# honglianghe/CDNet

Measured on AMD Instinct MI355X. Metric: tiles/sec (train fwd+bwd+Adam), 256x256, higher is better.
Workload: dtype fp32

## Files before the change

cdnet_amd/_lib.py:

```python
import ctypes as C
import os

_HERE = os.path.dirname(os.path.abspath(__file__))
LIB_PATH = os.environ.get('CDNET_LIB_PATH') or os.path.join(_HERE, 'libcdnet_hip.so')

_vp, _i, _sz, _f, _u = C.c_void_p, C.c_int, C.c_size_t, C.c_float, C.c_uint


class ConvSrc(C.Structure):
    _fields_ = [('x', C.c_void_p), ('res', C.c_void_p), ('scale', C.c_void_p), ('shift', C.c_void_p),
                ('C', C.c_int), ('Hs', C.c_int), ('Ws', C.c_int), ('pool', C.c_int), ('relu', C.c_int),
                ('off_y', C.c_int), ('off_x', C.c_int), ('f16', C.c_int), ('row_stride', C.c_int)]


class ConvArgs(C.Structure):
    _fields_ = [('src', ConvSrc * 2), ('nsrc', C.c_int), ('w', C.c_void_p), ('bias', C.c_void_p),
                ('oscale', C.c_void_p), ('oshift', C.c_void_p), ('orelu', C.c_int), ('out', C.c_void_p),
                ('Cout', C.c_int), ('out_cstride', C.c_int), ('out_coff', C.c_int), ('stats', C.c_void_p),
                ('N', C.c_int), ('H', C.c_int), ('W', C.c_int), ('taps', C.c_int), ('npar', C.c_int),
                ('ostride', C.c_int), ('nchunk', C.c_int), ('tile', C.c_int), ('CK', C.c_int), ('BN', C.c_int),
                ('out_f16', C.c_int), ('debug', C.c_int), ('ws', C.c_int), ('f32', C.c_int),
                ('eres', C.c_void_p), ('eres_scale', C.c_void_p), ('eres_shift', C.c_void_p), ('eres_f16', C.c_int), ('eres_relu', C.c_int),
                ('taps1', C.c_int), ('pad_', C.c_int), ('pool_out', C.c_void_p),
                ('dot_w', C.c_void_p), ('dot_b', C.c_void_p), ('dot_out', C.c_void_p)]


class PackJob(C.Structure):
    _fields_ = [('w', C.c_void_p), ('packed', C.c_void_p), ('Cout', C.c_int), ('Cin', C.c_int), ('KH', C.c_int), ('KW', C.c_int),
                ('CK', C.c_int), ('BN', C.c_int), ('mode', C.c_int), ('pad_', C.c_int)]


class HeadFeat(C.Structure):
    _fields_ = [('raw', C.c_void_p), ('res', C.c_void_p), ('scale', C.c_void_p), ('shift', C.c_void_p),
                ('relu', C.c_int), ('f16', C.c_int)]


class FuseTerm(C.Structure):
    _fields_ = [('x', C.c_void_p), ('Hs', C.c_int), ('Ws', C.c_int), ('scale', C.c_void_p), ('shift', C.c_void_p),
                ('f16', C.c_int), ('pad_', C.c_int)]


class GradTerm(C.Structure):
    _fields_ = [('g', C.c_void_p), ('cstride', C.c_int), ('coff', C.c_int)]


class GradIn(C.Structure):
    _fields_ = [('g', C.c_void_p), ('Hg', C.c_int), ('Wg', C.c_int), ('oy', C.c_int), ('ox', C.c_int),
                ('pooled', C.c_int), ('coff', C.c_int), ('cstride', C.c_int), ('pad_', C.c_int)]


class BnBwdArgs(C.Structure):
    _fields_ = [('raw', C.c_void_p), ('res', C.c_void_p), ('scale', C.c_void_p), ('shift', C.c_void_p),
                ('mean', C.c_void_p), ('invstd', C.c_void_p), ('gin', GradIn * 3), ('ngin', C.c_int),
                ('f16', C.c_int), ('relu', C.c_int), ('N', C.c_int), ('H', C.c_int), ('W', C.c_int), ('C', C.c_int),
                ('hc_coef', C.c_void_p), ('hc_w', C.c_void_p), ('hc_slot', C.c_int), ('hc_k0', C.c_int), ('hc_nk', C.c_int),
                ('hc_pad_', C.c_int)]


class AugSample(C.Structure):
    _fields_ = [('minv', C.c_double * 6), ('img', C.c_void_p), ('weight', C.c_void_p), ('label', C.c_void_p)] + \
        [(n, C.c_int32) for n in ('H', 'W', 'img_stride', 'weight_stride', 'label_stride', 'label_i32')] + \
        [('color', C.c_float * 4)] + [(n, C.c_int32) for n in ('hflip', 'vflip', 'filter', 'y0', 'x0')] + \
        [('alpha', C.c_float), ('sigma', C.c_float), ('seed', C.c_uint32)]


class AugGeo(C.Structure):
    _fields_ = [('paff', C.c_double * 6), ('rinv', C.c_double * 6)] + [(n, C.c_int32) for n in ('Hr', 'Wr', 'fy0', 'fx0')] + \
        [('flags', C.c_uint32), ('reserved', C.c_int32)]


class WgradReduceDesc(C.Structure):
    _fields_ = [('slab', C.c_void_p), ('dw', C.c_void_p)] + [(n, C.c_int) for n in (
        'ksplit', 'npar', 'ci_blocks', 'co_blocks', 'taps', 'CI', 'CO', 'Csrc_real', 'Cin_real', 'src_coff', 'Cout', 'mode', 'block0', 'blocks')]

class DilatedConvArgs(C.Structure):
    _fields_ = [(n, C.c_void_p) for n in ('in_', 'w', 'scale', 'shift', 'out')] + [(n, C.c_int) for n in (
        'N', 'H', 'W', 'Cin', 'in_cstride', 'Cout', 'out_cstride', 'out_coff', 'taps', 'dilation', 'leaky')] + [
        ('slope', C.c_float), ('f32', C.c_int), ('out_nchw', C.c_int)]

class DilatedBwdDataArgs(C.Structure):
    _fields_ = [(n, C.c_void_p) for n in ('g', 'w', 'dx')] + [(n, C.c_int) for n in (
        'N', 'H', 'W', 'Cout', 'g_cstride', 'Cin', 'dx_cstride', 'dx_coff', 'taps', 'dilation', 'accumulate', 'f32')]

class DilatedWgradArgs(C.Structure):
    _fields_ = [(n, C.c_void_p) for n in ('x', 'g', 'dw', 'ws')] + [('ws_bytes', C.c_size_t)] + [(n, C.c_int) for n in (
        'N', 'H', 'W', 'Cin', 'x_cstride', 'Cout', 'g_cstride', 'taps', 'dilation')]

class SliceBnFwdArgs(C.Structure):
    _fields_ = [(n, C.c_void_p) for n in ('z', 'out', 'gamma', 'beta', 'running_mean', 'running_var', 'mean', 'invstd', 'ws')] + [
        ('ws_floats', C.c_size_t), ('P', C.c_longlong)] + [(n, C.c_int) for n in ('C', 'z_cstride', 'out_cstride', 'out_coff')] + [
        (n, C.c_float) for n in ('eps', 'momentum', 'p_drop')] + [('layer', C.c_int), ('key', C.c_ulonglong)]

class SliceBnBwdArgs(C.Structure):
    _fields_ = [(n, C.c_void_p) for n in ('dy', 'z', 'mean', 'invstd', 'gamma', 'dgamma', 'dbeta', 'g', 'ws')] + [
        ('ws_floats', C.c_size_t), ('P', C.c_longlong)] + [(n, C.c_int) for n in ('C', 'z_cstride', 'dy_cstride', 'dy_coff', 'g_cstride')] + [
        (n, C.c_float) for n in ('slope', 'p_drop')] + [('layer', C.c_int), ('key', C.c_ulonglong)]


MIRRORS = {
    'cdnet_conv_src': ConvSrc, 'cdnet_conv_args': ConvArgs, 'cdnet_pack_job': PackJob, 'cdnet_head_feat': HeadFeat,
    'cdnet_wgrad_reduce_desc': WgradReduceDesc, 'cdnet_grad_in': GradIn, 'cdnet_bn_bwd_args': BnBwdArgs, 'cdnet_fuse_term': FuseTerm,
    'cdnet_grad_term': GradTerm, 'cdnet_aug_sample': AugSample, 'cdnet_aug_geo': AugGeo, 'cdnet_dilated_conv_args': DilatedConvArgs,
    'cdnet_dilated_bwd_data_args': DilatedBwdDataArgs, 'cdnet_dilated_wgrad_args': DilatedWgradArgs,
    'cdnet_slice_bn_fwd_args': SliceBnFwdArgs, 'cdnet_slice_bn_bwd_args': SliceBnBwdArgs,
}

SIGNATURES = {
    'cdnet_abi_version': (_i, []),
    'cdnet_abi_sizeof': (_sz, [C.c_char_p]),
    'cdnet_last_error': (C.c_char_p, []),
    'cdnet_build_info': (C.c_char_p, []),
    'cdnet_spin': (_i, [_i, _vp]),
    'cdnet_box_copy': (_i, [_vp, _vp, _sz, _vp]),
    'cdnet_box_mfma': (_i, [_vp, _vp, _vp, _i, _i, _i, _vp]),
    'cdnet_ddm_codes': (_i, [_vp, _i, _i, _i, _i, _vp, _i, _i, _vp, _vp, _vp]),
    'cdnet_ddm_normalize': (_i, [_vp, _vp, _i, _i, _i, _vp, _vp]),
    'cdnet_probmaps': (_i, [_vp, _vp, _i, _i, _i, _i, _vp, _vp, _vp]),
    'cdnet_tta_boost_argmax': (_i, [_vp, _vp, _vp, _vp, _i, _i, _vp, _i, _i, _vp, _vp, _vp, _vp, _vp, _vp]),
    'cdnet_fuse_sum': (_i, [_vp, _i, _i, _i, _i, _i, _i, _vp, _i, _i, _vp]),
    'cdnet_upsample_bilinear_backward': (_i, [_vp, _i, _i, _i, _i, _i, _i, _i, _i, _vp, _vp]),
    'cdnet_s2d_to_nhwc': (_i, [_vp, _i, _i, _i, _i, _vp, _vp]),
    'cdnet_fuse_sum_f32': (_i, [_vp, _i, _i, _i, _i, _i, _i, _vp, _i, _i, _vp]),
    'cdnet_upsample_bilinear_backward_f32': (_i, [_vp, _i, _i, _i, _i, _i, _i, _i, _i, _vp, _vp]),
    'cdnet_s2d_to_nhwc_f32': (_i, [_vp, _i, _i, _i, _i, _vp, _vp]),
    'cdnet_bn_backward_stats': (_i, [_vp, _vp, _vp, _vp, _vp, _sz, _vp, _vp]),
    'cdnet_bn_backward_apply': (_i, [_vp, _vp, _vp, _vp]),
    'cdnet_bn_backward_finalize': (_i, [_vp, _vp, _vp, _vp, _vp, _i, _vp, _vp]),
    'cdnet_conv_ws_eligible': (_i, [_vp]),
    'cdnet_grad_sum': (_i, [_vp, _i, _vp, C.c_longlong, _i, _vp, _vp]),
    'cdnet_grad_sum_f32': (_i, [_vp, _i, _vp, C.c_longlong, _i, _vp, _vp]),
    'cdnet_label_pair_histogram': (_i, [_vp, _vp, _i, _i, _i, _i, _vp, _vp, _vp, _vp, _vp, _vp]),
    'cdnet_remap_label': (_i, [_vp, _i, _i, _i, _vp, _vp, _vp, _vp]),
    'cdnet_label_areas': (_i, [_vp, _i, _i, _i, _vp, _vp, _vp]),
    'cdnet_label_apply': (_i, [_vp, _i, _i, _i, _vp, _vp, _vp]),
    'cdnet_label_csr_workspace_bytes': (_sz, [_i]),
    'cdnet_label_csr': (_i, [_vp, _i, _i, _i, _vp, _sz, _vp, _vp, _vp, _vp, _vp]),
    'cdnet_hausdorff_tile_pixels': (_i, []),
    'cdnet_hausdorff_chunk_pixels': (_i, []),
    'cdnet_hausdorff_pairs': (_i, [_vp] * 8 + [_i, _i, _i, _vp, _i, _vp, _i, _vp, _vp, _vp]),
    'cdnet_watershed_workspace_bytes': (_sz, [_i, _i, _i]),
    'cdnet_watershed_process': (_i, [_vp, _i, _i, _i, _i, _vp, _sz, _vp, _vp, _vp, _vp]),
    'cdnet_fill_label_process': (_i, [_vp, _i, _i, _i, _i, _vp, _sz, _vp, _vp]),
    'cdnet_label_process': (_i, [_vp, _i, _i, _i, _i, _vp, _sz, _vp, _vp]),
    'cdnet_instance_redilate_workspace_bytes': (_sz, [_i, _i, _i, _i]),
    'cdnet_instance_redilate': (_i, [_vp, _i, _i, _i, _i, _i, _vp, _sz, _vp, _vp, _vp]),
    'cdnet_instance_redilate_lds_rows': (_i, []),
    'cdnet_instance_redilate_lds_cols': (_i, []),
    'cdnet_label_count': (_i, [_vp, _i, _i, _i, _vp, _vp, _vp, _vp]),
    'cdnet_tile_postproc_workspace_bytes': (_sz, [_i, _i, _i, _i]),
    'cdnet_tile_postproc': (_i, [_vp, _vp, _vp, _i, _i, _i, _i, _vp, _i, _i, _i, _i, _vp, _sz] + [_vp] * 10),
    'cdnet_cc_workspace_bytes': (_sz, [_i, _i, _i]),
    'cdnet_cc_chain': (_i, [_vp, _i, _i, _i, _i, _i, _i, _vp, _sz, _vp, _vp, _vp, _vp, _vp, _vp]),
    'cdnet_mask_views_argmax': (_i, [_vp, _i, _i, _i, _vp, _i, _i, _vp, _vp, _vp]),
    'cdnet_tile_mask_postproc_workspace_bytes': (_sz, [_i, _i, _i, _i]),
    'cdnet_tile_mask_postproc': (_i, [_vp, _i, _i, _i, _i, _i, _i, _vp, _sz] + [_vp] * 8),
    'cdnet_dilate_labels': (_i, [_vp, _i, _i, _i, _i, _vp, _vp]),
    'cdnet_conv_packed_weight_elems': (_sz, [_i] * 6),
    'cdnet_pack_conv_weights': (_i, [_vp, _vp] + [_i] * 7 + [_vp]),
    'cdnet_pack_conv_weights_scaled': (_i, [_vp, _vp, _vp] + [_i] * 7 + [_vp]),
    'cdnet_pack_batch_table_bytes': (_sz, [_i]),
    'cdnet_pack_conv_weights_batch': (_i, [_vp, _i, _vp, _sz, _i, _vp]),
    'cdnet_conv_forward': (_i, [_vp, _vp]),
    'cdnet_dilated_packed_weight_elems': (_sz, [_i, _i, _i, _i]),
    'cdnet_dilated_pack_weights': (_i, [_vp, _vp, _i, _i, _i, _i, _vp]),
    'cdnet_dilated_conv_forward': (_i, [_vp, _vp]),
    'cdnet_dilated_pack_weights_bwd': (_i, [_vp, _vp, _i, _i, _i, _i, _vp]),
    'cdnet_dilated_conv_backward_data': (_i, [_vp, _vp]),
    'cdnet_dilated_wgrad_workspace_bytes': (_sz, [_i] * 6),
    'cdnet_dilated_conv_backward_weight': (_i, [_vp, _vp]),
    'cdnet_slice_bn_workspace_floats': (_sz, [C.c_longlong, _i]),
    'cdnet_slice_bn_train_forward': (_i, [_vp, _vp]),
    'cdnet_slice_bn_train_backward': (_i, [_vp, _vp]),
    'cdnet_dropout_mask': (_i, [C.c_ulonglong, _i, _sz, _f, _vp, _vp]),
    'cdnet_maxpool2_forward': (_i, [_vp, _i, _vp, _i, _i, _vp, _i, _i, _i, _i, _i, _i, _vp]),
    'cdnet_maxpool2_backward': (_i, [_vp, _i, _i, _vp, _i, _vp, _i, _i, _i, _i, _i, _vp]),
    'cdnet_upsample4_bilinear_forward': (_i, [_vp, _i, _vp, _i, _i, _i, _i, _i, _i, _i, _vp]),
    'cdnet_upsample4_bilinear_backward': (_i, [_vp, _i, _i, _vp, _i, _i, _i, _i, _i, _vp]),
    'cdnet_src_materialize': (_i, [_vp, _i, _i, _i, _vp, _vp]),
    'cdnet_input_pack': (_i, [_vp, _i, _i, _i, _i, _vp, _vp]),
    'cdnet_input_pack_f32': (_i, [_vp, _i, _i, _i, _i, _vp, _vp]),
    'cdnet_bn_fold_eval': (_i, [_vp, _vp, _vp, _vp, _vp, _f, _i, _vp, _vp, _vp]),
    'cdnet_bn_finalize_train': (_i, [_vp, _i, _i, _f, _vp, _vp, _vp, _f, _f, _vp, _vp, _vp, _vp, _vp, _vp, _vp]),
    'cdnet_dam_head_forward': (_i, [_vp, _vp, _vp, _vp, _i, _i, _i, _vp, _vp, _vp, _vp]),
    'cdnet_final_conv1x1': (_i, [_vp, _vp, _vp, _i, _i, _i, _i, _vp, _vp]),
    'cdnet_bias_grad_workspace_floats': (_sz, [_i]),
    'cdnet_bias_grad': (_i, [_vp, _sz, _i, _vp, _sz, _vp, _vp]),
    'cdnet_bias_grad_f32': (_i, [_vp, _sz, _i, _vp, _sz, _vp, _vp]),
    'cdnet_final_conv1x1_backward_workspace_floats': (_sz, []),
    'cdnet_final_conv1x1_backward': (_i, [_vp, _vp, _vp, _i, _i, _i, _i, _vp, _vp, _sz, _vp, _vp, _vp]),
    'cdnet_final_conv1x1_c16': (_i, [_vp, _vp, _vp, _i, _i, _i, _i, _vp, _vp]),
    'cdnet_final_conv1x1_c16_backward_workspace_floats': (_sz, []),
    'cdnet_final_conv1x1_c16_backward': (_i, [_vp, _vp, _vp, _i, _i, _i, _i, _vp, _vp, _sz, _vp, _vp, _vp]),
    'cdnet_conv_wgrad_slab_floats': (_sz, [_i] * 6),
    'cdnet_conv_backward_weight': (_i, [_vp, _i, _i, _i, _vp] + [_i] * 9 + [_vp, _vp, _i, _vp]),
    'cdnet_conv_backward_weight_last_form': (_i, []),
    'cdnet_conv_forward_last_form': (_i, []),
    'cdnet_wgrad_reduce_desc_fill': (_i, [_i] * 9 + [_vp, _vp, _i, _i, _vp]),
    'cdnet_wgrad_reduce_batch': (_i, [_vp, _i, _i, _vp]),
    'cdnet_bn_backward_workspace_floats': (_sz, [_i]),
    'cdnet_bn_backward': (_i, [_vp, _vp, _vp, _vp, _vp, _sz, _vp, _vp, _vp]),
    'cdnet_bn_backward_last_plan': (_i, []),
    'cdnet_bn_backward_last_sums_plan': (_i, []),
    'cdnet_dam_head_backward_workspace_floats': (_sz, [_i, _i, _i]),
    'cdnet_dam_head_backward': (_i, [_vp] * 7 + [_i, _i, _i, _vp, _vp, _vp, _vp, _sz, _vp, _vp]),
    'cdnet_dam_head_backward_fused_blocks': (_i, []),
    'cdnet_dam_head_backward_fused_scratch_bytes': (_i, []),
    'cdnet_dam_head_backward_fused_workspace_floats': (_sz, []),
    'cdnet_dam_head_backward_fused': (_i, [_vp] * 7 + [_i, _i, _i, _vp, _vp, _vp, _vp, _sz, _vp, _vp]),
    'cdnet_dam_head_backward_coef_scratch_bytes': (_i, []),
    'cdnet_dam_head_backward_coef': (_i, [_vp] * 7 + [_i, _i, _i, _vp, _vp, _vp, _sz, _vp, _vp]),
    'cdnet_dam_loss_workspace_floats': (_sz, [_i, _i]),
    'cdnet_dam_loss': (_i, [_vp] * 7 + [_i, _i, _i, _i, _vp, _sz, _vp, _vp, _vp, _vp, _vp]),
    'cdnet_dam_loss_classes_workspace_floats': (_sz, [_i, _i, _i]),
    'cdnet_dam_loss_classes': (_i, [_vp] * 7 + [_i, _i, _i, _i, _i, _vp, _sz, _vp, _vp, _vp, _vp, _vp]),
    'cdnet_dam_loss_terms': (_i, [_vp] * 7 + [_i, _i, _i, _i, _i, _vp, _sz, _vp, _vp, _vp, _vp, _vp, _u]),
    'cdnet_mask_loss_workspace_floats': (_sz, [_i, _i]),
    'cdnet_mask_loss': (_i, [_vp, _vp, _vp, _i, _i, _i, _u, _vp, _sz, _vp, _vp, _vp]),
    'cdnet_variance_loss_workspace_bytes': (_sz, [_i, _i, _i, _i]),
    'cdnet_variance_loss': (_i, [_vp, _vp, _i, _i, _i, _i, _i, _f, _vp, _sz, _vp, _vp, _vp, _vp, _vp, _vp]),
    'cdnet_boundary_loss_workspace_bytes': (_sz, [_i, _i, _i, _i, _i]),
    'cdnet_boundary_loss': (_i, [_vp, _vp, _i, _i, _i, _i, _i, _f, _vp, _sz, _vp, _vp, _vp, _vp]),
    'cdnet_boundary_loss_scratch_bytes': (_i, []),
    'cdnet_dam_val_sums_workspace_floats': (_sz, [_i, _i]),
    'cdnet_dam_val_sums': (_i, [_vp] * 8 + [_i, _i, _i, _vp, _sz, _vp, _vp]),
    'cdnet_dam_val_sums_classes_workspace_floats': (_sz, [_i, _i, _i]),
    'cdnet_dam_val_sums_classes': (_i, [_vp] * 8 + [_i, _i, _i, _i, _vp, _sz, _vp, _vp]),
    'cdnet_adam_step': (_i, [_vp, _vp, _vp, _vp, _sz, _f, _f, _f, _f, _f, _i, _f, _vp]),
    'cdnet_moment_step': (_i, [_vp, _vp, _vp, _vp, _vp, _sz, C.c_double, C.c_double, _f, _i, _i, _f, _f, _f, _f, _i, _f, _vp]),
    'cdnet_sgd_step': (_i, [_vp, _vp, _vp, _sz, _f, _f, _f, _i, _f, _vp]),
    'cdnet_window_pack': (_i, [_vp] + [_i] * 9 + [_vp, _vp]),
    'cdnet_window_pack_f32': (_i, [_vp] + [_i] * 9 + [_vp, _vp]),
    'cdnet_window_stitch': (_i, [_vp] + [_i] * 9 + [_vp, _vp]),
    'cdnet_label_encoding_workspace_bytes': (_sz, [_i, _i, _i, _i]),
    'cdnet_label_encoding_instances_workspace_bytes': (_sz, [_i, _i, _i, _i]),
    'cdnet_label_encoding_instances': (_i, [_vp, _i, _i, _i, _i, _vp, _vp, _vp, _sz, _vp, _vp, _vp, _vp, _vp, _vp]),
    'cdnet_augment_workspace_bytes': (_sz, [_i, _i, _i]),
    'cdnet_augment_batch': (_i, [_vp, _vp, _i, _i, _vp, _vp, _sz, _vp, _vp, _vp, _i, _vp, _vp, _vp]),
    'cdnet_augment_geo_workspace_bytes': (_sz, [_i, _i, _i, _i]),
    'cdnet_augment_batch_geo': (_i, [_vp, _vp, _vp, _vp, _i, _i, _i, _vp, _vp, _sz, _vp, _vp, _vp, _i, _vp, _vp, _vp]),
    'cdnet_label_encoding': (_i, [_vp, _i, _i, _i, _i, _vp, _vp, _vp, _sz, _vp, _vp, _vp, _vp, _vp, _vp]),
    'cdnet_weight_map_radius': (_i, [C.c_double, C.c_double]),
    'cdnet_weight_map': (_i, [_vp, _i, _i, C.c_double, C.c_double, _vp, _vp]),
    'cdnet_resize_workspace_bytes': (_sz, [_i] * 7),
    'cdnet_resize_bilinear': (_i, [_vp] + [_i] * 6 + [_vp, _vp, _i, _vp, _vp, _i, _i, _i, _vp, _sz, _vp, _vp]),
    'cdnet_resize_last_form': (_i, []),
    'cdnet_fill_remove_small': (_i, [_vp, _i, _i, _i, _i, _i, _vp, _sz, _vp, _vp]),
    'cdnet_label8_dilate': (_i, [_vp, _i, _i, _i, _i, _vp, _sz, _vp, _vp, _vp, _vp]),
}

_lib = None


class CdnetHipError(RuntimeError):
    pass


def load():
    global _lib
    if _lib is not None:
        return _lib
    import torch
    if not os.path.exists(LIB_PATH):
        raise CdnetHipError('libcdnet_hip.so is not built: run `python -m cdnet_amd.csrc.build` '
                            '(or __graft_entry__.build()). There is no CPU fallback.')
    lib = C.CDLL(LIB_PATH)
    for name, (res, args) in SIGNATURES.items():
        fn = getattr(lib, name)
        fn.restype = res
        fn.argtypes = args
    if lib.cdnet_abi_version() != 5:
        raise CdnetHipError('ABI version mismatch (libcdnet_hip.so is version %d, this binding 5): rebuild with python -m cdnet_amd.csrc.build' % lib.cdnet_abi_version())
    _lib = lib
    return lib


def check(status, what=''):
    if status != 0:
        msg = load().cdnet_last_error().decode(errors='replace')
        raise CdnetHipError('%s failed (code %d): %s' % (what, status, msg))


def call(name, *args):
    check(getattr(load(), name)(*args), name)


def entry(name, f32):
    return name + '_f32' if f32 else name


_RAW_STREAM = None


def stream_ptr():
    global _RAW_STREAM
    if _RAW_STREAM is None:
        import torch
        get, dev = getattr(torch._C, '_cuda_getCurrentRawStream', None), getattr(torch._C, '_cuda_getDevice', None)
        if get is not None and dev is not None:
            _RAW_STREAM = lambda: get(dev())
        else:
            _RAW_STREAM = lambda: torch.cuda.current_stream().cuda_stream
    return C.c_void_p(_RAW_STREAM())


def ptr(t):
    if t is None:
        return None
    assert t.is_cuda and t.is_contiguous(), 'ABI needs contiguous device tensors'
    return C.c_void_p(t.data_ptr())
```

cdnet_amd/csrc/build.py:

```python
import os
import subprocess
import sys

HERE = os.path.dirname(os.path.abspath(__file__))
PKG = os.path.dirname(HERE)
LIB = os.path.join(PKG, 'libcdnet_hip.so')
OBJ_DIR = os.path.join(HERE, 'build')
SOURCES = ['abi.hip', 'box.hip', 'postproc.hip', 'postproc_tile.hip', 'conv.hip', 'conv_ws.hip', 'pack.hip', 'conv32.hip', 'conv32ws.hip', 'conv16ws.hip', 'dilated.hip', 'dilated_train.hip', 'resample.hip', 'wgrad.hip', 'model.hip', 'head_bwd.hip', 'classifier16.hip', 'dam_loss.hip', 'bn_bwd.hip', 'cdm.hip', 'metrics.hip', 'augment.hip', 'optim.hip', 'variance.hip', 'boundary.hip', 'mask_loss.hip', 'weight_map.hip', 'instance_fill.hip', 'resize.hip']
FLAGS = ['--offload-arch=gfx950', '-O3', '-std=c++20', '-fPIC', '-ffp-contract=off', '-Wall',
         '-Wno-unused-function', '-Wno-unused-result']


def _newer(a, bs):
    return os.path.exists(a) and all(os.path.getmtime(a) >= os.path.getmtime(b) for b in bs)


def build(force=False, verbose=False):
    hipcc = os.environ.get('HIPCC', 'hipcc')
    flags = FLAGS + os.environ.get('CDNET_HIPCC_FLAGS', '').split()
    os.makedirs(OBJ_DIR, exist_ok=True)
    headers = [os.path.join(HERE, f) for f in os.listdir(HERE) if f.endswith('.h')]
    headers.append(os.path.join(os.path.dirname(PKG), 'include', 'cdnet_hip.h'))
    objs, procs = [], []
    for s in SOURCES:
        src = os.path.join(HERE, s)
        if not os.path.exists(src):
            continue
        obj = os.path.join(OBJ_DIR, s.replace('.hip', '.o'))
        objs.append(obj)
        if force or not _newer(obj, [src] + headers):
            cmd = [hipcc] + flags + ['-c', src, '-o', obj]
            if verbose:
                print(' '.join(cmd))
            procs.append((s, subprocess.Popen(cmd)))
    for s, p in procs:
        if p.wait() != 0:
            raise RuntimeError('hipcc failed on ' + s)
    if force or procs or not _newer(LIB, objs):
        cmd = [hipcc, '--offload-arch=gfx950', '-shared', '-fPIC', '-o', LIB] + objs
        if verbose:
            print(' '.join(cmd))
        subprocess.check_call(cmd)
    return LIB


if __name__ == '__main__':
    print(build(force='--force' in sys.argv, verbose=True))
```

cdnet_amd/csrc/conv32.hip:

```cpp
#include <type_traits>
#include "common.h"
#include "conv_args.h"
#include "launch.h"
#include "split_bf16.h"
#include <stdlib.h>

using namespace cdnet;

namespace {

constexpr int CK = 16;
constexpr int PSTR = CK * 2 + 16;
constexpr int XF_MAX = 2048;

template <int TH, int TW, int BN, int TAPS>
struct Lds32 {
    static constexpr int NPIX = (TH + 2) * (TW + 2);
    static constexpr int A_PLANE = NPIX * PSTR;
    static constexpr int B_PLANE = TAPS * CK * BN * 2;
    static constexpr int STAGE = 2 * A_PLANE + 2 * B_PLANE;
    static constexpr int STATS_BYTES = 4 * 2 * BN * 4;
    static constexpr int MAIN = ((STAGE > STATS_BYTES ? STAGE : STATS_BYTES) + 15) / 16 * 16;
    static int bytes(int ctot) { return MAIN + 2 * ((ctot + 7) / 8 * 8) * 4; }
};


template <int MPW, int NPW, int TW>
__device__ __forceinline__ void store_tile_f32(const ConvArgs &A, const f32x16 (&acc)[MPW][NPW], int n, int y0, int x0, int mblock0, int nblock0,
                                               int half, int l31, int cout0, int pa_, int pb_) {
    const int Ho = A.H * A.ostride, Wo = A.W * A.ostride;
    float *out = reinterpret_cast<float *>(A.out);
    const float *eres = reinterpret_cast<const float *>(A.eres);
    const bool full = y0 + 16 <= A.H && x0 + TW <= A.W && cout0 + (nblock0 + NPW) * 32 <= A.Cout && A.ostride == 1 && TW == 16 &&
                      !(A.debug & 16);
    if (full) {
        const int cs = A.out_cstride, ce = A.Cout;
        float *tb = out + (((size_t)n * A.H + y0) * A.W + x0) * cs + A.out_coff;
        const float *te = eres ? eres + (((size_t)n * A.H + y0) * A.W + x0) * ce : nullptr;
#pragma unroll
        for (int ni = 0; ni < NPW; ++ni) {
            const int co = cout0 + (nblock0 + ni) * 32 + l31;
            const float osc = A.oscale ? A.oscale[co] : 1.f;
            const float osh = fmaf(A.bias ? A.bias[co] : 0.f, osc, A.oshift ? A.oshift[co] : 0.f);
            const float esc = (eres && A.eres_scale) ? A.eres_scale[co] : 1.f;
            const float esh = (eres && A.eres_shift) ? A.eres_shift[co] : 0.f;
            float *ob = tb + co;
#pragma unroll
            for (int mi = 0; mi < MPW; ++mi) {
                const int rowb = ((mblock0 + mi) * 2) * A.W + 4 * half;
                float ev[16];
                if (eres) {
#pragma unroll
                    for (int r = 0; r < 16; ++r) {
                        const int p = (r & 3) + 8 * (r >> 2);
                        ev[r] = te[(rowb + (p / 16) * A.W + (p % 16)) * ce + co];
                    }
                }
#pragma unroll
                for (int r = 0; r < 16; ++r) {
                    const int p = (r & 3) + 8 * (r >> 2);
                    const int off = (rowb + (p / 16) * A.W + (p % 16)) * cs;
                    float v = fmaf(acc[mi][ni][r], osc, osh);
                    if (A.orelu) v = fmaxf(v, 0.f);
                    if (eres) {
                        v = fmaf(ev[r], esc, esh) + v;
                        if (A.eres_relu) v = fmaxf(v, 0.f);
                    }
                    ob[off] = v;
                }
            }
        }
        return;
    }
#pragma unroll
    for (int ni = 0; ni < NPW; ++ni) {
        const int co = cout0 + (nblock0 + ni) * 32 + l31;
        const bool cok = co < A.Cout;
        const float osc = (A.oscale && cok) ? A.oscale[co] : 1.f;
        const float osh = fmaf((A.bias && cok) ? A.bias[co] : 0.f, osc, (A.oshift && cok) ? A.oshift[co] : 0.f);
        const float esc = (A.eres && A.eres_scale && cok) ? A.eres_scale[co] : 1.f;
        const float esh = (A.eres && A.eres_shift && cok) ? A.eres_shift[co] : 0.f;
#pragma unroll
        for (int mi = 0; mi < MPW; ++mi) {
            float ev[16];
            if (A.eres) {
#pragma unroll
                for (int r = 0; r < 16; ++r) {
                    const int m = (mblock0 + mi) * 32 + (r & 3) + 8 * (r >> 2) + 4 * half;
                    int y = y0 + m / TW, x = x0 + m % TW;
                    y = y < A.H ? y : A.H - 1; x = x < A.W ? x : A.W - 1;
                    ev[r] = eres[(((size_t)n * A.H + y) * A.W + x) * A.Cout + (cok ? co : 0)];
                }
            }
#pragma unroll
            for (int r = 0; r < 16; ++r) {
                const int m = (mblock0 + mi) * 32 + (r & 3) + 8 * (r >> 2) + 4 * half;
                const int y = y0 + m / TW, x = x0 + m % TW;
                float v = fmaf(acc[mi][ni][r], osc, osh);
                if (A.orelu) v = fmaxf(v, 0.f);
                if (A.eres) {
                    v = fmaf(ev[r], esc, esh) + v;
                    if (A.eres_relu) v = fmaxf(v, 0.f);
                }
                if (cok && y < A.H && x < A.W) {
                    const size_t opix = ((size_t)n * Ho + (y * A.ostride + pa_)) * Wo + (x * A.ostride + pb_);
                    out[opix * A.out_cstride + A.out_coff + co] = v;
                }
            }
        }
    }
}

template <int TH, int TW, int BN, int WM, int WN, int TAPS>
__global__ __launch_bounds__(256, 2) void conv_f32_kernel(ConvArgs A) {
    using L = Lds32<TH, TW, BN, TAPS>;
    constexpr int HW_ = TW + 2, NPIX = L::NPIX;
    constexpr int MT = TH * TW / 32, NT = BN / 32;
    constexpr int MPW = MT / WM, NPW = NT / WN;
    constexpr int VPP = CK / 8;
    constexpr int NA = (NPIX * VPP + 255) / 256;
    constexpr int NBV = 2 * L::B_PLANE / 16;
    constexpr int NB = (NBV + 255) / 256;
    static_assert(MT % WM == 0 && NT % WN == 0 && WM * WN == 4, "wave tiling");

    extern __shared__ __attribute__((aligned(16))) unsigned char smem[];
    unsigned char *lds_a = smem;
    unsigned char *lds_b = smem + 2 * L::A_PLANE;
    float (*s_stats)[2][BN] = reinterpret_cast<float (*)[2][BN]>(smem);
    float *s_xf = reinterpret_cast<float *>(smem + L::MAIN);

    const int tid = threadIdx.x, lane = tid & 63, wave = tid >> 6;
    const int wm = wave / WN, wn = wave % WN;
    const int half = lane >> 5, l31 = lane & 31;
    const int c0n = A.src[0].C, ctot = c0n + (A.nsrc > 1 ? A.src[1].C : 0);
    const int xfs = (ctot + 7) / 8 * 8;
    for (int c = tid; c < ctot; c += 256) {
        const ConvSrc &S = c < c0n ? A.src[0] : A.src[1];
        const int cc = c < c0n ? c : c - c0n;
        s_xf[c] = S.scale ? S.scale[cc] : 1.f;
        s_xf[xfs + c] = S.shift ? S.shift[cc] : 0.f;
    }

    const int tiles_x = (A.W + TW - 1) / TW, tiles_y = (A.H + TH - 1) / TH;
    const int tiles_img = tiles_x * tiles_y;
    int tile, cout_tile;
    {
        const int NC = (int)gridDim.y, lin = (int)blockIdx.y * (int)gridDim.x + (int)blockIdx.x;
        const int T = (int)gridDim.x * NC, q = T >> 3, rem = T & 7;
        const int xcd = lin & 7, idx = lin >> 3;
        const int seq = xcd < rem ? xcd * (q + 1) + idx : rem * (q + 1) + (xcd - rem) * q + idx;
        tile = seq / NC;
        cout_tile = seq - tile * NC;
    }
    const int z = tile / tiles_img, rt = tile - z * tiles_img;
    const int n = z / A.npar, par = z - n * A.npar;
    const int ty_ = rt / tiles_x;
    const int y0 = ty_ * TH, x0 = (rt - ty_ * tiles_x) * TW;

    int eoff[2][NA];
    const int slot = tid % VPP;
#pragma unroll
    for (int si = 0; si < 2; ++si) {
        if (si >= A.nsrc) break;
        const ConvSrc &s = A.src[si];
        const int rs = s.row_stride ? s.row_stride : s.Ws * s.C;
#pragma unroll
        for (int i = 0; i < NA; ++i) {
            const int v = tid + i * 256;
            const int pix = v / VPP;
            const int hy = pix / HW_, hx = pix - hy * HW_;
            const int y = y0 - 1 + hy, x = x0 - 1 + hx;
            const int ys = y - s.off_y, xs = x - s.off_x;
            const bool ok = v < NPIX * VPP && (unsigned)y < (unsigned)A.H && (unsigned)x < (unsigned)A.W && (unsigned)ys < (unsigned)s.Hs &&
                            (unsigned)xs < (unsigned)s.Ws;
            eoff[si][i] = ok ? ys * rs + xs * s.C + slot * 8 : -1;
        }
    }
    auto chunk_src = [&](int c, int &si, int &cc0) {
        const int n0 = A.src[0].C / CK;
        if (c < n0) { si = 0; cc0 = c * CK; } else { si = 1; cc0 = (c - n0) * CK; }
    };
    const unsigned short *wbase = A.w + ((size_t)(par * gridDim.y + cout_tile) * A.nchunk) * (size_t)(L::B_PLANE);

    f32x4 pa[NA][2];
    u32x4 pb[NB];
    auto issue = [&](int chunk) {
        int si, cc0;
        chunk_src(chunk, si, cc0);
        const ConvSrc &s = A.src[si];
        const size_t rs = s.row_stride ? (size_t)s.row_stride : (size_t)s.Ws * s.C;
        const float *base = reinterpret_cast<const float *>(s.x) + (size_t)n * s.Hs * rs + cc0;
#pragma unroll
        for (int i = 0; i < NA; ++i) {
            const int e = si ? eoff[1][i] : eoff[0][i];
            const f32x4 *p = reinterpret_cast<const f32x4 *>(base + (e >= 0 ? e : 0));
            pa[i][0] = p[0];
            pa[i][1] = p[1];
        }
        const u32x4 *wsrc = reinterpret_cast<const u32x4 *>(wbase + (size_t)chunk * L::B_PLANE);
#pragma unroll
        for (int i = 0; i < NB; ++i) {
            const int v = tid + i * 256;
            if (v < NBV) pb[i] = wsrc[v];
        }
    };
    auto commit = [&](int chunk) {
        int si, cc0;
        chunk_src(chunk, si, cc0);
        const ConvSrc &s = A.src[si];
        const bool on = s.scale != nullptr, relu = s.relu != 0;
        const float *xf = s_xf + (si ? c0n : 0) + cc0 + slot * 8;
        float sc[8], sh[8];
        if (on) {
#pragma unroll
            for (int j = 0; j < 8; ++j) { sc[j] = xf[j]; sh[j] = xf[xfs + j]; }
        }
        f32x4 rr[NA][2];
        if (s.res) {
            const size_t rs = s.row_stride ? (size_t)s.row_stride : (size_t)s.Ws * s.C;
            const float *rbase = reinterpret_cast<const float *>(s.res) + (size_t)n * s.Hs * rs + cc0;
#pragma unroll
            for (int i = 0; i < NA; ++i) {
                const int e = si ? eoff[1][i] : eoff[0][i];
                const f32x4 *p = reinterpret_cast<const f32x4 *>(rbase + (e >= 0 ? e : 0));
                rr[i][0] = p[0];
                rr[i][1] = p[1];
            }
        }
        unsigned char *dst0 = lds_a + (tid / VPP) * PSTR + slot * 16;
#pragma unroll
        for (int i = 0; i < NA; ++i) {
            if (tid + i * 256 >= NPIX * VPP) continue;
            const int e = si ? eoff[1][i] : eoff[0][i];
            u32x4 hi = {0u, 0u, 0u, 0u}, lo = {0u, 0u, 0u, 0u};
            if (e >= 0) {
                float v[8] = {pa[i][0][0], pa[i][0][1], pa[i][0][2], pa[i][0][3], pa[i][1][0], pa[i][1][1], pa[i][1][2], pa[i][1][3]};
                if (on) {
#pragma unroll
                    for (int j = 0; j < 8; ++j) v[j] = fmaf(v[j], sc[j], sh[j]);
                }
                if (s.res) {
                    const float r[8] = {rr[i][0][0], rr[i][0][1], rr[i][0][2], rr[i][0][3], rr[i][1][0], rr[i][1][1], rr[i][1][2], rr[i][1][3]};
#pragma unroll
                    for (int j = 0; j < 8; ++j) v[j] += r[j];
                }
                if (relu) {
#pragma unroll
                    for (int j = 0; j < 8; ++j) v[j] = fmaxf(v[j], 0.f);
                }
                split8(v, hi, lo);
            }
            unsigned char *d = dst0 + i * (256 / VPP) * PSTR;
            *reinterpret_cast<u32x4 *>(d) = hi;
            *reinterpret_cast<u32x4 *>(d + L::A_PLANE) = lo;
        }
        u32x4 *bdst = reinterpret_cast<u32x4 *>(lds_b);
#pragma unroll
        for (int i = 0; i < NB; ++i) {
            const int v = tid + i * 256;
            if (v < NBV) bdst[v] = pb[i];
        }
    };

    int abase[MPW];
#pragma unroll
    for (int mi = 0; mi < MPW; ++mi) {
        const int m = (wm * MPW + mi) * 32 + l31;
        abase[mi] = ((m / TW) * HW_ + m % TW) * PSTR + half * 16;
    }
    const int bbase = half * BN * 16 + (wn * NPW * 32 + l31) * 16;
    int toff[TAPS];
#pragma unroll
    for (int t = 0; t < TAPS; ++t) {
        int r, c;
        if (TAPS == 9) { r = t / 3; c = t % 3; }
        else if (TAPS == 4) {
            const int a = par >> 1, b = par & 1, ty = t >> 1, tx = t & 1;
            r = a == 0 ? (ty == 0 ? 1 : 0) : (ty == 0 ? 2 : 1);
            c = b == 0 ? (tx == 0 ? 1 : 0) : (tx == 0 ? 2 : 1);
        } else { r = 1; c = 1; }
        toff[t] = (r * HW_ + c) * PSTR;
    }
    f32x16 acc[MPW][NPW];
#pragma unroll
    for (int mi = 0; mi < MPW; ++mi)
#pragma unroll
        for (int ni = 0; ni < NPW; ++ni)
#pragma unroll
            for (int r = 0; r < 16; ++r) acc[mi][ni][r] = 0.f;

    issue(0);
    for (int chunk = 0; chunk < A.nchunk; ++chunk) {
        __syncthreads();
        commit(chunk);
        __syncthreads();
        if (chunk + 1 < A.nchunk) issue(chunk + 1);
#pragma unroll
        for (int t = 0; t < TAPS; ++t) {
            bf16x8 ah[MPW], al[MPW], bh[NPW], bl[NPW];
#pragma unroll
            for (int mi = 0; mi < MPW; ++mi) {
                ah[mi] = *reinterpret_cast<const bf16x8 *>(lds_a + abase[mi] + toff[t]);
                al[mi] = *reinterpret_cast<const bf16x8 *>(lds_a + L::A_PLANE + abase[mi] + toff[t]);
            }
#pragma unroll
            for (int ni = 0; ni < NPW; ++ni) {
                bh[ni] = *reinterpret_cast<const bf16x8 *>(lds_b + bbase + t * 2 * BN * 16 + ni * 512);
                bl[ni] = *reinterpret_cast<const bf16x8 *>(lds_b + L::B_PLANE + bbase + t * 2 * BN * 16 + ni * 512);
            }
#pragma unroll
            for (int mi = 0; mi < MPW; ++mi)
#pragma unroll
                for (int ni = 0; ni < NPW; ++ni) {
                    acc[mi][ni] = mfma3(acc[mi][ni], ah[mi], al[mi], bh[ni], bl[ni]);
                }
        }
    }
    __syncthreads();

    const int cout0 = cout_tile * BN;
    if (A.stats) {
        float ssum[NPW], ssq[NPW];
        const bool full_tile = y0 + TH <= A.H && x0 + TW <= A.W && !(A.debug & 16);
#pragma unroll
        for (int ni = 0; ni < NPW; ++ni) {
            ssum[ni] = 0.f; ssq[ni] = 0.f;
            if (full_tile) {
#pragma unroll
                for (int mi = 0; mi < MPW; ++mi)
#pragma unroll
                    for (int r = 0; r < 16; ++r) {
                        const float v = acc[mi][ni][r];
                        ssum[ni] += v;
                        ssq[ni] = fmaf(v, v, ssq[ni]);
                    }
            } else {
#pragma unroll
            for (int mi = 0; mi < MPW; ++mi)
#pragma unroll
                for (int r = 0; r < 16; ++r) {
                    const int m = (wm * MPW + mi) * 32 + (r & 3) + 8 * (r >> 2) + 4 * half;
                    const float v = ((y0 + m / TW) < A.H && (x0 + m % TW) < A.W) ? acc[mi][ni][r] : 0.f;
                    ssum[ni] += v;
                    ssq[ni] = fmaf(v, v, ssq[ni]);
                }
            }
            ssum[ni] += __shfl_xor(ssum[ni], 32);
            ssq[ni] += __shfl_xor(ssq[ni], 32);
            if (half == 0) {
                s_stats[wave][0][(wn * NPW + ni) * 32 + l31] = ssum[ni];
                s_stats[wave][1][(wn * NPW + ni) * 32 + l31] = ssq[ni];
            }
        }
        __syncthreads();
        if (tid < 2 * BN) {
            const int which = tid / BN, col = tid % BN;
            const int wn_of = col / (NPW * 32);
            float v = 0.f;
#pragma unroll
            for (int k = 0; k < WM; ++k) v += s_stats[k * WN + wn_of][which][col];
            const int co = cout0 + col;
            if (co < A.Cout) A.stats[((size_t)tile * 2 + which) * A.Cout + co] = v;
        }
    }
    store_tile_f32<MPW, NPW, TW>(A, acc, n, y0, x0, wm * MPW, wn * NPW, half, l31, cout0, par >> 1, par & 1);
}

template <int TH, int TW, int BN, int WM, int WN, int TAPS>
int launch_conv32(const ConvArgs &A, hipStream_t st) {
    using L = Lds32<TH, TW, BN, TAPS>;
    int ctot = 0;
    for (int i = 0; i < A.nsrc; ++i) ctot += A.src[i].C;
    const int smem = L::bytes(ctot);
    dim3 grid(cdiv(A.W, TW) * cdiv(A.H, TH) * A.N * A.npar, cdiv(A.Cout, BN), 1);
    g_conv_last_form = conv_form(CDNET_CONV_FAMILY_F32, BN, TAPS, 0, false, false, false, 0, 0, TH);
    return launch_lds<conv_f32_kernel<TH, TW, BN, WM, WN, TAPS>>(grid, 256, L::bytes(XF_MAX), smem, st, "hipFuncSetAttribute(conv32)", "conv_f32_kernel", A);
}

template <int TAPS>
int dispatch_conv32(const ConvArgs &A, hipStream_t st) {
    if (A.tile == 16 && A.BN == 64) return launch_conv32<16, 16, 64, 4, 1, TAPS>(A, st);
    if (A.tile == 16 && A.BN == 32) return launch_conv32<16, 16, 32, 4, 1, TAPS>(A, st);
    if (A.tile == 8 && A.BN == 64) return launch_conv32<8, 8, 64, 2, 2, TAPS>(A, st);
    set_error("cdnet_conv_forward(f32): unsupported configuration tile=%d CK=%d BN=%d", A.tile, A.CK, A.BN);
    return CDNET_E_ARG;
}

template <int BN, int NCH, bool XF, bool ERES>
__global__ __launch_bounds__(256, 4) void conv1x1_f32_stream_kernel(ConvArgs A) {
    constexpr int NPW = BN / 32;
    constexpr int B_PLANE = CK * BN * 2;
    constexpr int CIN = NCH * CK;
    __shared__ __attribute__((aligned(16))) unsigned char smem[NCH * 2 * B_PLANE + 2 * CIN * 4];
    unsigned char *lds_b = smem;
    float *s_xf = reinterpret_cast<float *>(smem + NCH * 2 * B_PLANE);

    const int tid = threadIdx.x, lane = tid & 63, wave = __builtin_amdgcn_readfirstlane(tid >> 6);
    const int half = lane >> 5, l31 = lane & 31;
    const int cout_tile = blockIdx.y, cout0 = cout_tile * BN;
    const ConvSrc &S = A.src[0];
    {
        const u32x4 *wsrc = reinterpret_cast<const u32x4 *>(A.w + (size_t)cout_tile * NCH * B_PLANE);
        u32x4 *bdst = reinterpret_cast<u32x4 *>(lds_b);
        for (int v = tid; v < NCH * 2 * B_PLANE / 16; v += 256) bdst[v] = wsrc[v];
        for (int c = tid; c < CIN; c += 256) {
            s_xf[c] = S.scale ? S.scale[c] : 1.f;
            s_xf[CIN + c] = S.shift ? S.shift[c] : 0.f;
        }
    }
    __syncthreads();

    const size_t P = (size_t)A.N * A.H * A.W;
    const int nblk = (int)((P + 31) / 32), bstride = (int)gridDim.x * 4;
    int blk = (int)blockIdx.x * 4 + wave;
    if (blk >= nblk) return;
    const bool relu = S.relu != 0, orelu = A.orelu != 0, eres_relu = A.eres_relu != 0;
    const int cout = A.Cout;
    const int bbase = half * BN * 16 + l31 * 16;

    float osc[NPW], osh[NPW], esc[NPW], esh[NPW];
#pragma unroll
    for (int ni = 0; ni < NPW; ++ni) {
        const int co = cout0 + ni * 32 + l31, c = co < A.Cout ? co : 0;
        osc[ni] = A.oscale ? A.oscale[c] : 1.f;
        osh[ni] = fmaf(A.bias ? A.bias[c] : 0.f, osc[ni], A.oshift ? A.oshift[c] : 0.f);
        esc[ni] = (ERES && A.eres_scale) ? A.eres_scale[c] : 1.f;
        esh[ni] = (ERES && A.eres_shift) ? A.eres_shift[c] : 0.f;
    }

    const char *xbase = reinterpret_cast<const char *>(S.x);
    char *obase = reinterpret_cast<char *>(A.out) + (size_t)A.out_coff * 4;
    const char *ebase = ERES ? reinterpret_cast<const char *>(A.eres) : xbase;
    const unsigned cs4 = (unsigned)A.out_cstride * 4, ce4 = (unsigned)cout * 4;
    const unsigned vo_in = l31 * (CIN * 4) + half * 32;
    unsigned vo_out[NPW], vo_eres[NPW];
#pragma unroll
    for (int ni = 0; ni < NPW; ++ni) {
        const unsigned co = cout0 + ni * 32 + l31;
        vo_out[ni] = co < (unsigned)cout ? 4 * half * cs4 + co * 4 : 0x7fff0000u;
        vo_eres[ni] = co < (unsigned)cout ? 4 * half * ce4 + co * 4 : 0x7fff0000u;
    }
    auto rsrc = [&](const char *base, size_t bytes) {
        return __builtin_amdgcn_make_buffer_rsrc(const_cast<char *>(base), 0, (int)bytes, 0x00020000);
    };

    auto request = [&](f32x4 (&v)[NCH][2], int b) {
        const size_t left = P - (size_t)b * 32;
        const __amdgpu_buffer_rsrc_t rx = rsrc(xbase + (size_t)b * (32 * CIN * 4), (left < 32 ? left : 32) * (CIN * 4));
#pragma unroll
        for (int c = 0; c < NCH; ++c) {
            v[c][0] = __builtin_bit_cast(f32x4, __builtin_amdgcn_raw_buffer_load_b128(rx, (int)(vo_in + c * 64), 0, 0));
            v[c][1] = __builtin_bit_cast(f32x4, __builtin_amdgcn_raw_buffer_load_b128(rx, (int)(vo_in + c * 64 + 16), 0, 0));
        }
    };
    auto block = [&](auto tail_c, const f32x4 (&cur)[NCH][2], f32x4 (&nxt)[NCH][2]) {
        constexpr bool TAIL = decltype(tail_c)::value;
        asm volatile("" ::: "memory");
        if (!TAIL) {
            request(nxt, blk + bstride < nblk ? blk + bstride : blk);
            __builtin_amdgcn_sched_barrier(0);
        }
        f32x16 acc[NPW];
#pragma unroll
        for (int ni = 0; ni < NPW; ++ni)
#pragma unroll
            for (int r = 0; r < 16; ++r) acc[ni][r] = 0.f;
#pragma unroll
        for (int c = 0; c < NCH; ++c) {
            float v[8] = {cur[c][0][0], cur[c][0][1], cur[c][0][2], cur[c][0][3], cur[c][1][0], cur[c][1][1], cur[c][1][2], cur[c][1][3]};
            if (XF) {
                const float *xf = s_xf + c * CK + half * 8;
#pragma unroll
                for (int j = 0; j < 8; ++j) {
                    v[j] = fmaf(v[j], xf[j], xf[CIN + j]);
                    v[j] = relu ? fmaxf(v[j], 0.f) : v[j];
                }
            }
            u32x4 hi, lo;
            split8(v, hi, lo);
            const bf16x8 ah = __builtin_bit_cast(bf16x8, hi), al = __builtin_bit_cast(bf16x8, lo);
#pragma unroll
            for (int ni = 0; ni < NPW; ++ni) {
                const bf16x8 bh = *reinterpret_cast<const bf16x8 *>(lds_b + c * 2 * B_PLANE + bbase + ni * 512);
                const bf16x8 bl = *reinterpret_cast<const bf16x8 *>(lds_b + c * 2 * B_PLANE + B_PLANE + bbase + ni * 512);
                acc[ni] = mfma3(acc[ni], ah, al, bh, bl);
            }
        }
        const size_t left = P - (size_t)blk * 32, rows = left < 32 ? left : 32;
        const __amdgpu_buffer_rsrc_t ro = rsrc(obase + (size_t)blk * 32 * cs4, rows * cs4);
        float ev[NPW][16];
        if (ERES) {
            const __amdgpu_buffer_rsrc_t re = rsrc(ebase + (size_t)blk * 32 * ce4, rows * ce4);
#pragma unroll
            for (int ni = 0; ni < NPW; ++ni)
#pragma unroll
                for (int r = 0; r < 16; ++r) {
                    const unsigned pr = (r & 3) + 8 * (r >> 2);
                    ev[ni][r] = __builtin_bit_cast(float, TAIL ? __builtin_amdgcn_raw_buffer_load_b32(re, (int)(vo_eres[ni] + pr * ce4), 0, 0)
                                                               : __builtin_amdgcn_raw_buffer_load_b32(re, (int)vo_eres[ni], (int)(pr * ce4), 0));
                }
        }
#pragma unroll
        for (int ni = 0; ni < NPW; ++ni)
#pragma unroll
            for (int r = 0; r < 16; ++r) {
                const unsigned pr = (r & 3) + 8 * (r >> 2);
                float v = fmaf(acc[ni][r], osc[ni], osh[ni]);
                v = orelu ? fmaxf(v, 0.f) : v;
                if (ERES) {
                    v = fmaf(ev[ni][r], esc[ni], esh[ni]) + v;
                    v = eres_relu ? fmaxf(v, 0.f) : v;
                }
                if (TAIL) __builtin_amdgcn_raw_buffer_store_b32(__builtin_bit_cast(unsigned, v), ro, (int)(vo_out[ni] + pr * cs4), 0, 0);
                else __builtin_amdgcn_raw_buffer_store_b32(__builtin_bit_cast(unsigned, v), ro, (int)vo_out[ni], (int)(pr * cs4), 0);
            }
    };
    f32x4 xa[NCH][2], xb[NCH][2];
    const int nfull = (int)(P / 32);
    if (blk < nfull) {
        request(xa, blk);
#pragma unroll
        for (int c = 0; c < NCH; ++c) asm volatile("" ::"v"(xa[c][0]), "v"(xa[c][1]));
        for (;;) {
            block(std::false_type{}, xa, xb);
            blk += bstride;
            if (blk >= nfull) break;
            block(std::false_type{}, xb, xa);
            blk += bstride;
            if (blk >= nfull) break;
        }
    }
    if (blk < nblk) {
        request(xa, blk);
        block(std::true_type{}, xa, xb);
    }
}

template <int BN, int NCH>
int launch_conv1x1_stream(const ConvArgs &A, hipStream_t st) {
    int n_cu = 0;
    if (const int rc = cu_count(&n_cu)) return rc;
    const long long nblk = ((long long)A.N * A.H * A.W + 31) / 32;
    const int ctiles = cdiv(A.Cout, BN);
    const long long waves = (long long)n_cu * 16 / ctiles > 4 ? (long long)n_cu * 16 / ctiles : 4;
    const long long rounds = (nblk + waves - 1) / waves;
    const long long G = ((nblk + rounds - 1) / rounds + 3) / 4;
    dim3 grid((unsigned)G, ctiles, 1);
    return with_bool(A.src[0].scale != nullptr, [&](auto xf_c) {
        return with_bool(A.eres != nullptr, [&](auto er_c) {
            g_conv_last_form = conv_form(CDNET_CONV_FAMILY_STREAM, BN, 1, decltype(xf_c)::value ? 1 : 0, false, false, false, 0, 0, 16, 16, NCH, decltype(er_c)::value);
            conv1x1_f32_stream_kernel<BN, NCH, decltype(xf_c)::value, decltype(er_c)::value><<<grid, 256, 0, st>>>(A);
            return check_launch("conv1x1_f32_stream_kernel");
        });
    });
}

int try_conv1x1_stream(const ConvArgs &A, hipStream_t st) {
    if (A.debug & CONV_DBG_NO_STREAM_1X1) return -1;
    if (A.taps != 1 || A.taps1 != 0 || A.npar != 1 || A.ostride != 1 || A.ws || A.stats || A.pool_out || A.nsrc != 1) return -1;
    const ConvSrc &s = A.src[0];
    if (s.off_y || s.off_x || s.Hs != A.H || s.Ws != A.W || (s.row_stride && s.row_stride != s.Ws * s.C) || s.pool || s.res) return -1;
    if (s.relu && !s.scale) return -1;
    if (s.C != A.nchunk * CK || (long long)A.N * A.H * A.W > (1LL << 31) - 64 || (long long)A.out_cstride * 4 * 36 >= (1LL << 31)) return -1;
    auto go = [&](auto bn_c) -> int {
        constexpr int BN = decltype(bn_c)::value;
        if (A.nchunk == 1) return launch_conv1x1_stream<BN, 1>(A, st);
        if (A.nchunk == 2) return launch_conv1x1_stream<BN, 2>(A, st);
        if (A.nchunk == 4) return launch_conv1x1_stream<BN, 4>(A, st);
        return -1;
    };
    if (A.BN == 64) return go(std::integral_constant<int, 64>{});
    if (A.BN == 32) return go(std::integral_constant<int, 32>{});
    return -1;
}

__global__ __launch_bounds__(256) void materialize_f32_kernel(const ConvSrc s, int N, int H, int W, float *__restrict__ out) {
    const int VPP = s.C / 4;
    const size_t total = (size_t)N * H * W * VPP;
    const bool relu = s.relu != 0, on = s.scale != nullptr;
    const int Hl = s.pool ? (s.Hs + (s.pool == 2)) / 2 : s.Hs, Wl = s.pool ? (s.Ws + (s.pool == 2)) / 2 : s.Ws;
    const size_t rs = s.row_stride ? (size_t)s.row_stride : (size_t)s.Ws * s.C;
    const float *sx = reinterpret_cast<const float *>(s.x), *sr = reinterpret_cast<const float *>(s.res);
    for (size_t i = (size_t)blockIdx.x * 256 + threadIdx.x; i < total; i += (size_t)gridDim.x * 256) {
        const int c = (int)(i % VPP) * 4;
        const size_t pix = i / VPP;
        const int x = (int)(pix % W), y = (int)((pix / W) % H), n = (int)(pix / ((size_t)W * H));
        float4 sc = make_float4(1.f, 1.f, 1.f, 1.f), sh = make_float4(0.f, 0.f, 0.f, 0.f);
        if (on) { sc = *reinterpret_cast<const float4 *>(s.scale + c); sh = *reinterpret_cast<const float4 *>(s.shift + c); }
        const size_t img = (size_t)n * s.Hs * rs;
        float4 val = make_float4(0.f, 0.f, 0.f, 0.f);
        const int ys = y - s.off_y, xs = x - s.off_x;
        auto xf = [&](float4 v, const float4 *r) {
            v.x = fmaf(v.x, sc.x, sh.x); v.y = fmaf(v.y, sc.y, sh.y); v.z = fmaf(v.z, sc.z, sh.z); v.w = fmaf(v.w, sc.w, sh.w);
            if (r) { v.x += r->x; v.y += r->y; v.z += r->z; v.w += r->w; }
            if (relu) { v.x = fmaxf(v.x, 0.f); v.y = fmaxf(v.y, 0.f); v.z = fmaxf(v.z, 0.f); v.w = fmaxf(v.w, 0.f); }
            return v;
        };
        if (ys >= 0 && ys < Hl && xs >= 0 && xs < Wl) {
            if (!s.pool) {
                const size_t e = img + (size_t)ys * rs + (size_t)xs * s.C + c;
                const float4 raw = *reinterpret_cast<const float4 *>(sx + e);
                if (sr) { const float4 r = *reinterpret_cast<const float4 *>(sr + e); val = xf(raw, &r); }
                else val = xf(raw, nullptr);
            } else {
                float4 raw[4];
                bool ok[4];
#pragma unroll
                for (int q = 0; q < 4; ++q) {
                    int yy = 2 * ys + (q >> 1), xx = 2 * xs + (q & 1);
                    ok[q] = q == 0 || (yy < s.Hs && xx < s.Ws);
                    yy = yy < s.Hs ? yy : s.Hs - 1;
                    xx = xx < s.Ws ? xx : s.Ws - 1;
                    raw[q] = *reinterpret_cast<const float4 *>(sx + img + (size_t)yy * rs + (size_t)xx * s.C + c);
                }
#pragma unroll
                for (int q = 0; q < 4; ++q) {
                    const float4 t = xf(raw[q], nullptr);
                    if (q == 0) val = t;
                    else if (ok[q]) { val.x = fmaxf(val.x, t.x); val.y = fmaxf(val.y, t.y); val.z = fmaxf(val.z, t.z); val.w = fmaxf(val.w, t.w); }
                }
            }
        }
        *reinterpret_cast<float4 *>(out + pix * s.C + c) = val;
    }
}

}

namespace cdnet {

int conv_forward_f32(const ConvArgs &A, hipStream_t st) {
    CDNET_REQUIRE(A.CK == 16, "cdnet_conv_forward(f32): CK must be 16 (got %d)", A.CK);
    for (int i = 0; i < A.nsrc; ++i)
        CDNET_REQUIRE(!A.src[i].pool, "cdnet_conv_forward(f32): pooled sources must be materialised (cdnet_src_materialize)");
    CDNET_REQUIRE(!A.out_f16, "cdnet_conv_forward(f32): out_f16 must be 0");
    {
        const int rc = conv_forward_f32_ws(A, st);
        if (rc >= 0) return rc;
    }
    CDNET_REQUIRE(A.ws != 2, "cdnet_conv_forward(f32): the BatchNorm-backward statistics epilogue (ws = 2) needs the producer / consumer kernel "
                             "(ask cdnet_conv_ws_eligible first)");
    CDNET_REQUIRE(A.taps1 == 0 || A.taps1 == A.taps, "cdnet_conv_forward(f32): a one-tap second source runs on conv_ws32_kernel only (ask cdnet_conv_ws_eligible)");
    CDNET_REQUIRE(!A.pool_out, "cdnet_conv_forward(f32): the fused max-pool output rides in conv_ws32_kernel's epilogue only (ask cdnet_conv_ws_eligible)");
    if (A.taps == 9) return dispatch_conv32<9>(A, st);
    if (A.taps == 4) return dispatch_conv32<4>(A, st);
    {
        const int rc = try_conv1x1_stream(A, st);
        if (rc >= 0) return rc;
    }
    return dispatch_conv32<1>(A, st);
}

int materialize_f32(const ConvSrc &s, int N, int H, int W, void *out, hipStream_t st) {
    const size_t total = (size_t)N * H * W * (s.C / 4);
    size_t g = (total + 255) / 256;
    g = g > 8192 ? 8192 : g;
    materialize_f32_kernel<<<(int)g, 256, 0, st>>>(s, N, H, W, reinterpret_cast<float *>(out));
    return check_launch("cdnet_src_materialize(f32)");
}

}
```

cdnet_amd/csrc/conv_args.h:

```cpp
#pragma once
#include "../../include/cdnet_hip.h"

struct ConvSrc {
    const unsigned short *x;
    const unsigned short *res;
    const float *scale;
    const float *shift;
    int C, Hs, Ws, pool, relu, off_y, off_x;
    int f16, row_stride;
};

struct ConvArgs {
    ConvSrc src[2];
    int nsrc;
    const unsigned short *w;
    const float *bias;
    const float *oscale;
    const float *oshift;
    int orelu;
    unsigned short *out;
    int Cout, out_cstride, out_coff;
    float *stats;
    int N, H, W;
    int taps, npar, ostride, nchunk;
    int tile, CK, BN;
    int out_f16;
    int debug;
    int ws;
    int f32;
    const unsigned short *eres;
    const float *eres_scale, *eres_shift;
    int eres_f16, eres_relu;
    int taps1, pad_;
    unsigned short *pool_out;
    const float *dot_w, *dot_b;
    float *dot_out;
};

enum : int {
    CONV_DBG_WS16_QUAD = 16,
    CONV_DBG_ONE_TILE = 32,
    CONV_DBG_PERSIST_SMALL = 64,
    CONV_DBG_OLD_WS16 = 128,
    CONV_DBG_NO_STREAM_1X1 = 256,
    CONV_DBG_GRID_SHIFT = 8,
};
enum : int {
    WGRAD_DBG_NO_WS = 8,
    WGRAD_DBG_ALL_QUADS = 16,
};

static_assert(sizeof(ConvSrc) == sizeof(cdnet_conv_src), "ConvSrc layout");
static_assert(sizeof(ConvArgs) == sizeof(cdnet_conv_args), "ConvArgs layout");

namespace cdnet {
extern thread_local int g_conv_last_form;
constexpr int conv_form(int family, int bn, int taps, int xf = 0, bool stats = false, bool stream = false, bool mix = false, int ncs = 0,
                        int site = 0, int tile = 16, int ck = 16, int nch = 0, bool eres = false) {
    return family | ((bn == 128 ? 2 : (bn == 64 ? 1 : 0)) << 4) | (taps << 6) | (xf << 10) | ((stats ? 1 : 0) << 12) | ((stream ? 1 : 0) << 13) |
           ((mix ? 1 : 0) << 14) | (ncs << 15) | (site << 17) | ((tile == 8 ? 1 : 0) << 20) | ((ck == 64 ? 2 : (ck == 32 ? 1 : 0)) << 21) |
           (nch << 23) | ((eres ? 1 : 0) << 26);
}
int conv_forward_f32(const ConvArgs &A, hipStream_t st);
int conv_forward_f32_ws(const ConvArgs &A, hipStream_t st, bool dry_run = false);
int conv_forward_ws16(const ConvArgs &A, hipStream_t st, bool dry_run = false);
int conv_forward_ws(const ConvArgs &A, hipStream_t st, bool dry_run = false);
int materialize_f32(const ConvSrc &s, int N, int H, int W, void *out, hipStream_t st);
}
```

cdnet_amd/engine.py:

```python
import ctypes as C
import os
import torch

from . import _lib
from ._lib import ConvArgs, ConvSrc, PackJob


def _dp(t):
    return None if t is None else t.data_ptr()


class Src:
    __slots__ = ('x', 'scale', 'shift', 'relu', 'pool', 'res', 'off', 'N', 'Hs', 'Ws', 'Cc', 'ptr_off', 'row_stride', 'grad_to', 'is_input')

    def __init__(self, x, scale=None, shift=None, relu=False, pool=False, res=None, off=(0, 0), view=None, grad_to=None, is_input=False):
        assert x.dtype in (torch.bfloat16, torch.float16, torch.float32) and x.is_contiguous()
        assert res is None or res.dtype == x.dtype
        self.x, self.scale, self.shift, self.relu, self.pool, self.res, self.off = x, scale, shift, relu, pool, res, off
        self.grad_to, self.is_input = grad_to, is_input
        if view is None:
            assert x.dim() == 4
            self.N, self.Hs, self.Ws, self.Cc = x.shape
            self.ptr_off, self.row_stride = 0, 0
        else:
            self.ptr_off, self.Hs, self.Ws, self.Cc, self.row_stride = view
            self.N = x.shape[0]

    @property
    def f16(self):
        return {torch.bfloat16: 0, torch.float16: 1, torch.float32: 2}[self.x.dtype]

    @property
    def f32(self):
        return self.x.dtype == torch.float32

    @property
    def C(self):
        return self.Cc

    def ptr(self):
        return self.x.data_ptr() + self.x.element_size() * self.ptr_off

    def logical_hw(self):
        h, w = self.Hs, self.Ws
        if self.pool:
            c = 1 if int(self.pool) == 2 else 0
            return ((h + c) // 2, (w + c) // 2)
        return (h, w)

    def fill(self, cs):
        cs.x = self.ptr()
        cs.res = _dp(self.res)
        cs.scale, cs.shift = _dp(self.scale), _dp(self.shift)
        cs.C, cs.Hs, cs.Ws = self.C, self.Hs, self.Ws
        cs.pool, cs.relu = int(self.pool), int(self.relu)
        cs.off_y, cs.off_x = self.off
        cs.f16 = int(self.f16)
        cs.row_stride = int(self.row_stride)


_SUPPORTED = {(16, 16, 32), (16, 16, 64), (16, 32, 32), (16, 32, 64), (16, 32, 128), (16, 64, 64),
              (8, 32, 64), (8, 32, 128), (8, 64, 64)}


def choose_cfg(src_channels, Cout, H, W, override=None, taps=9, transposed=False, N=16, f32=False):
    if f32:
        assert all(c % 16 == 0 for c in src_channels), src_channels
        assert override is None or (tuple(override)[1] == 16 and tuple(override) in ((16, 16, 64), (16, 16, 32), (8, 16, 64))), \
            'fp32 precision: configuration override %s is not one of the fp32 kernels' % (override,)
        if override is not None:
            return tuple(override)
        small = min(H, W) <= 8 or (min(H, W) <= 16 and N <= 32)
        if small and Cout > 32:
            if os.environ.get('CDNET_F32_WS16', '1') == '1' and taps == 9 and not transposed and H == 16 and W == 16 and \
                    sum(src_channels) >= 256 and Cout >= 256 and 8 <= N <= 32:
                return (16, 16, 32)
            return (8, 16, 64)
        return (16, 16, 64 if Cout > 32 else 32)
    if override is not None:
        assert tuple(override) in _SUPPORTED, override
        return tuple(override)
    ctot = sum(src_channels)
    small = min(H, W) <= 8 or (min(H, W) <= 16 and N <= 32)
    ck = 64
    while any(c % ck for c in src_channels):
        ck //= 2
    assert ck >= 16, 'source channels must be multiples of 16: %s' % (src_channels,)
    if small:
        ws16 = taps == 9 and not transposed and H % 16 == 0 and W % 16 == 0 and min(H, W) == 16 and ctot % 64 == 0 and 256 <= ctot <= 768
        if ck >= 32 and not ws16:
            return (8, 32, 64)
    if ck == 64:
        ck = 32
    bn = 64 if Cout > 32 else 32
    if ck >= 16:
        ck = 16
    if ck == 16 and bn > 64:
        bn = 64
    return (16, ck, bn)


def dominant_kernel_name(precision, tiles=16):
    if precision == 'fp32':
        return 'conv_ws32_kernel<64,0,false>'
    quad = tiles * 256 * 256 * (64 + 64) * 2 >= (512 << 20)
    return 'conv_ws16_kernel<64,0,false,false,0,4,4,true,false,true,%s>' % ('true' if quad else 'false')


def packed_elems(Cout, nchunk, taps, CK, BN, npar):
    return _lib.load().cdnet_conv_packed_weight_elems(Cout, nchunk, taps, CK, BN, npar)


def _pack_dims(w, cfg, mode):
    _, CK, BN = cfg[:3]
    if mode == 0:
        Cout, Cin, KH, KW = w.shape
    elif mode == 1:
        Cin, Cout, KH, KW = w.shape
    elif mode in (4, 5, 6):
        Cout, ct, KH, KW = w.shape
        Cin = 4 * ct
    elif mode == 7:
        Cin, ct, KH, KW = w.shape
        Cout = 4 * ct
    else:
        Cin, Cout, KH, KW = w.shape
    taps = {2: 4, 3: 1, 4: 9, 5: 1, 6: 9, 7: 9}.get(mode, KH * KW)
    npar = 4 if mode in (2, 3) else 1
    return Cout, Cin, KH, KW, CK, BN, taps, npar


def pack_job(w, cfg, mode, out, split=False):
    Cout, Cin, KH, KW, CK, BN, taps, npar = _pack_dims(w, cfg, mode)
    assert out.numel() == packed_elems(Cout, Cin // CK, taps, CK, BN, npar) * (2 if split else 1)
    j = PackJob()
    j.w, j.packed, j.Cout, j.Cin, j.KH, j.KW, j.CK, j.BN = w.data_ptr(), out.data_ptr(), Cout, Cin, KH, KW, CK, BN
    j.mode = mode | (PACK_SPLIT if split else 0)
    return j


PACK_SPLIT = 16


def pack_weights(w, cfg, mode, Cin_pad=None, out=None, split=False, cout_scale=None):
    assert w.dtype == torch.float32 and w.is_cuda and w.is_contiguous()
    Cout, Cin, KH, KW, CK, BN, taps, npar = _pack_dims(w, cfg, mode)
    Cin_p = Cin if Cin_pad is None else Cin_pad
    if Cin_p != Cin:
        if mode == 0:
            wp = torch.zeros((Cout, Cin_p, KH, KW), dtype=torch.float32, device=w.device)
            wp[:, :Cin] = w
        else:
            raise NotImplementedError
        w, Cin = wp.contiguous(), Cin_p
    n = packed_elems(Cout, Cin // CK, taps, CK, BN, npar) * (2 if split else 1)
    if out is None or out.numel() != n:
        out = torch.empty((n,), dtype=torch.int16, device=w.device)
    if cout_scale is not None:
        assert mode == 0 and cout_scale.dtype == torch.float32 and cout_scale.numel() == Cout
        _lib.call('cdnet_pack_conv_weights_scaled', _lib.ptr(w), _lib.ptr(cout_scale), _lib.ptr(out), Cout, Cin, KH, KW, CK, BN,
                  mode | (PACK_SPLIT if split else 0), _lib.stream_ptr())
        return out
    _lib.call('cdnet_pack_conv_weights', _lib.ptr(w), _lib.ptr(out), Cout, Cin, KH, KW, CK, BN, mode | (PACK_SPLIT if split else 0),
              _lib.stream_ptr())
    return out


CONV_DEBUG = 0


def conv_forward(srcs, wpacked, Cout, cfg, taps=9, transposed=False, bias=None, oscale=None, oshift=None,
                 orelu=False, out=None, stats=None, H=None, W=None, out_dtype=torch.bfloat16, eres=None, query_ws=False, bns=None, taps1=0, pool_out=None, dot=None,
                 pad_chunks=0, debug_or=0, out_coff=0):
    tile, CK, BN = cfg[:3]
    s0 = srcs[0]
    f32 = s0.f32
    assert all(s.f32 == f32 for s in srcs)
    if f32:
        out_dtype = torch.float32
    N = s0.N
    if H is None:
        H, W = s0.logical_hw()
        H, W = H + 0, W + 0
    ostride = 2 if transposed else 1
    npar = 4 if transposed else 1
    a = ConvArgs()
    nchunk = 0
    for i, s in enumerate(srcs):
        assert s.C % CK == 0, (s.C, CK)
        s.fill(a.src[i])
        nchunk += s.C // CK
    a.nsrc = len(srcs)
    if dot is not None:
        assert out is None and stats is None and eres is None and bns is None and pool_out is None and not f32 and not transposed
        a.dot_w, a.dot_b, a.dot_out = dot[0].data_ptr(), dot[1].data_ptr(), dot[2].data_ptr()
        assert dot[0].numel() == Cout and dot[0].dtype == torch.float32 and dot[2].dtype == torch.float32 and dot[2].numel() == N * H * W
    elif out is None:
        out = torch.empty((N, H * ostride, W * ostride, Cout), dtype=out_dtype, device=s0.x.device)
    ntiles = ((H + tile - 1) // tile) * ((W + tile - 1) // tile)
    if stats is True:
        stats = torch.empty((N * npar * ntiles, 2, Cout), dtype=torch.float32, device=s0.x.device)
    a.w, a.bias, a.oscale, a.oshift = _dp(wpacked), _dp(bias), _dp(oscale), _dp(oshift)
    a.orelu = int(orelu)
    a.out, a.Cout, a.out_cstride, a.out_coff = (None if out is None else out.data_ptr()), Cout, (Cout if out is None else out.shape[3]), out_coff
    a.stats = _dp(stats)
    a.N, a.H, a.W = N, H, W
    assert pad_chunks == 0 or (len(srcs) == 2 and taps == 9 and not f32 and all(s.scale is None and not s.relu and s.res is None and not s.f16 for s in srcs))
    a.taps, a.npar, a.ostride, a.nchunk = taps, npar, ostride, nchunk + pad_chunks
    a.tile, a.CK, a.BN = tile, CK, BN
    a.out_f16 = int(out is not None and out.dtype == torch.float16)
    a.ws = 0
    a.taps1 = taps1
    a.pool_out = _dp(pool_out)
    a.debug = CONV_DEBUG | debug_or
    a.f32 = int(f32)
    assert out is None or (out.dtype == torch.float32) == f32
    if eres is not None:
        assert not transposed and stats is None and not orelu and out.dtype == (torch.float32 if f32 else torch.bfloat16) and tuple(eres.x.shape) == tuple(out.shape)
        assert eres.f32 == f32
        a.eres, a.eres_scale, a.eres_shift = eres.x.data_ptr(), _dp(eres.scale), _dp(eres.shift)
        a.eres_f16, a.eres_relu = int(eres.f16), int(eres.relu)
    if bns is not None:
        raw, sc, sh, mu, inv, partial = bns
        assert eres is None and stats is None and bias is None and oscale is None and oshift is None and tuple(raw.shape) == tuple(out.shape)
        a.ws = 2
        a.eres, a.oscale, a.oshift, a.eres_scale, a.eres_shift, a.stats = raw.data_ptr(), sc.data_ptr(), sh.data_ptr(), mu.data_ptr(), inv.data_ptr(), partial.data_ptr()
    if query_ws:
        return int(_lib.load().cdnet_conv_ws_eligible(C.byref(a)))
    _lib.call('cdnet_conv_forward', C.byref(a), _lib.stream_ptr())
    return out, stats
```

cdnet_amd/trainer.py:

```python
import ctypes as C
import os

import torch

from . import _lib, engine, optim, runtime, streams
from ._lib import BnBwdArgs, GradIn, GradTerm
from .allreduce import BucketReducer, bucketed_allreduce
from .engine import Src
from .optim import HEAD_PARAMS, FlatState
from .synth import synthetic_batch


_WGRAD_WGS_DEEP, _WGRAD_WGS_SHALLOW = 128, 160
_WGRAD_WGS_KQ = 128
_WGRAD_WGS_F32 = 160
_RU_1X1_SIDE = True
WGRAD_STREAM = True
HEAD_BWD_FUSE = True
HEAD_COEF_SRC = os.environ.get('CDNET_HEAD_COEF_SRC', '1') != '0'
_WGRAD_DEFER = 0x100
_WGRAD_DEEP_HW = 16384


class _on_stream:
    __slots__ = ('s', 'prev')

    def __init__(self, s):
        self.s = s

    def __enter__(self):
        self.prev = torch.cuda.current_stream()
        torch.cuda.set_stream(self.s)

    def __exit__(self, *exc):
        torch.cuda.set_stream(self.prev)
        return False


class _G:
    __slots__ = ('t', 'Hg', 'Wg', 'oy', 'ox', 'pooled', 'coff', 'cstride', 'event', 'masked', 'hc')

    def __init__(self, t, Hg, Wg, oy=0, ox=0, pooled=0, coff=0, cstride=0):
        self.t, self.Hg, self.Wg, self.oy, self.ox, self.pooled, self.coff, self.cstride = t, Hg, Wg, oy, ox, pooled, coff, cstride
        self.event = None
        self.masked = False
        self.hc = None


def _choose_ci_tiles(C_src, Cout):
    if Cout <= 32 and runtime.PRECISION != 'fp32':
        return 1
    best, best_cost = 2, None
    for ci_t in (2, 1, 4):
        CI, CO = ci_t * 32, (4 // ci_t) * 32
        cost = -(-C_src // CI) * CI * -(-Cout // CO) * CO
        if best_cost is None or cost < best_cost:
            best, best_cost = ci_t, cost
    return best


def _wgrad_wgs(beside, HW, Cout):
    if not beside:
        return 256
    if runtime.PRECISION == 'fp32':
        return _WGRAD_WGS_F32
    if Cout <= 32 and HW > 65536:
        return _WGRAD_WGS_KQ
    return _WGRAD_WGS_DEEP if HW <= _WGRAD_DEEP_HW or HW > 65536 else _WGRAD_WGS_SHALLOW


class Trainer:
    def __init__(self, model, lr=1e-3, weight_decay=1e-4, betas=(0.9, 0.99), eps=None, quirk_sample0=True,
                 world_size=1, bucket_mb=25, optimizer='adam', momentum=0.95):
        self.model = model
        self._pack_jobs = None
        self._pack_prec = None
        self._ar = None
        self.optimizer = str(optimizer).lower()
        if self.optimizer not in optim.OPTIMIZERS:
            raise ValueError('Optimizer {} not available (one of {})'.format(optimizer, ', '.join(optim.OPTIMIZERS)))
        if eps is None:
            eps = optim.RANGER_EPS if self.optimizer == 'ranger' else 1e-8
        self.lr, self.wd, self.betas, self.eps, self.momentum = lr, weight_decay, betas, eps, momentum
        self.quirk = int(quirk_sample0)
        self.world = world_size
        self.bucket = int(float(bucket_mb) * (1 << 20) // 4)
        self.flat = FlatState(model, self.optimizer)
        frozen = set(self.flat.frozen)
        self._frozen_ids = frozenset(id(p) for n, p in model.named_parameters() if n in frozen)
        self._nograd = set()
        self.narrowed = {}
        model._trainer_bound = True
        model._head_flat = self.flat.P[:self.flat.n_head] if self.flat.n_head == 855 else None
        self.dev = self.flat.P.device
        self._bufs = {}
        self._wss = {}
        self.losses = torch.zeros((11,), dtype=torch.float32, device=self.dev)
        self.alpha = 0.0
        self.dice, self.weight_map = 1, 1
        self.loss_var = torch.full((1,), -1.0, dtype=torch.float32, device=self.dev)
        self.boundary = 0
        self.loss_boundary = torch.zeros((1,), dtype=torch.float32, device=self.dev)
        self.tape = []
        self._cat_cache = {}
        self._wstream, self._events = None, {}
        self.ar_stats = None
        self._packb_pending = False
        self._packb_stream = True
        self._side_active = False
        self.head_fused = False
        self.head_coef = False
        self._rd_mb = float(os.environ.get('CDNET_WGRAD_REDUCE_MB', '300'))
        self._rd_pending, self._rd_params, self._rd_bytes, self._rd_tables = [], [], 0, {}
        self._forwards, self._bn_base = 0, 0
        if world_size > 1:
            self.sync_from_rank0()

    def sync_from_rank0(self, src=0):
        import torch.distributed as dist
        if not (dist.is_available() and dist.is_initialized()) or dist.get_world_size() == 1:
            return
        f = self.flat
        works = [dist.broadcast(t, src=src, async_op=True) for t in (f.P, f.M, f.V, f.S) if t is not None]
        meta = torch.tensor([float(f.step_count), float(self._bn_base + self._forwards)], dtype=torch.float64, device=self.dev)
        works.append(dist.broadcast(meta, src=src, async_op=True))
        bufs = [b for b in self.model.buffers() if b.is_floating_point()]
        if bufs:
            flatb = torch.cat([b.detach().reshape(-1).float() for b in bufs])
            dist.broadcast(flatb, src=src)
            off = 0
            with torch.no_grad():
                for b in bufs:
                    b.copy_(flatb[off:off + b.numel()].view(b.shape))
                    off += b.numel()
        for w in works:
            w.wait()
        f.step_count = int(meta[0].item())
        self._bn_base, self._forwards = int(meta[1].item()), 0
        self.refresh_parameters()

    def reduce_scalars(self, values):
        import torch.distributed as dist
        if self.world <= 1 or not (dist.is_available() and dist.is_initialized()):
            return values
        t = torch.as_tensor(values, dtype=torch.float64).to(self.dev)
        dist.all_reduce(t, op=dist.ReduceOp.SUM)
        return (t / dist.get_world_size()).cpu().numpy()

    def buf(self, key, shape, dtype):
        b = self._bufs.get(key)
        if b is None or tuple(b.shape) != tuple(shape) or b.dtype != dtype:
            b = torch.empty(shape, dtype=dtype, device=self.dev)
            self._bufs[key] = b
        return b

    def _ws(self, name, need, side=False):
        ws = self._wss.get(name)
        if ws is None or ws.numel() < need:
            if side and self._wstream is not None:
                self._wstream.synchronize()
            ws = self._wss[name] = torch.empty((need,), dtype=torch.float32, device=self.dev)
        return ws

    def grad_sum(self, gl, mask, npix, Cc, out):
        assert 1 <= len(gl) <= 6
        arr = (GradTerm * len(gl))()
        for k, g in enumerate(gl):
            assert not g.pooled and g.oy == 0 and g.ox == 0
            arr[k].g, arr[k].cstride, arr[k].coff = g.t.data_ptr(), g.cstride or Cc, g.coff
        _lib.call(_lib.entry('cdnet_grad_sum', out.dtype == torch.float32), C.byref(arr), len(gl), None if mask is None else _lib.ptr(mask),
                  npix, Cc, _lib.ptr(out), _lib.stream_ptr())

    def take(self, grads, key):
        gl = grads.pop(key, None)
        if gl is not None:
            for g_ in gl:
                if g_.event is not None:
                    torch.cuda.current_stream().wait_event(g_.event)
                    g_.event = None
        return gl

    def cat_grad(self, o, grads):
        key = id(o)
        if key not in self._cat_cache:
            gl = self.take(grads, key)
            if gl is None:
                d = None
            elif len(gl) == 1 and not gl[0].coff and gl[0].cstride in (0, o.shape[3]):
                d = gl[0].t
            else:
                d = self.buf(('dcat', key), o.shape, runtime.act_dtype())
                self.grad_sum(gl, None, o.shape[0] * o.shape[1] * o.shape[2], o.shape[3], d)
            self._cat_cache[key] = d
        return self._cat_cache[key]

    def forward(self, x):
        m = self.model
        m.train()
        self._forwards += 1
        runtime.TAPE = self.tape
        del self.tape[:]
        try:
            out = m(x)
        finally:
            runtime.TAPE = None
        return out

    def loss_and_grads(self, mask, point, direction, label, dirlab, point_t, weight):
        B, _, H, W = mask.shape
        lib = _lib.load()
        ND = direction.shape[1]
        ws = self._ws('loss', lib.cdnet_dam_loss_classes_workspace_floats(B, H * W, ND))
        dmask = self.buf('dmask', mask.shape, torch.float32)
        dpoint = self.buf('dpoint', point.shape, torch.float32)
        ddir = self.buf('ddir', direction.shape, torch.float32)
        assert label.dtype == torch.uint8 and dirlab.dtype == torch.uint8 and weight.dtype == torch.uint8
        assert point_t.dtype == torch.float16
        if self.dice != 1:
            raise ValueError('dice = %r with a DAM model: the reference dies on an unbound loss_direction_dice (train_util_dam.py:297); only 1 works'
                             % (self.dice,))
        from .utils import loss_terms
        terms = loss_terms(self.dice, self.weight_map, self.alpha)
        args = (_lib.ptr(mask), _lib.ptr(point), _lib.ptr(direction), _lib.ptr(label.contiguous()),
                _lib.ptr(dirlab.contiguous()), _lib.ptr(point_t.contiguous()), _lib.ptr(weight.contiguous()), B, H, W, ND,
                self.quirk, _lib.ptr(ws), ws.numel(), _lib.ptr(self.losses), _lib.ptr(dmask),
                _lib.ptr(dpoint), _lib.ptr(ddir), _lib.stream_ptr())
        if terms == 7:
            _lib.call('cdnet_dam_loss_classes', *args)
        else:
            _lib.call('cdnet_dam_loss_terms', *args, terms)
        if self.alpha:
            self._variance_term(mask, label, dmask)
        if self.boundary:
            self._boundary_term(mask, label, dmask)
        return dmask, dpoint, ddir

    def _variance_term(self, mask, label, dmask, total=None):
        if self.alpha not in (1, 2):
            raise ValueError('alpha = %r: the variance term is built for alpha = 1 and 2 (0 switches it off)' % (self.alpha,))
        B, K, H, W = mask.shape
        need = _lib.load().cdnet_variance_loss_workspace_bytes(B, K, H, W)
        ws = self._ws('variance', (need + 3) // 4)
        total = self.losses[0:1] if total is None else total
        _lib.call('cdnet_variance_loss', _lib.ptr(mask), _lib.ptr(label.contiguous()), 1, B, K, H, W, float(self.alpha), _lib.ptr(ws),
                  ws.numel() * 4, _lib.ptr(self.loss_var), None if dmask is None else _lib.ptr(total), None if dmask is None else _lib.ptr(dmask),
                  None, None, _lib.stream_ptr())

    def _boundary_term(self, mask, label, dmask, total=None):
        if self.boundary not in (1, 2, 3):
            raise ValueError('boundary = %r: 1 (BoundaryLoss), 2 (FocalLoss2d) or 3 (RobustFocalLoss2d); 0 switches the term off' % (self.boundary,))
        B, K, H, W = mask.shape
        need = _lib.load().cdnet_boundary_loss_workspace_bytes(self.boundary, B, K, H, W)
        if need == 0:
            raise ValueError('the boundary term serves three-class mask logits, got %s' % (tuple(mask.shape),))
        ws = self._ws('boundary', (need + 3) // 4)
        total = self.losses[0:1] if total is None else total
        _lib.call('cdnet_boundary_loss', _lib.ptr(mask), _lib.ptr(label.contiguous()), self.boundary, B, K, H, W, 1.0, _lib.ptr(ws),
                  ws.numel() * 4, _lib.ptr(self.loss_boundary), _lib.ptr(total), _lib.ptr(dmask), _lib.stream_ptr())

    def backward(self, dmask, dpoint, ddir):
        m = self.model
        f1, f2, f3 = m._last_feats
        N, H, W, _ = f1.x.shape
        hf = [runtime.head_feat(f) for f in (f1, f2, f3)]
        dhead = self.flat.G[:self.flat.n_head]
        owner = self._head_fusable(f1, f2, f3)
        self.head_fused = owner is not None
        self.head_coef = owner is not None and HEAD_COEF_SRC and os.environ.get('CDNET_BN_DZ_REUSE', '1').strip() not in ('0', '') \
            and self._head_coef_ok(f1) and self._head_coef_ok(f2)
        if self.head_coef:
            coef = self.buf('head_coef', (N, H, W, 16), torch.float32)
            dz3 = self.buf('dF2', (N, H, W, 64), torch.float32)
            hw = m.head_weight_block()
            ws = self._ws('head', _lib.load().cdnet_dam_head_backward_fused_workspace_floats())
            _lib.call('cdnet_dam_head_backward_coef', C.byref(hf[0]), C.byref(hf[1]), C.byref(hf[2]), _lib.ptr(hw), _lib.ptr(dmask),
                      _lib.ptr(dpoint), _lib.ptr(ddir), N, H, W, _lib.ptr(coef), _lib.ptr(dz3), _lib.ptr(ws), ws.numel(), _lib.ptr(dhead),
                      _lib.stream_ptr())
            heads = [(f1.x, _G(None, H, W)), (f2.x, _G(None, H, W)), (f3.x, _G(dz3, H, W))]
            heads[0][1].hc = (coef, hw, 640, 10, 3)
            heads[1][1].hc = (coef, hw, 64, 1, 9)
            heads[2][1].masked = True
            self._run_tape(heads, None)
            return
        df = [self.buf('dF%d' % k, (N, H, W, 64), runtime.act_dtype()) for k in range(3)]
        if owner is not None:
            ws = self._ws('head', _lib.load().cdnet_dam_head_backward_fused_workspace_floats())
            _lib.call('cdnet_dam_head_backward_fused', C.byref(hf[0]), C.byref(hf[1]), C.byref(hf[2]), _lib.ptr(m.head_weight_block()),
                      _lib.ptr(dmask), _lib.ptr(dpoint), _lib.ptr(ddir), N, H, W, _lib.ptr(df[0]), _lib.ptr(df[1]), _lib.ptr(df[2]),
                      _lib.ptr(ws), ws.numel(), _lib.ptr(dhead), _lib.stream_ptr())
            heads = [(f.x, _G(d, H, W)) for f, d in zip((f1, f2, f3), df)]
            heads[2][1].masked = True
            self._run_tape(heads, None)
            return
        ws = self._ws('head', _lib.load().cdnet_dam_head_backward_workspace_floats(N, H, W))
        _lib.call('cdnet_dam_head_backward', C.byref(hf[0]), C.byref(hf[1]), C.byref(hf[2]), _lib.ptr(m.head_weight_block()),
                  _lib.ptr(dmask), _lib.ptr(dpoint), _lib.ptr(ddir), N, H, W, _lib.ptr(df[0]), _lib.ptr(df[1]),
                  _lib.ptr(df[2]), _lib.ptr(ws), ws.numel(), _lib.ptr(dhead), _lib.stream_ptr())
        self._run_tape([((f.grad_to or (f.x,))[0], _G(d, H, W)) for f, d in zip((f1, f2, f3), df)], None)

    def _head_coef_ok(self, f):
        readers = 0
        for Rt in self.tape:
            if isinstance(Rt, runtime.FuseRecord):
                if any(t.x is f.x for t in Rt.terms):
                    return False
                continue
            for sx in Rt.srcs:
                if sx.res is f.x or (sx.x is f.x and (sx.pool or tuple(sx.off) != (0, 0))):
                    return False
                readers += sx.x is f.x
        P = next((Rt for Rt in self.tape if not isinstance(Rt, runtime.FuseRecord) and Rt.out is f.x), None)
        owner = None if P is None or P.layer.kind != 'conv1' else P.fused_res_of
        return readers <= 2 and owner is not None and owner.layer.bn is not None and owner.relu == 2 and owner.res is f.x \
            and owner.out.dtype == torch.float32 and tuple(owner.out.shape) == tuple(f.x.shape)

    def _head_fusable(self, f1, f2, f3):
        if not HEAD_BWD_FUSE or runtime.PRECISION != 'fp32' or getattr(self.model, 'VARIANT', None) != 'rev1':
            return None
        for f in (f1, f2, f3):
            if f.x.dtype != torch.float32 or f.scale is not None or f.shift is not None or f.res is not None or f.relu or f.pool \
                    or f.grad_to is not None or tuple(f.off) != (0, 0) or f.C != 64:
                return None
        owner = None
        for Rt in self.tape:
            if isinstance(Rt, runtime.FuseRecord):
                if any(t.x is f3.x for t in Rt.terms):
                    return None
                continue
            if any(sx.x is f3.x or sx.res is f3.x for sx in Rt.srcs):
                return None
            if Rt.out is f3.x:
                owner = Rt.fused_res_of if Rt.layer.kind == 'conv1' else None
        if owner is None or owner.layer.bn is None or owner.relu != 2 or owner.res is not f3.x \
                or owner.out.dtype != torch.float32 or tuple(owner.out.shape) != tuple(f3.x.shape):
            return None
        return owner

    def _classifier_backward(self, key, f, conv, dl):
        N, H, W, _ = f.x.shape
        K = conv.out_channels
        df = self.buf(key, (N, H, W, 64), runtime.act_dtype())
        ws = self._ws('slab', _lib.load().cdnet_final_conv1x1_backward_workspace_floats(), side=True)
        hf = runtime.head_feat(f)
        w = conv.weight.detach().reshape(K, 64)
        _lib.call('cdnet_final_conv1x1_backward', C.byref(hf), _lib.ptr(w), _lib.ptr(dl), K, N, H, W, _lib.ptr(df), _lib.ptr(ws),
                  ws.numel(), _lib.ptr(conv.weight.grad), _lib.ptr(conv.bias.grad), _lib.stream_ptr())
        return _G(df, H, W)

    def _run_tape(self, heads, params):
        grads = {}

        def add(t, g):
            grads.setdefault(id(t), []).append(g)
        for t, g in heads:
            add(t, g)
        self._overlap_begin()
        self._overlap_done(params)
        self._backward_tape(grads, add)

    def _backward_tape(self, grads, add):
        self._cat_cache = {}
        self._rd_pending, self._rd_params, self._rd_bytes = [], [], 0
        if len(self._rd_tables) > 16:
            self._rd_tables.clear()
        self._readers, self._producer, self._bn_partials = {}, {}, {}
        self._tape_pos = {Rt: k for k, Rt in enumerate(self.tape)}
        for Rt in self.tape:
            if isinstance(Rt, runtime.FuseRecord):
                for t in Rt.terms:
                    self._readers[id(t.x)] = self._readers.get(id(t.x), 0) + 1
                continue
            for sx in Rt.srcs:
                self._readers[id(sx.x)] = self._readers.get(id(sx.x), 0) + 1
                if sx.res is not None:
                    self._readers[id(sx.res)] = self._readers.get(id(sx.res), 0) + 1
            self._producer[id(Rt.out)] = Rt
        self._nograd = self._no_grad_outputs()
        side = self._side_stream()
        self._side_active = side is not None
        if self._packb_pending:
            torch.cuda.current_stream().wait_event(self._event('packb'))
            self._packb_pending = False
        for k, R in enumerate(reversed(self.tape)):
            if isinstance(R, runtime.FuseRecord):
                self._fuse_backward(R, grads, add)
                continue
            gl = self.take(grads, id(R.out))
            if gl is None:
                continue
            owner = R.fused_res_of
            if owner is not None:
                grads.setdefault(id(owner.out), []).extend(gl)
                owner.deferred = R
                continue
            self._layer_backward(k, R, gl, grads, add, side)
            d = R.deferred
            if d is not None:
                R.deferred = None
                self._layer_backward(('deferred', k), d, self.take(grads, id(d.out)), grads, add, side)
        if side is not None:
            with _on_stream(side):
                self._flush_reduces()
            ev = self._event(-1)
            ev.record(side)
            torch.cuda.current_stream().wait_event(ev)
        else:
            self._flush_reduces()

    def _no_grad_outputs(self):
        dead = set()
        if not self._frozen_ids:
            return dead
        fr = self._frozen_ids
        for Rt in self.tape:
            if isinstance(Rt, runtime.FuseRecord):
                continue
            L = Rt.layer
            ps = (L.weight, L.bias, None if L.bn is None else L.bn.weight, None if L.bn is None else L.bn.bias)
            if all(p is None or id(p) in fr for p in ps) and \
                    all(sx.res is None and (sx.is_input or id((sx.grad_to or (sx.x,))[0]) in dead) for sx in Rt.srcs):
                dead.add(id(Rt.out))
        return dead

    def _fuse_backward(self, R, grads, add):
        terms, o, relu, H, W, Cc, coff, name = R.terms, R.out, R.relu, R.H, R.W, R.C, R.coff, R.node.name
        sliced = o.shape[3] != Cc
        if sliced:
            d, dcs, dco = self.cat_grad(o, grads), o.shape[3], coff
            if d is None:
                return
        else:
            gl = self.take(grads, id(o))
            if gl is None:
                return
            if relu and self._residual_tail(grads, gl, terms, o, H, W, Cc):
                return
            if relu or len(gl) > 1 or gl[0].coff or gl[0].cstride not in (0, Cc):
                d = self.buf(('dfuse', name), o.shape, o.dtype)
                self.grad_sum(gl, o if relu else None, o.shape[0] * H * W, Cc, d)
            else:
                d = gl[0].t
            dcs, dco = 0, 0
        N = o.shape[0]
        for k, t in enumerate(terms):
            if t.Hs == H and t.Ws == W:
                add(t.x, _G(d, H, W, coff=dco, cstride=dcs))
            else:
                din = self.buf(('dup', name, k), (N, t.Hs, t.Ws, Cc), d.dtype)
                _lib.call(_lib.entry('cdnet_upsample_bilinear_backward', d.dtype == torch.float32), _lib.ptr(d),
                          N, H, W, Cc, dcs, dco, t.Hs, t.Ws, _lib.ptr(din), _lib.stream_ptr())
                add(t.x, _G(din, t.Hs, t.Ws))

    def _residual_tail(self, grads, gl, terms, o, H, W, Cc):
        if runtime.DEBUG_NORELU:
            return False
        if len(terms) == 1:
            y = terms[0]
            P = self._producer.get(id(y.x)) if y.scale is not None else None
            if P is None or P.layer.bn is None or P.res is not None or self._readers.get(id(y.x), 0) != 1 or id(y.x) in grads \
                    or tuple(y.x.shape) != tuple(o.shape) or P.fused_res_of is not None or (y.Hs, y.Ws) != (H, W):
                return False
            P.relu, P.res = True, None
            grads[id(y.x)] = gl
            return True
        if len(terms) != 2 or len(gl) > 3:
            return False
        bn_t = [t for t in terms if t.scale is not None]
        if not bn_t or any((t.Hs, t.Ws) != (H, W) for t in terms):
            return False
        y = max(bn_t, key=lambda t: self._tape_pos.get(self._producer.get(id(t.x)), -1))
        x = terms[1] if terms[0] is y else terms[0]
        P = self._producer.get(id(y.x))
        if P is None or P.layer.bn is None or P.res is not None or self._readers.get(id(y.x), 0) != 1 or id(y.x) in grads \
                or tuple(y.x.shape) != tuple(o.shape) or P.fused_res_of is not None:
            return False
        if any(g.pooled or g.oy or g.ox or (g.Hg, g.Wg) != (H, W) for g in gl):
            return False
        P.relu, P.res, P.res_grad_to = 2, o, x.x
        grads[id(y.x)] = gl
        return True

    def _weights_done(self, params):
        if not self._rd_pending:
            self._overlap_done(params)
            return
        self._rd_params.append(params)
        if self._rd_bytes >= self._rd_mb * (1 << 20):
            self._flush_reduces()

    def _flush_reduces(self):
        if self._rd_pending:
            key = tuple(self._rd_pending)
            tab = self._rd_tables.get(key)
            if tab is None:
                lib = _lib.load()
                descs = (_lib.WgradReduceDesc * len(key))()
                b0 = 0
                for i, a in enumerate(key):
                    _lib.call('cdnet_wgrad_reduce_desc_fill', *a, b0, C.byref(descs[i]))
                    b0 += descs[i].blocks
                dev_tab = torch.frombuffer(bytearray(bytes(descs)), dtype=torch.uint8).to(self.dev)
                tab = self._rd_tables[key] = (dev_tab, len(key), b0)
            _lib.call('cdnet_wgrad_reduce_batch', _lib.ptr(tab[0]), tab[1], tab[2], _lib.stream_ptr())
        for params in self._rd_params:
            self._overlap_done(params)
        self._rd_pending, self._rd_params, self._rd_bytes = [], [], 0

    def _layer_backward(self, k, R, gl, grads, add, side):
        L, srcs, out, Hl, Wl = R.layer, R.srcs, R.out, R.H, R.W
        No, Ho, Wo, Co = out.shape
        params = (L.weight, L.bias, None if L.bn is None else L.bn.weight, None if L.bn is None else L.bn.bias)
        part = self._bn_partials.pop(id(out), None)
        if len(gl) == 1 and gl[0].masked:
            g = self._bn_backward_masked(R, out, gl[0], add)
        elif part is not None:
            assert len(gl) == 1, (L.name, len(gl))
            a, ktab = self._bn_backward_stats(L, out, gl[0], partial=part)
            g = self.buf(('draw', L.name), (No, Ho, Wo, Co), runtime.act_dtype())
            _lib.call('cdnet_bn_backward_apply', C.byref(a), _lib.ptr(ktab), _lib.ptr(g), _lib.stream_ptr())
        elif L.bn is not None or len(gl) > 1 or gl[0].pooled or gl[0].coff or (gl[0].cstride not in (0, Co)):
            g = self._bn_backward(R, out, gl, add)
        else:
            g = gl[0].t
        if side is None:
            self._weight_backward(L, srcs, g, Hl, Wl)
            self._weights_done(params)
            self._input_backward(L, srcs, g, Hl, Wl, add)
        else:
            ev = self._event(k)
            ev.record()
            beside = _RU_1X1_SIDE and L.kind == 'conv1' and isinstance(k, tuple) and L.needs_input_grad
            if not beside:
                self._input_backward(L, srcs, g, Hl, Wl, add)
            side.wait_event(ev)
            with _on_stream(side):
                if beside:
                    ev2 = self._event(('beside', k))

                    def add_beside(tgt, g_):
                        g_.event = ev2
                        add(tgt, g_)
                    self._input_backward(L, srcs, g, Hl, Wl, add_beside)
                    ev2.record()
                self._weight_backward(L, srcs, g, Hl, Wl)
                self._weights_done(params)

    def _bn_backward_stats(self, L, out, g, partial):
        a = self._bn_args(L, out, [_G(g.t, g.Hg, g.Wg)], res=None, relu=1)
        ktab = self.buf(('ktab', L.name), (7, out.shape[3]), torch.float32)
        bn = L.bn
        _lib.call('cdnet_bn_backward_finalize', C.byref(a), _lib.ptr(bn.weight.detach()), _lib.ptr(bn.weight.grad), _lib.ptr(bn.bias.grad),
                  _lib.ptr(partial), partial.shape[0], _lib.ptr(ktab), _lib.stream_ptr())
        return a, ktab

    def _bn_backward_masked(self, R, out, g, add):
        L = R.layer
        No, Ho, Wo, Co = out.shape
        a = self._bn_args(L, out, [_G(g.t, g.Hg, g.Wg)], res=None, relu=0)
        draw = self.buf(('draw', L.name), (No, Ho, Wo, Co), runtime.act_dtype())
        ws = self._ws('bn', _lib.load().cdnet_bn_backward_workspace_floats(Co))
        bn = L.bn
        _lib.call('cdnet_bn_backward', C.byref(a), _lib.ptr(bn.weight.detach()), _lib.ptr(bn.weight.grad), _lib.ptr(bn.bias.grad),
                  _lib.ptr(ws), ws.numel(), _lib.ptr(draw), None, _lib.stream_ptr())
        add(R.res, _G(g.t, Ho, Wo))
        return draw

    def _stats_fusable(self, L, srcs, H, W, N, wpb, cfgb, cin_total):
        f32 = runtime.PRECISION == 'fp32'
        if not f32 or os.environ.get('CDNET_BN_STATS_FUSE', '1') != '1' or runtime.DEBUG_NORELU:
            return None
        if L.kind != 'conv3' or L.transposed or len(srcs) != 1:
            return None
        sx = srcs[0]
        if sx.is_input or sx.scale is None or sx.shift is None or sx.relu is not True or sx.res is not None or sx.pool \
                or tuple(sx.off) != (0, 0) or sx.x.dtype != runtime.raw_dtype() or sx.grad_to is not None or sx.row_stride:
            return None
        if f32 and cin_total % 64:
            return None
        PR = self._producer.get(id(sx.x))
        if PR is None or PR.layer.bn is None or PR.res is not None or PR.relu is not True \
                or self._readers.get(id(sx.x), 0) != 1 or tuple(sx.x.shape) != (N, H, W, cin_total):
            return None
        P = PR.layer
        key = ('statsfusable', L.name, N, H, W, runtime.PRECISION)
        hit = self._bufs.get(key)
        if hit is None:
            part = torch.zeros((1024, 2, cin_total), dtype=torch.float32, device=self.dev)
            gin = self.buf(('din', L.name), (N, H, W, cin_total), runtime.act_dtype())
            gdummy = self.buf(('draw', L.name), (N, H, W, L.Cout), runtime.act_dtype())
            ok = engine.conv_forward([Src(gdummy)], wpb, cin_total, cfgb, taps=L.taps, out=gin, H=H, W=W, query_ws=True,
                                     bns=(sx.x, P.scale, P.shift, P.save_mean, P.save_invstd, part))
            hit = self._bufs[key] = (part if ok else False)
        if hit is False:
            return None
        return P, hit

    def _bn_args(self, L, out, gl, res, relu):
        a = BnBwdArgs()
        a.raw = out.data_ptr()
        a.res = None if res is None else res.data_ptr()
        if L.bn is not None:
            a.scale, a.shift = L.scale.data_ptr(), L.shift.data_ptr()
            a.mean, a.invstd = L.save_mean.data_ptr(), L.save_invstd.data_ptr()
        a.ngin = len(gl)
        assert 1 <= len(gl) <= 3, (L.name, len(gl))
        for k, g in enumerate(gl):
            if g.hc is not None:
                coef, hw, w0, k0, nk = g.hc
                a.hc_coef, a.hc_w, a.hc_slot, a.hc_k0, a.hc_nk = coef.data_ptr(), hw.data_ptr() + 4 * w0, k, k0, nk
            a.gin[k].g = None if g.t is None else g.t.data_ptr()
            a.gin[k].Hg, a.gin[k].Wg, a.gin[k].oy, a.gin[k].ox = g.Hg, g.Wg, g.oy, g.ox
            a.gin[k].pooled, a.gin[k].coff, a.gin[k].cstride = int(g.pooled), g.coff, g.cstride or out.shape[3]
        a.f16 = {torch.bfloat16: 0, torch.float16: 1, torch.float32: 2}[out.dtype]
        a.relu = relu
        a.N, a.H, a.W, a.C = out.shape
        return a

    def _bn_backward(self, R, out, gl, add):
        L = R.layer
        No, Ho, Wo, Co = out.shape
        res = R.res
        has_bn = L.bn is not None
        if len(gl) > 3:
            plain = [g for g in gl if not g.pooled and g.oy == 0 and g.ox == 0 and (g.Hg, g.Wg) == (Ho, Wo)]
            rest = [g for g in gl if g not in plain]
            assert len(rest) <= 2 and len(plain) >= 2, (L.name, len(gl))
            d = self.buf(('gsum', L.name), (No, Ho, Wo, Co), runtime.act_dtype())
            self.grad_sum(plain, None, No * Ho * Wo, Co, d)
            gl = rest + [_G(d, Ho, Wo)]
        a = self._bn_args(L, out, gl, res, int(R.relu))
        draw = self.buf(('draw', L.name), (No, Ho, Wo, Co), runtime.act_dtype())
        dz = None
        if res is not None:
            dz = self.buf(('dz', L.name), (No, Ho, Wo, Co), runtime.act_dtype())
        ws = self._ws('bn', _lib.load().cdnet_bn_backward_workspace_floats(Co))
        bn = L.bn
        _lib.call('cdnet_bn_backward', C.byref(a), _lib.ptr(bn.weight.detach()) if has_bn else None,
                  _lib.ptr(bn.weight.grad) if has_bn else None, _lib.ptr(bn.bias.grad) if has_bn else None,
                  _lib.ptr(ws), ws.numel(), _lib.ptr(draw), _lib.ptr(dz), _lib.stream_ptr())
        if res is not None:
            add(R.res_grad_to if R.res_grad_to is not None else res, _G(dz, Ho, Wo))
            R.res_grad_to = None
        return draw

    def _side_stream(self):
        if not WGRAD_STREAM or self.dev.type != 'cuda':
            return None
        if self._wstream is None:
            self._wstream = streams.side_stream(self.dev)
            self._events = {}
        return self._wstream

    def _event(self, k):
        e = self._events.get(k)
        if e is None:
            e = self._events[k] = torch.cuda.Event()
        return e

    def _weight_backward(self, L, srcs, g, H, W):
        lib = _lib.load()
        N = g.shape[0]
        Cout = L.Cout
        cin_total = sum(s.C for s in srcs)
        cin_real = L.Cin
        mode = {'conv3': 0, 'conv1': 0, 'convT4': 2, 'convT2': 3, 'conv3s2': 6}[L.kind]
        taps, npar, ostride = L.taps, (4 if L.transposed else 1), (2 if L.transposed else 1)
        cap = _wgrad_wgs(self._side_active and L.needs_input_grad, H * W, Cout)
        coff = 0
        for s in srcs:
            ci_t = _choose_ci_tiles(s.C, Cout)
            CI, CO = ci_t * 32, (4 // ci_t) * 32
            other = -(-s.C // CI) * -(-Cout // CO) * npar
            ntiles = N * (-(-H // 8)) * (-(-W // 16))
            ksplit = max(1, min(ntiles, cap // other if other < cap else 1))
            nslab = lib.cdnet_conv_wgrad_slab_floats(s.C, Cout, taps, npar, ci_t, ksplit)
            defer = self._rd_mb > 0
            slab = self.buf(('wslab', L.name, coff), (nslab,), torch.float32) if defer else self._ws('slab', nslab, side=True)
            cs = engine.ConvSrc()
            s.fill(cs)
            csrc_real = min(s.C, cin_real - coff) if cin_total != cin_real else s.C
            _lib.call('cdnet_conv_backward_weight', C.byref(cs), coff, csrc_real, cin_real, _lib.ptr(g), Cout, N, H, W, taps,
                      npar, ostride, ci_t, ksplit, _lib.ptr(slab), _lib.ptr(L.weight.grad), mode | (_WGRAD_DEFER if defer else 0),
                      _lib.stream_ptr())
            if defer:
                self._rd_pending.append((s.C, coff, csrc_real, cin_real, Cout, taps, npar, ci_t, ksplit, slab.data_ptr(),
                                         L.weight.grad.data_ptr(), mode))
                self._rd_bytes += nslab * 4
            coff += s.C
        if L.bias is not None and L.bn is None:
            owner = L.bias_grad_from
            if owner is not None:
                L.bias.grad.copy_(owner.bn.bias.grad)
            else:
                ws = self._ws('slab', lib.cdnet_bias_grad_workspace_floats(Cout), side=True)
                _lib.call(_lib.entry('cdnet_bias_grad', g.dtype == torch.float32), _lib.ptr(g), g.numel() // Cout, Cout,
                          _lib.ptr(ws), ws.numel(), _lib.ptr(L.bias.grad), _lib.stream_ptr())

    def _narrow_ok(self, L, g, wpb, cfgb, gin, H, W, c_live):
        key = ('narrow', L.name, tuple(g.shape), c_live, runtime.PRECISION, engine.CONV_DEBUG)
        ok = self._bufs.get(key)
        if ok is None:
            q = [engine.conv_forward([Src(g)], wpb, c, cfgb, taps=L.taps, out=gin, H=H, W=W, query_ws=True) for c in (gin.shape[3], c_live)]
            ok = self._bufs[key] = c_live % 8 == 0 and q[0] == q[1]
            self.narrowed[L.name] = c_live if ok else None
        return ok

    def _input_backward(self, L, srcs, g, H, W, add):
        if not L.needs_input_grad:
            return
        N = g.N if isinstance(g, Src) else g.shape[0]
        Cout = L.Cout
        cin_total = sum(s.C for s in srcs)
        dead = [id((s.grad_to or (s.x,))[0]) in self._nograd for s in srcs] if self._nograd else [False] * len(srcs)
        if all(dead):
            return
        wpb, cfgb = L.backward_pack(cin_total, H, W)
        if L.kind == 'conv3s2':
            Cp = cin_total // 4
            gs2d = self.buf(('ds2d', L.name), (N, H, W, cin_total), runtime.act_dtype())
            engine.conv_forward([Src(g)], wpb, cin_total, cfgb, taps=9, out=gs2d, H=H, W=W)
            gin = self.buf(('din', L.name), (N, 2 * H, 2 * W, Cp), runtime.act_dtype())
            _lib.call(_lib.entry('cdnet_s2d_to_nhwc', gin.dtype == torch.float32), _lib.ptr(gs2d), N, H, W, Cp, _lib.ptr(gin),
                      _lib.stream_ptr())
            add(srcs[0].x, _G(gin, 2 * H, 2 * W))
            return
        if not L.transposed:
            gin = self.buf(('din', L.name), (N, H, W, cin_total), runtime.act_dtype())
            fuse = None if isinstance(g, Src) else self._stats_fusable(L, srcs, H, W, N, wpb, cfgb, cin_total)
            if fuse is not None:
                P, part = fuse
                engine.conv_forward([Src(g)], wpb, cin_total, cfgb, taps=L.taps, out=gin, H=H, W=W,
                                    bns=(srcs[0].x, P.scale, P.shift, P.save_mean, P.save_invstd, part))
                self._bn_partials[id(srcs[0].x)] = part
            else:
                c_live = srcs[0].C if dead == [False, True] and not isinstance(g, Src) and self._narrow_ok(L, g, wpb, cfgb, gin, H, W, srcs[0].C) \
                    else cin_total
                engine.conv_forward([g if isinstance(g, Src) else Src(g)], wpb, c_live, cfgb, taps=L.taps, out=gin, H=H, W=W)
        else:
            gin = self.buf(('din', L.name), (N, H, W, cin_total), runtime.act_dtype())
            views = [Src(g, view=(a * 2 * W * Cout, H, W, 2 * Cout, 4 * W * Cout)) for a in (0, 1)]
            engine.conv_forward(views, wpb, cin_total, cfgb, taps=(9 if L.kind == 'convT4' else 1), out=gin, H=H, W=W)
        coff = 0
        for s, dead_s in zip(srcs, dead):
            if s.is_input or dead_s:
                coff += s.C
                continue
            tgt, pool = s.grad_to or (s.x, int(s.pool))
            add(tgt, _G(gin, H, W, oy=s.off[0], ox=s.off[1], pooled=pool, coff=coff, cstride=cin_total))
            coff += s.C

    def _overlap_begin(self):
        self._ar = None
        if not self._reduce_active() or os.environ.get('CDNET_ALLREDUCE_OVERLAP', '1') == '0':
            return
        f = self.flat
        base = f.G.data_ptr()
        pend = {}
        owners = [p for L in (R.layer for R in self.tape if not isinstance(R, runtime.FuseRecord)) for p in (L.weight, L.bias, None if L.bn is None else L.bn.weight,
                                                 None if L.bn is None else L.bn.bias) if p is not None]
        for p in owners:
            off = (p.grad.data_ptr() - base) // 4
            if 0 <= off < f.n_used:
                pend[off] = off + p.numel()
        if f.n_head:
            pend[0] = f.n_head
        self._ar = BucketReducer(f.G, f.n_used, self.bucket, pend)

    def _overlap_done(self, params):
        if self._ar is None:
            return
        if params is None:
            self._ar.done([0])
        else:
            base = self.flat.G.data_ptr()
            self._ar.done([(p.grad.data_ptr() - base) // 4 for p in params if p is not None])

    def _reduce_active(self):
        return self.world > 1 or os.environ.get('CDNET_FORCE_ALLREDUCE', '0') == '1'

    def allreduce_and_step(self):
        f = self.flat
        gscale = 1.0
        works = None
        if self._reduce_active():
            if self._ar is not None:
                ranges = self._ar.finish(wait=False)
                works = self._ar.works
                self.ar_stats = dict(buckets=len(works), released_during_backward=self._ar.early)
                self._ar = None
            else:
                bucketed_allreduce(f.G, f.n_used, self.bucket)
            gscale = 1.0 / self.world
        f.step_count += 1
        step = self._rule_stepper(gscale)
        if works is None:
            step(0, f.n_used)
        else:
            for w, (a, b) in zip(works, ranges):
                w.wait()
                step(a, b)
        runtime.WEIGHTS_EPOCH[0] += 1
        self._repack_all()

    def _rule_stepper(self, gscale):
        return optim.stepper(self, gscale)

    def _repack_all(self):
        f = self.flat
        lo, hi = f.P.data_ptr(), f.P.data_ptr() + f.P.numel() * 4
        if self._pack_jobs is not None and self._pack_prec != runtime.PRECISION:
            self._pack_jobs = None
        if self._pack_jobs is None:
            groups = ([], []), ([], [])
            for L in runtime.LAYERS:
                if not (lo <= L.weight.data_ptr() < hi):
                    continue
                w = L.weight.detach()
                if L.wp is not None and not L.wp_padded:
                    groups[0][0].append(engine.pack_job(w, L.cfg, L.pack_mode, L.wp, split=L.cfg_f32)); groups[0][1].append((L, 'wp_version'))
                if L.wpb is not None:
                    mode = (4 if L.kind == 'convT4' else 5) if L.transposed else (7 if L.kind == 'conv3s2' else 1)
                    groups[1][0].append(engine.pack_job(w, L.cfg_bwd, mode, L.wpb, split=L.cfg_f32)); groups[1][1].append((L, 'wpb_version'))
            if not groups[0][0] or not groups[1][0] or self.flat.step_count < 1:
                return
            self._pack_jobs = []
            self._pack_prec = runtime.PRECISION
            for jobs, owners in groups:
                arr = (engine.PackJob * len(jobs))(*jobs)
                nbytes = _lib.load().cdnet_pack_batch_table_bytes(len(jobs))
                table = torch.empty((nbytes,), dtype=torch.uint8, device=f.P.device)
                self._pack_jobs.append((arr, len(jobs), table, owners, [True]))
        side = self._side_stream()
        for k, (arr, n, table, owners, first) in enumerate(self._pack_jobs):
            if k == 1 and side is not None and self._packb_stream:
                ev = self._event('adam')
                ev.record()
                side.wait_event(ev)
                with _on_stream(side):
                    _lib.call('cdnet_pack_conv_weights_batch', C.byref(arr), n, _lib.ptr(table), table.numel(), int(first[0]), _lib.stream_ptr())
                    self._event('packb').record()
                self._packb_pending = True
            else:
                _lib.call('cdnet_pack_conv_weights_batch', C.byref(arr), n, _lib.ptr(table), table.numel(), int(first[0]), _lib.stream_ptr())
            first[0] = False
            for L, attr in owners:
                setattr(L, attr, (L.weight._version, runtime.WEIGHTS_EPOCH[0]))

    def write_bn_counters(self):
        with torch.no_grad():
            unused = tuple(getattr(self.model, 'UNUSED_PREFIXES', ()))
            for name, mod in self.model.named_modules():
                if isinstance(mod, torch.nn.BatchNorm2d) and mod.num_batches_tracked is not None and not (name + '.').startswith(unused or ('\0',)):
                    mod.num_batches_tracked.fill_(self._bn_base + self._forwards)

    def refresh_parameters(self):
        if hasattr(self.model, 'sync_real_parameters') and getattr(self.model, '_rt', None) is not None:
            self.model._ensure_runtime()
        runtime.WEIGHTS_EPOCH[0] += 1

    def state_dict(self):
        return optim.state_dict(self)

    def load_state_dict(self, sd):
        optim.load_state_dict(self, sd)

    def train_step(self, x, label, dirlab, point_t, weight):
        mask, point, direction = self.forward(x)
        dmask, dpoint, ddir = self.loss_and_grads(mask, point, direction, label, dirlab, point_t, weight)
        self.backward(dmask, dpoint, ddir)
        self.allreduce_and_step()
        return self.losses


class UNetTrainer(Trainer):

    def __init__(self, model, **kw):
        super().__init__(model, **kw)
        self.mask_losses = torch.zeros((8,), dtype=torch.float32, device=self.dev)
        self.unet_losses = self.mask_losses[0:3]
        self.unet_metrics = self.mask_losses[3:8]

    def mask_loss(self, logits, label, weight, terms, dmask):
        B, K, H, W = logits.shape
        if K != 3:
            raise ValueError('the mask loss serves the 3-class configuration (options.py: out_c = 3), got %d classes' % K)
        assert label.dtype == torch.uint8 and (weight is None or weight.dtype == torch.uint8)
        ws = self._ws('mask_loss', _lib.load().cdnet_mask_loss_workspace_floats(B, H * W))
        _lib.call('cdnet_mask_loss', _lib.ptr(logits), _lib.ptr(label.contiguous()), None if weight is None else _lib.ptr(weight.contiguous()),
                  B, H, W, terms, _lib.ptr(ws), ws.numel(), _lib.ptr(self.mask_losses), None if dmask is None else _lib.ptr(dmask),
                  _lib.stream_ptr())

    def loss_and_grads(self, logits, label, weight):
        from .utils import loss_terms
        terms = loss_terms(self.dice, self.weight_map, self.alpha)
        dmask = self.buf('dmask', logits.shape, torch.float32)
        self.mask_loss(logits, label, weight, terms, dmask)
        total = self.mask_losses[0:1]
        if self.dice == 2:
            if self.alpha:
                self._variance_term(logits, label, None)
            return dmask
        if self.alpha:
            self._variance_term(logits, label, dmask, total)
        if self.boundary:
            self._boundary_term(logits, label, dmask, total)
        return dmask

    def backward(self, dlogits):
        conv, feat = self.model.final_conv, self.model._last_feat
        self._run_tape([(feat.x, self._classifier_backward('dF', feat, conv, dlogits))], [conv.weight, conv.bias])

    def train_step(self, x, label, weight):
        logits = self.forward(x)
        dlogits = self.loss_and_grads(logits, label, weight)
        self.backward(dlogits)
        self.allreduce_and_step()
        return self.unet_losses


class BackboneUNetTrainer(UNetTrainer):

    def _classifier_backward(self, key, f, conv, dl):
        N, H, W, _ = f.x.shape
        K = conv.out_channels
        df = self.buf(key, (N, H, W, 16), runtime.act_dtype())
        ws = self._ws('classifier16', _lib.load().cdnet_final_conv1x1_c16_backward_workspace_floats())
        hf = runtime.head_feat16(f)
        w = conv.weight.detach().reshape(K, 16)
        _lib.call('cdnet_final_conv1x1_c16_backward', C.byref(hf), _lib.ptr(w), _lib.ptr(dl), K, N, H, W, _lib.ptr(df), _lib.ptr(ws),
                  ws.numel(), _lib.ptr(conv.weight.grad), _lib.ptr(conv.bias.grad), _lib.stream_ptr())
        return _G(df, H, W)


class FullNetTrainer(UNetTrainer):

    def __init__(self, model, seed=0, **kw):
        if runtime.PRECISION != 'fp32':
            raise NotImplementedError('FullNet trains in the fp32 precision mode only (CDNET_PRECISION=fp32 / runtime.set_precision("fp32")); '
                                      'bf16-mode training is not built')
        super().__init__(model, **kw)
        self.seed = int(seed)

    def dropout_key(self):
        return ((self.seed & 0xffffffff) << 32) | (self.flat.step_count & 0xffffffff)

    def forward(self, x):
        self.model._train_key = self.dropout_key()
        return super().forward(x)

    def backward(self, dlogits):
        self._ar = None
        self.model.train_backward(self.tape[-1], dlogits)


class AblationTrainer(Trainer):

    def __init__(self, model, **kw):
        assert getattr(model, 'VARIANT', 'rev1') in ('MandD', 'MandDandP') and model.DIRECTION_OUT in (5, 9, 17), \
            'AblationTrainer serves model_unet_MandD / MandD4 / MandD16 / MandDandP'
        super().__init__(model, **kw)

    def loss_and_grads(self, outputs, label, dirlab, point_t, weight):
        if len(outputs) == 3:
            return super().loss_and_grads(outputs[0], outputs[1], outputs[2], label, dirlab, point_t, weight)
        mask, direction = outputs
        B, _, H, W = mask.shape
        point = self.buf('zero_point', (B, 1, H, W), torch.float32)
        pt = self.buf('zero_point_t', (B, H, W), torch.float16)
        point.zero_()
        pt.zero_()
        dmask, _, ddir = super().loss_and_grads(mask, point, direction, label, dirlab, pt, weight)
        return dmask, None, ddir

    def backward(self, dmask, dpoint, ddir):
        m = self.model
        f1m, f2, f3 = m._last_feats
        heads, params = [], []
        for name, f, conv, dl in (('m', f1m, m.mask_conv, dmask), ('d', f2, m.direction_conv, ddir), ('p', f3, m.point_conv, dpoint)):
            if f is None or dl is None:
                continue
            heads.append(((f.grad_to or (f.x,))[0], self._classifier_backward('dF' + name, f, conv, dl)))
            params += [conv.weight, conv.bias]
        self._run_tape(heads, params)

    def train_step(self, x, label, dirlab, point_t, weight):
        out = self.forward(x)
        g = self.loss_and_grads(out, label, dirlab, point_t, weight)
        self.backward(*g)
        self.allreduce_and_step()
        return self.losses


def make_bench_step(model, B, dev, rank, world):
    tr = Trainer(model, world_size=world)
    batch = synthetic_batch(B, dev, seed=2022 + rank)

    def step():
        return tr.train_step(*batch)
    metric = 'tiles/sec (train fwd+bwd+Adam), 256x256'
    workload = ('CDNet UNet2RevA1_vgg16 (UNet+DAM) training step: forward, 5-term loss, backward%s, %s fused Adam; '
                '256x256x3 synthetic tiles, batch %d per GPU' % ('', 'RCCL gradient all-reduce,' if world > 1 else '', B))
    return step, metric, workload
```

include/cdnet_hip.h:

```cpp
#ifndef CDNET_HIP_H
#define CDNET_HIP_H

#include <stddef.h>
#include <stdint.h>

#ifdef __cplusplus
extern "C" {
#endif

#define CDNET_OK            0
#define CDNET_E_ARG         1
#define CDNET_E_WORKSPACE   2
#define CDNET_E_LAUNCH      3

#define CDNET_ABI_VERSION   5

int         cdnet_abi_version(void);
size_t      cdnet_abi_sizeof(const char *struct_name);
const char *cdnet_last_error(void);
const char *cdnet_build_info(void);
int         cdnet_spin(int microseconds, void *stream);
int         cdnet_box_copy(const void *src, void *dst, size_t bytes, void *stream);
int         cdnet_box_mfma(const uint32_t *seed, float *sink, unsigned long long *stamps, int workgroups, int waves_per_wg, int iters, void *stream);

size_t cdnet_tile_postproc_workspace_bytes(int B, int C, int H, int W);
int cdnet_tile_postproc(const float *mask_logits, const float *dir_logits, const float *point, int B, int C, int H, int W,
                        const int8_t *lut_host, int nbr, int extra_zero, int min_area, int radius, void *workspace, size_t workspace_bytes,
                        float *prob, uint8_t *dcm, int32_t *minmax, uint8_t *pred, uint8_t *fill, uint8_t *small, int32_t *label,
                        int32_t *final_, int32_t *counts, void *stream);

int cdnet_ddm_codes(const uint8_t *dcm, int N, int H, int W, int classes, const int8_t *lut_host, int nbr,
                    int extra_zero, uint8_t *code, int32_t *minmax, void *stream);
int cdnet_ddm_normalize(const uint8_t *code, const int32_t *minmax, int N, int H, int W, float *out,
                        void *stream);

int cdnet_probmaps(const float *mask_logits, const float *dir_logits, int N, int C, int H, int W,
                   float *prob, uint8_t *dcm, void *stream);

int cdnet_tta_boost_argmax(const float *probs, const float *points, const uint8_t *codes, const int32_t *minmax,
                           int I, int V, const int *view_xform_host, int H, int W,
                           float *prob_mean, float *point_mean, uint8_t *ddm16, uint8_t *pred,
                           float *pmax_ws, void *stream);

size_t cdnet_watershed_workspace_bytes(int N, int H, int W);
int cdnet_watershed_process(const uint8_t *pred, int N, int H, int W, int min_size, void *workspace, size_t workspace_bytes,
                            uint8_t *dist, int32_t *marker, int32_t *labels, void *stream);
int cdnet_fill_label_process(const uint8_t *pred, int N, int H, int W, int min_size, void *workspace, size_t workspace_bytes,
                             int32_t *labels, void *stream);
int cdnet_label_process(const uint8_t *pred, int N, int H, int W, int min_size, void *workspace, size_t workspace_bytes,
                        int32_t *labels, void *stream);

size_t cdnet_instance_redilate_workspace_bytes(int N, int H, int W, int cap);
int cdnet_instance_redilate(const int32_t *label, int N, int H, int W, int r, int cap, void *workspace, size_t workspace_bytes,
                            int32_t *out, int32_t *err_flag, void *stream);
int cdnet_instance_redilate_lds_rows(void);
int cdnet_instance_redilate_lds_cols(void);
int cdnet_label_count(const int32_t *lab, int N, int plane, int cap, int32_t *seen, int32_t *counts, int32_t *err_flag, void *stream);

size_t cdnet_cc_workspace_bytes(int N, int H, int W);
int cdnet_cc_chain(const uint8_t *pred, int fg_value, int N, int H, int W, int min_area, int radius,
                   void *workspace, size_t workspace_bytes,
                   uint8_t *fill, uint8_t *small, int32_t *label, int32_t *final_, int32_t *counts,
                   void *stream);

int cdnet_mask_views_argmax(const float *logits, int I, int V, int K, const int *view_xform_host, int H, int W, float *prob_mean,
                            uint8_t *pred, void *stream);
size_t cdnet_tile_mask_postproc_workspace_bytes(int B, int K, int H, int W);
int cdnet_tile_mask_postproc(const float *logits, int B, int K, int H, int W, int min_area, int radius, void *workspace, size_t workspace_bytes,
                             float *prob, uint8_t *pred, uint8_t *fill, uint8_t *small, int32_t *label, int32_t *final_, int32_t *counts,
                             void *stream);
int cdnet_dilate_labels(const int32_t *label, int N, int H, int W, int radius, int32_t *out, void *stream);


typedef struct cdnet_conv_src {
    const uint16_t *x;
    const uint16_t *res;
    const float *scale;
    const float *shift;
    int C;
    int Hs, Ws;
    int pool;
    int relu;
    int off_y, off_x;
    int f16;
    int row_stride;
} cdnet_conv_src;

typedef struct cdnet_conv_args {
    cdnet_conv_src src[2];
    int nsrc;
    const uint16_t *w;
    const float *bias;
    const float *oscale;
    const float *oshift;
    int orelu;
    uint16_t *out;
    int Cout, out_cstride, out_coff;
    float *stats;
    int N, H, W;
    int taps;
    int npar;
    int ostride;
    int nchunk;
    int tile, CK, BN;
    int out_f16;
    int debug;
    int ws;
    int f32;
    const uint16_t *eres;
    const float *eres_scale, *eres_shift;
    int eres_f16, eres_relu;
    int taps1;
    int pad_;
    uint16_t *pool_out;
    const float *dot_w;
    const float *dot_b;
    float *dot_out;
} cdnet_conv_args;

size_t cdnet_conv_packed_weight_elems(int Cout, int nchunk, int taps, int CK, int BN, int npar);
#define CDNET_PACK_SPLIT 16
int cdnet_pack_conv_weights(const float *w, void *packed, int Cout, int Cin, int KH, int KW, int CK, int BN, int mode,
                            void *stream);
int cdnet_pack_conv_weights_scaled(const float *w, const float *cout_scale, void *packed, int Cout, int Cin, int KH, int KW, int CK,
                                   int BN, int mode, void *stream);
typedef struct cdnet_pack_job {
    const float *w;
    void *packed;
    int Cout, Cin, KH, KW, CK, BN, mode, pad_;
} cdnet_pack_job;
size_t cdnet_pack_batch_table_bytes(int n_jobs);
int cdnet_pack_conv_weights_batch(const cdnet_pack_job *jobs, int n_jobs, void *table, size_t table_bytes, int upload,
                                  void *stream);
int cdnet_conv_forward(const cdnet_conv_args *args, void *stream);

#define CDNET_CONV_FAMILY_FWD    1
#define CDNET_CONV_FAMILY_WS     2
#define CDNET_CONV_FAMILY_WS16   3
#define CDNET_CONV_FAMILY_F32    4
#define CDNET_CONV_FAMILY_STREAM 5
#define CDNET_CONV_FAMILY_WS32   6
int cdnet_conv_forward_last_form(void);

typedef struct cdnet_dilated_conv_args {
    const void *in;
    const void *w;
    const float *scale;
    const float *shift;
    void *out;
    int N, H, W;
    int Cin, in_cstride;
    int Cout, out_cstride, out_coff;
    int taps, dilation;
    int leaky;
    float slope;
    int f32, out_nchw;
} cdnet_dilated_conv_args;
size_t cdnet_dilated_packed_weight_elems(int Cin, int Cout, int taps, int f32);
int cdnet_dilated_pack_weights(const float *w, void *packed, int Cin, int Cout, int taps, int f32, void *stream);
int cdnet_dilated_conv_forward(const cdnet_dilated_conv_args *args, void *stream);


typedef struct cdnet_dilated_bwd_data_args {
    const void *g;
    const void *w;
    void *dx;
    int N, H, W;
    int Cout, g_cstride;
    int Cin, dx_cstride, dx_coff;
    int taps, dilation;
    int accumulate;
    int f32;
} cdnet_dilated_bwd_data_args;
int cdnet_dilated_pack_weights_bwd(const float *w, void *packed, int Cin, int Cout, int taps, int f32, void *stream);
int cdnet_dilated_conv_backward_data(const cdnet_dilated_bwd_data_args *args, void *stream);

typedef struct cdnet_dilated_wgrad_args {
    const float *x;
    const float *g;
    float *dw;
    void *ws;
    size_t ws_bytes;
    int N, H, W;
    int Cin, x_cstride;
    int Cout, g_cstride;
    int taps, dilation;
} cdnet_dilated_wgrad_args;
size_t cdnet_dilated_wgrad_workspace_bytes(int N, int H, int W, int Cin, int Cout, int taps);
int cdnet_dilated_conv_backward_weight(const cdnet_dilated_wgrad_args *args, void *stream);

typedef struct cdnet_slice_bn_fwd_args {
    const float *z;
    float *out;
    const float *gamma, *beta;
    float *running_mean, *running_var;
    float *mean, *invstd;
    float *ws;
    size_t ws_floats;
    long long P;
    int C, z_cstride, out_cstride, out_coff;
    float eps, momentum, p_drop;
    int layer;
    unsigned long long key;
} cdnet_slice_bn_fwd_args;
typedef struct cdnet_slice_bn_bwd_args {
    const float *dy;
    const float *z;
    const float *mean, *invstd, *gamma;
    float *dgamma, *dbeta;
    float *g;
    float *ws;
    size_t ws_floats;
    long long P;
    int C, z_cstride, dy_cstride, dy_coff, g_cstride;
    float slope, p_drop;
    int layer;
    unsigned long long key;
} cdnet_slice_bn_bwd_args;
size_t cdnet_slice_bn_workspace_floats(long long P, int C);
int cdnet_slice_bn_train_forward(const cdnet_slice_bn_fwd_args *args, void *stream);
int cdnet_slice_bn_train_backward(const cdnet_slice_bn_bwd_args *args, void *stream);
int cdnet_dropout_mask(unsigned long long key, int layer, size_t count, float p_drop, uint8_t *mask, void *stream);


int cdnet_maxpool2_forward(const void *x, int x_cstride, void *y, int y_cstride, int y_coff, uint8_t *idx, int idx_cstride, int N, int H, int W,
                           int C, int f32, void *stream);
int cdnet_maxpool2_backward(const float *dy, int dy_cstride, int dy_coff, const uint8_t *idx, int idx_cstride, float *dx, int dx_cstride, int N,
                            int H, int W, int C, void *stream);
int cdnet_upsample4_bilinear_forward(const void *x, int x_cstride, void *y, int y_cstride, int y_coff, int N, int Hs, int Ws, int C, int f32,
                                     void *stream);
int cdnet_upsample4_bilinear_backward(const float *dy, int dy_cstride, int dy_coff, float *dx, int dx_cstride, int N, int Hs, int Ws, int C,
                                      void *stream);

int cdnet_input_pack(const float *x, int N, int C, int H, int W, void *out_bf16_nhwc16, void *stream);
int cdnet_input_pack_f32(const float *x, int N, int C, int H, int W, float *out_f32_nhwc16, void *stream);
int cdnet_bn_fold_eval(const float *gamma, const float *beta, const float *running_mean, const float *running_var,
                       const float *conv_bias, float eps, int C, float *scale, float *shift, void *stream);
int cdnet_bn_finalize_train(const float *stats, int T, int C, float count, const float *gamma, const float *beta,
                            const float *conv_bias, float eps, float momentum, float *running_mean,
                            float *running_var, float *scale, float *shift, float *save_mean, float *save_invstd,
                            void *stream);

typedef struct cdnet_head_feat {
    const uint16_t *raw;
    const uint16_t *res;
    const float *scale;
    const float *shift;
    int relu;
    int f16;
} cdnet_head_feat;

#define CDNET_HEAD_WEIGHT_FLOATS 855
int cdnet_dam_head_forward(const cdnet_head_feat *f1, const cdnet_head_feat *f2, const cdnet_head_feat *f3,
                           const float *head_weights, int N, int H, int W, float *mask, float *point,
                           float *direction, void *stream);
int cdnet_final_conv1x1(const cdnet_head_feat *f, const float *w, const float *b, int K, int N, int H, int W,
                        float *out, void *stream);
size_t cdnet_bias_grad_workspace_floats(int C);
int cdnet_bias_grad(const uint16_t *grad_out, size_t npix, int C, float *workspace, size_t workspace_floats, float *db, void *stream);
int cdnet_bias_grad_f32(const float *grad_out, size_t npix, int C, float *workspace, size_t workspace_floats, float *db, void *stream);
size_t cdnet_final_conv1x1_backward_workspace_floats(void);
int cdnet_final_conv1x1_backward(const cdnet_head_feat *f, const float *w, const float *dlogits, int K, int N, int H, int W,
                                 uint16_t *df, float *workspace, size_t workspace_floats, float *dw, float *db, void *stream);
int cdnet_final_conv1x1_c16(const cdnet_head_feat *f, const float *w, const float *b, int K, int N, int H, int W,
                            float *out, void *stream);
size_t cdnet_final_conv1x1_c16_backward_workspace_floats(void);
int cdnet_final_conv1x1_c16_backward(const cdnet_head_feat *f, const float *w, const float *dlogits, int K, int N, int H, int W,
                                     void *df, float *workspace, size_t workspace_floats, float *dw, float *db, void *stream);

int cdnet_conv_ws_eligible(const cdnet_conv_args *args);

int cdnet_src_materialize(const cdnet_conv_src *src, int N, int H, int W, uint16_t *out, void *stream);

size_t cdnet_conv_wgrad_slab_floats(int C_src, int Cout, int taps, int npar, int ci_tiles, int ksplit);
int cdnet_conv_backward_weight(const cdnet_conv_src *src, int src_coff, int Csrc_real, int Cin_real,
                               const uint16_t *grad_out, int Cout, int N, int H, int W, int taps, int npar,
                               int ostride, int ci_tiles, int ksplit, float *slab, float *dw, int mode, void *stream);

#define CDNET_WGRAD_FAMILY_GEN  1
#define CDNET_WGRAD_FAMILY_WS   2
#define CDNET_WGRAD_FAMILY_F32  3
#define CDNET_WGRAD_FAMILY_WS32 4
int cdnet_conv_backward_weight_last_form(void);

#define CDNET_WGRAD_DEFER_REDUCE 0x100
typedef struct cdnet_wgrad_reduce_desc {
    const float *slab;
    float *dw;
    int ksplit, npar, ci_blocks, co_blocks, taps, CI, CO, Csrc_real, Cin_real, src_coff, Cout, mode;
    int block0, blocks;
} cdnet_wgrad_reduce_desc;
int cdnet_wgrad_reduce_desc_fill(int C_src, int src_coff, int Csrc_real, int Cin_real, int Cout, int taps, int npar, int ci_tiles,
                                 int ksplit, const float *slab, float *dw, int mode, int block0, cdnet_wgrad_reduce_desc *out);
int cdnet_wgrad_reduce_batch(const cdnet_wgrad_reduce_desc *table_dev, int n, int total_blocks, void *stream);

typedef struct cdnet_grad_in {
    const uint16_t *g;
    int Hg, Wg;
    int oy, ox;
    int pooled;
    int coff, cstride;
    int pad_;
} cdnet_grad_in;

typedef struct cdnet_bn_bwd_args {
    const uint16_t *raw;
    const uint16_t *res;
    const float *scale, *shift;
    const float *mean, *invstd;
    cdnet_grad_in gin[3];
    int ngin;
    int f16, relu;
    int N, H, W, C;
    const float *hc_coef, *hc_w;
    int hc_slot, hc_k0, hc_nk, hc_pad_;
} cdnet_bn_bwd_args;

size_t cdnet_bn_backward_workspace_floats(int C);
int cdnet_bn_backward_stats(const cdnet_bn_bwd_args *args, const float *gamma, float *dgamma, float *dbeta, float *workspace,
                            size_t workspace_floats, float *ktab, void *stream);
int cdnet_bn_backward_apply(const cdnet_bn_bwd_args *args, const float *ktab, uint16_t *draw, void *stream);
int cdnet_bn_backward_finalize(const cdnet_bn_bwd_args *args, const float *gamma, float *dgamma, float *dbeta, const float *partial,
                               int nb, float *ktab, void *stream);
int cdnet_bn_backward(const cdnet_bn_bwd_args *args, const float *gamma, float *dgamma, float *dbeta, float *workspace,
                      size_t workspace_floats, uint16_t *draw, uint16_t *dz_out, void *stream);

#define CDNET_BN_PATH_WINDOW  1
#define CDNET_BN_PATH_FLAT    2
#define CDNET_BN_PATH_GENERIC 3
int cdnet_bn_backward_last_plan(void);
int cdnet_bn_backward_last_sums_plan(void);

size_t cdnet_dam_head_backward_workspace_floats(int N, int H, int W);
int cdnet_dam_head_backward(const cdnet_head_feat *f1, const cdnet_head_feat *f2, const cdnet_head_feat *f3,
                            const float *head_weights, const float *dmask, const float *dpoint, const float *ddir,
                            int N, int H, int W, uint16_t *df1, uint16_t *df2, uint16_t *df3, float *workspace,
                            size_t workspace_floats, float *dhead_weights, void *stream);
int cdnet_dam_head_backward_fused_blocks(void);
int cdnet_dam_head_backward_fused_scratch_bytes(void);
size_t cdnet_dam_head_backward_fused_workspace_floats(void);
int cdnet_dam_head_backward_fused(const cdnet_head_feat *f1, const cdnet_head_feat *f2, const cdnet_head_feat *f3,
                                  const float *head_weights, const float *dmask, const float *dpoint, const float *ddir, int N, int H,
                                  int W, float *df1, float *df2, float *dz3, float *workspace, size_t workspace_floats,
                                  float *dhead_weights, void *stream);
int cdnet_dam_head_backward_coef_scratch_bytes(void);
int cdnet_dam_head_backward_coef(const cdnet_head_feat *f1, const cdnet_head_feat *f2, const cdnet_head_feat *f3,
                                 const float *head_weights, const float *dmask, const float *dpoint, const float *ddir, int N, int H,
                                 int W, float *coef, float *dz3, float *workspace, size_t workspace_floats, float *dhead_weights,
                                 void *stream);

size_t cdnet_dam_loss_workspace_floats(int B, int P);
int cdnet_dam_loss(const float *mask, const float *point, const float *direction, const uint8_t *label,
                   const uint8_t *dirlab, const uint16_t *point_target_f16, const uint8_t *weight_u8, int B, int H, int W,
                   int quirk_sample0, float *workspace, size_t workspace_floats, float *losses, float *dmask,
                   float *dpoint, float *ddir, void *stream);
size_t cdnet_dam_loss_classes_workspace_floats(int B, int P, int direction_classes);
int cdnet_dam_loss_classes(const float *mask, const float *point, const float *direction, const uint8_t *label,
                           const uint8_t *dirlab, const uint16_t *point_target_f16, const uint8_t *weight_u8, int B, int H, int W,
                           int direction_classes, int quirk_sample0, float *workspace, size_t workspace_floats, float *losses,
                           float *dmask, float *dpoint, float *ddir, void *stream);

#define CDNET_LOSS_WMAP 1u
#define CDNET_LOSS_CE   2u
#define CDNET_LOSS_DICE 4u

int cdnet_dam_loss_terms(const float *mask, const float *point, const float *direction, const uint8_t *label,
                         const uint8_t *dirlab, const uint16_t *point_target_f16, const uint8_t *weight_u8, int B, int H, int W,
                         int direction_classes, int quirk_sample0, float *workspace, size_t workspace_floats, float *losses,
                         float *dmask, float *dpoint, float *ddir, void *stream, unsigned terms);

size_t cdnet_mask_loss_workspace_floats(int B, int P);
int cdnet_mask_loss(const float *mask_logits, const uint8_t *label, const uint8_t *weight_u8, int B, int H, int W, unsigned terms,
                    float *workspace, size_t workspace_floats, float *losses, float *dmask, void *stream);

size_t cdnet_variance_loss_workspace_bytes(int B, int K, int H, int W);
int cdnet_variance_loss(const float *mask_logits, const uint8_t *label, int fg_value, int B, int K, int H, int W, float alpha,
                        void *workspace, size_t workspace_bytes, float *loss_var, float *total, float *dmask, int32_t *root_out,
                        int32_t *counts, void *stream);

size_t cdnet_boundary_loss_workspace_bytes(int kind, int B, int K, int H, int W);
int cdnet_boundary_loss(const float *mask_logits, const uint8_t *label, int kind, int B, int K, int H, int W, float beta,
                        void *workspace, size_t workspace_bytes, float *loss_out, float *total, float *dmask, void *stream);
int cdnet_boundary_loss_scratch_bytes(void);

#define CDNET_VAL_SUMS 42
size_t cdnet_dam_val_sums_workspace_floats(int B, int P);
int cdnet_dam_val_sums(const float *mask, const float *point, const float *dirn, const uint8_t *label, const uint8_t *dirlab,
                       const uint16_t *point_target_f16, const uint8_t *weight_u8, const int *dir_rank_host, int B, int H, int W,
                       float *workspace, size_t workspace_floats, float *sums, void *stream);
size_t cdnet_dam_val_sums_classes_workspace_floats(int B, int P, int direction_classes);
int cdnet_dam_val_sums_classes(const float *mask, const float *point, const float *dirn, const uint8_t *label, const uint8_t *dirlab,
                               const uint16_t *point_target_f16, const uint8_t *weight_u8, const int *dir_rank_host,
                               int direction_classes, int B, int H, int W, float *workspace, size_t workspace_floats, float *sums,
                               void *stream);

int cdnet_adam_step(float *param, const float *grad, float *exp_avg, float *exp_avg_sq, size_t n, float lr, float beta1,
                    float beta2, float eps, float weight_decay, int step, float grad_scale, void *stream);

int cdnet_moment_step(float *param, const float *grad, float *exp_avg, float *exp_avg_sq, float *slow, size_t n, double beta1,
                      double beta2, float grad_scale, int move, int rect, float decay, float step_size, float v_div, float eps,
                      int sync, float alpha, void *stream);
int cdnet_sgd_step(float *param, const float *grad, float *momentum_buffer, size_t n, float lr, float momentum, float weight_decay,
                   int step, float grad_scale, void *stream);

int cdnet_window_pack(const float *img, int C, int H, int W, int view_xform, int tile_h, int tile_w, int stride, int ny,
                      int nx, void *out_bf16_nhwc16, void *stream);
int cdnet_window_pack_f32(const float *img, int C, int H, int W, int view_xform, int tile_h, int tile_w, int stride, int ny,
                          int nx, float *out_f32_nhwc16, void *stream);
int cdnet_window_stitch(const float *tiles, int K, int tile_h, int tile_w, int stride, int overlap, int ny, int nx, int Hv,
                        int Wv, float *out, void *stream);

typedef struct cdnet_aug_sample {
    double minv[6];
    const uint8_t *img;
    const uint8_t *weight;
    const void *label;
    int32_t H, W, img_stride, weight_stride, label_stride, label_i32;
    float color[4];
    int32_t hflip, vflip, filter, y0, x0;
    float alpha, sigma;
    uint32_t seed;
} cdnet_aug_sample;
size_t cdnet_augment_workspace_bytes(int B, int size, int max_radius);
int cdnet_augment_batch(const cdnet_aug_sample *samples, const cdnet_aug_sample *samples_host, int B, int size, const float *norm_host,
                        void *workspace, size_t workspace_bytes, float *image, uint8_t *weight, void *label, int label_i32, int32_t *varied,
                        float *field, void *stream);

typedef struct cdnet_aug_geo {
    double paff[6];
    double rinv[6];
    int32_t Hr, Wr, fy0, fx0;
    uint32_t flags;
    int32_t reserved;
} cdnet_aug_geo;
size_t cdnet_augment_geo_workspace_bytes(int B, int size, int max_radius, int field_edge);
int cdnet_augment_batch_geo(const cdnet_aug_sample *samples, const cdnet_aug_sample *samples_host, const cdnet_aug_geo *geo,
                            const cdnet_aug_geo *geo_host, int field_edge, int B, int size, const float *norm_host, void *workspace,
                            size_t workspace_bytes, float *image, uint8_t *weight, void *label, int label_i32, int32_t *varied, float *field,
                            void *stream);

size_t cdnet_label_encoding_workspace_bytes(int N, int H, int W, int max_instances);
int cdnet_label_encoding(const uint8_t *label_ch0, int N, int H, int W, int max_instances, const double *rays_host,
                         const double *gauss_host, void *workspace, size_t workspace_bytes, uint8_t *label3,
                         uint16_t *point_f16, uint8_t *direction, int32_t *inst_out, int32_t *counts_out, void *stream);
size_t cdnet_label_encoding_instances_workspace_bytes(int N, int H, int W, int max_instances);
int cdnet_label_encoding_instances(const int32_t *label_inst, int N, int H, int W, int max_instances, const double *rays_host,
                                   const double *gauss_host, void *workspace, size_t workspace_bytes, uint8_t *label3,
                                   uint16_t *point_f16, uint8_t *direction, int32_t *inst, int32_t *counts, void *stream);

typedef struct cdnet_fuse_term {
    const uint16_t *x;
    int Hs, Ws;
    const float *scale;
    const float *shift;
    int f16, pad_;
} cdnet_fuse_term;
int cdnet_fuse_sum(const cdnet_fuse_term *terms, int nterm, int N, int H, int W, int C, int relu, uint16_t *out, int out_cstride,
                   int out_coff, void *stream);

int cdnet_upsample_bilinear_backward(const uint16_t *dout, int N, int H, int W, int C, int dout_cstride, int dout_coff, int Hs, int Ws,
                                     uint16_t *din, void *stream);
int cdnet_s2d_to_nhwc(const uint16_t *in, int N, int H2, int W2, int C, uint16_t *out, void *stream);
int cdnet_fuse_sum_f32(const cdnet_fuse_term *terms, int nterm, int N, int H, int W, int C, int relu, float *out, int out_cstride,
                       int out_coff, void *stream);
int cdnet_upsample_bilinear_backward_f32(const float *dout, int N, int H, int W, int C, int dout_cstride, int dout_coff, int Hs, int Ws,
                                         float *din, void *stream);
int cdnet_s2d_to_nhwc_f32(const float *in, int N, int H2, int W2, int C, float *out, void *stream);

typedef struct cdnet_grad_term {
    const uint16_t *g;
    int cstride, coff;
} cdnet_grad_term;
int cdnet_grad_sum(const cdnet_grad_term *terms, int nterm, const uint16_t *mask, long long npix, int C, uint16_t *out, void *stream);
int cdnet_grad_sum_f32(const cdnet_grad_term *terms, int nterm, const float *mask, long long npix, int C, float *out, void *stream);

int cdnet_label_pair_histogram(const int32_t *true_lab, const int32_t *pred_lab, int N, int plane, int cap, int hash_slots,
                               int32_t *area_true, int32_t *area_pred, uint32_t *hash_keys, int32_t *hash_counts, int32_t *err_flag,
                               void *stream);
int cdnet_remap_label(const int32_t *lab, int N, int plane, int cap, int32_t *scratch, int32_t *out, int32_t *err_flag, void *stream);
int cdnet_label_areas(const int32_t *lab, int N, int plane, int cap, int32_t *area, int32_t *err_flag, void *stream);
int cdnet_label_apply(const int32_t *lab, int N, int plane, int cap, const int32_t *lut, int32_t *out, void *stream);

size_t cdnet_label_csr_workspace_bytes(int cap);
int cdnet_label_csr(const int32_t *lab, int H, int W, int cap, void *workspace, size_t workspace_bytes, int32_t *tab, int32_t *pix,
                    int32_t *bpix, int32_t *err_flag, void *stream);
int cdnet_hausdorff_tile_pixels(void);
int cdnet_hausdorff_chunk_pixels(void);
int cdnet_hausdorff_pairs(const int32_t *true_lab, const int32_t *true_tab, const int32_t *true_pix, const int32_t *true_bpix,
                          const int32_t *pred_lab, const int32_t *pred_tab, const int32_t *pred_pix, const int32_t *pred_bpix, int H, int W,
                          int cap, const int32_t *pairs, int M, const int32_t *items, int n_items, int32_t *d2, int32_t *err_flag,
                          void *stream);

int cdnet_weight_map_radius(double w0, double sigma);
int cdnet_weight_map(const int32_t *instances, int H, int W, double w0, double sigma, uint8_t *weight, void *stream);

size_t cdnet_resize_workspace_bytes(int N, int H, int W, int C, int oh, int ow, int form);
int cdnet_resize_bilinear(const uint8_t *src, int N, int H, int W, int C, int oh, int ow, const int32_t *hbounds, const int32_t *hkk,
                          int hksize, const int32_t *vbounds, const int32_t *vkk, int vksize, int mask_mode, int form, void *workspace,
                          size_t workspace_bytes, uint8_t *out, void *stream);
int cdnet_resize_last_form(void);
int cdnet_fill_remove_small(const uint8_t *pred, int fg_value, int N, int H, int W, int min_area, void *workspace, size_t workspace_bytes,
                            uint8_t *small, void *stream);
int cdnet_label8_dilate(const uint8_t *mask, int N, int H, int W, int radius, void *workspace, size_t workspace_bytes, int32_t *label,
                        int32_t *final_, int32_t *counts, void *stream);

#ifdef __cplusplus
}
#endif
#endif
```

Measured before the change: 1097.

## Add fp32 transposed-conv kernels that run only live taps per parity

Moves the shared fp32 conv staging, stats and store code into a reusable header and adds a new convt32 source with two kernels. One computes stride-2 transposed conv forward as a quad of 4-tap parity sub-convolutions. The other computes the convT4 backward data gradient by running only the 4 of 9 taps that are non-zero for each source chunk. The backward path is on by default through an environment flag. This cuts MFMA work and LDS reads for these layers, at the cost of added kernel variants and routing heuristics based on CU count.

```diff
diff --git a/cdnet_amd/_lib.py b/cdnet_amd/_lib.py
--- a/cdnet_amd/_lib.py
+++ b/cdnet_amd/_lib.py
@@ -21,7 +21,7 @@
                 ('ostride', C.c_int), ('nchunk', C.c_int), ('tile', C.c_int), ('CK', C.c_int), ('BN', C.c_int),
                 ('out_f16', C.c_int), ('debug', C.c_int), ('ws', C.c_int), ('f32', C.c_int),
                 ('eres', C.c_void_p), ('eres_scale', C.c_void_p), ('eres_shift', C.c_void_p), ('eres_f16', C.c_int), ('eres_relu', C.c_int),
-                ('taps1', C.c_int), ('pad_', C.c_int), ('pool_out', C.c_void_p),
+                ('taps1', C.c_int), ('live_taps', C.c_int), ('pool_out', C.c_void_p),
                 ('dot_w', C.c_void_p), ('dot_b', C.c_void_p), ('dot_out', C.c_void_p)]
 
 
diff --git a/cdnet_amd/csrc/build.py b/cdnet_amd/csrc/build.py
--- a/cdnet_amd/csrc/build.py
+++ b/cdnet_amd/csrc/build.py
@@ -6,7 +6,7 @@
 PKG = os.path.dirname(HERE)
 LIB = os.path.join(PKG, 'libcdnet_hip.so')
 OBJ_DIR = os.path.join(HERE, 'build')
-SOURCES = ['abi.hip', 'box.hip', 'postproc.hip', 'postproc_tile.hip', 'conv.hip', 'conv_ws.hip', 'pack.hip', 'conv32.hip', 'conv32ws.hip', 'conv16ws.hip', 'dilated.hip', 'dilated_train.hip', 'resample.hip', 'wgrad.hip', 'model.hip', 'head_bwd.hip', 'classifier16.hip', 'dam_loss.hip', 'bn_bwd.hip', 'cdm.hip', 'metrics.hip', 'augment.hip', 'optim.hip', 'variance.hip', 'boundary.hip', 'mask_loss.hip', 'weight_map.hip', 'instance_fill.hip', 'resize.hip']
+SOURCES = ['abi.hip', 'box.hip', 'postproc.hip', 'postproc_tile.hip', 'conv.hip', 'conv_ws.hip', 'pack.hip', 'conv32.hip', 'convt32.hip', 'conv32ws.hip', 'conv16ws.hip', 'dilated.hip', 'dilated_train.hip', 'resample.hip', 'wgrad.hip', 'model.hip', 'head_bwd.hip', 'classifier16.hip', 'dam_loss.hip', 'bn_bwd.hip', 'cdm.hip', 'metrics.hip', 'augment.hip', 'optim.hip', 'variance.hip', 'boundary.hip', 'mask_loss.hip', 'weight_map.hip', 'instance_fill.hip', 'resize.hip']
 FLAGS = ['--offload-arch=gfx950', '-O3', '-std=c++20', '-fPIC', '-ffp-contract=off', '-Wall',
          '-Wno-unused-function', '-Wno-unused-result']
 
diff --git a/cdnet_amd/csrc/conv32.hip b/cdnet_amd/csrc/conv32.hip
--- a/cdnet_amd/csrc/conv32.hip
+++ b/cdnet_amd/csrc/conv32.hip
@@ -2,265 +2,45 @@
 #include "common.h"
 #include "conv_args.h"
 #include "launch.h"
-#include "split_bf16.h"
+#include "conv32_tile.h"
 #include <stdlib.h>
 
 using namespace cdnet;
+using namespace cdnet::conv32;
 
 namespace {
-
-constexpr int CK = 16;
-constexpr int PSTR = CK * 2 + 16;
-constexpr int XF_MAX = 2048;
-
-template <int TH, int TW, int BN, int TAPS>
-struct Lds32 {
-    static constexpr int NPIX = (TH + 2) * (TW + 2);
-    static constexpr int A_PLANE = NPIX * PSTR;
-    static constexpr int B_PLANE = TAPS * CK * BN * 2;
-    static constexpr int STAGE = 2 * A_PLANE + 2 * B_PLANE;
-    static constexpr int STATS_BYTES = 4 * 2 * BN * 4;
-    static constexpr int MAIN = ((STAGE > STATS_BYTES ? STAGE : STATS_BYTES) + 15) / 16 * 16;
-    static int bytes(int ctot) { return MAIN + 2 * ((ctot + 7) / 8 * 8) * 4; }
-};
-
-
-template <int MPW, int NPW, int TW>
-__device__ __forceinline__ void store_tile_f32(const ConvArgs &A, const f32x16 (&acc)[MPW][NPW], int n, int y0, int x0, int mblock0, int nblock0,
-                                               int half, int l31, int cout0, int pa_, int pb_) {
-    const int Ho = A.H * A.ostride, Wo = A.W * A.ostride;
-    float *out = reinterpret_cast<float *>(A.out);
-    const float *eres = reinterpret_cast<const float *>(A.eres);
-    const bool full = y0 + 16 <= A.H && x0 + TW <= A.W && cout0 + (nblock0 + NPW) * 32 <= A.Cout && A.ostride == 1 && TW == 16 &&
-                      !(A.debug & 16);
-    if (full) {
-        const int cs = A.out_cstride, ce = A.Cout;
-        float *tb = out + (((size_t)n * A.H + y0) * A.W + x0) * cs + A.out_coff;
-        const float *te = eres ? eres + (((size_t)n * A.H + y0) * A.W + x0) * ce : nullptr;
-#pragma unroll
-        for (int ni = 0; ni < NPW; ++ni) {
-            const int co = cout0 + (nblock0 + ni) * 32 + l31;
-            const float osc = A.oscale ? A.oscale[co] : 1.f;
-            const float osh = fmaf(A.bias ? A.bias[co] : 0.f, osc, A.oshift ? A.oshift[co] : 0.f);
-            const float esc = (eres && A.eres_scale) ? A.eres_scale[co] : 1.f;
-            const float esh = (eres && A.eres_shift) ? A.eres_shift[co] : 0.f;
-            float *ob = tb + co;
-#pragma unroll
-            for (int mi = 0; mi < MPW; ++mi) {
-                const int rowb = ((mblock0 + mi) * 2) * A.W + 4 * half;
-                float ev[16];
-                if (eres) {
-#pragma unroll
-                    for (int r = 0; r < 16; ++r) {
-                        const int p = (r & 3) + 8 * (r >> 2);
-                        ev[r] = te[(rowb + (p / 16) * A.W + (p % 16)) * ce + co];
-                    }
-                }
-#pragma unroll
-                for (int r = 0; r < 16; ++r) {
-                    const int p = (r & 3) + 8 * (r >> 2);
-                    const int off = (rowb + (p / 16) * A.W + (p % 16)) * cs;
-                    float v = fmaf(acc[mi][ni][r], osc, osh);
-                    if (A.orelu) v = fmaxf(v, 0.f);
-                    if (eres) {
-                        v = fmaf(ev[r], esc, esh) + v;
-                        if (A.eres_relu) v = fmaxf(v, 0.f);
-                    }
-                    ob[off] = v;
-                }
-            }
-        }
-        return;
-    }
-#pragma unroll
-    for (int ni = 0; ni < NPW; ++ni) {
-        const int co = cout0 + (nblock0 + ni) * 32 + l31;
-        const bool cok = co < A.Cout;
-        const float osc = (A.oscale && cok) ? A.oscale[co] : 1.f;
-        const float osh = fmaf((A.bias && cok) ? A.bias[co] : 0.f, osc, (A.oshift && cok) ? A.oshift[co] : 0.f);
-        const float esc = (A.eres && A.eres_scale && cok) ? A.eres_scale[co] : 1.f;
-        const float esh = (A.eres && A.eres_shift && cok) ? A.eres_shift[co] : 0.f;
-#pragma unroll
-        for (int mi = 0; mi < MPW; ++mi) {
-            float ev[16];
-            if (A.eres) {
-#pragma unroll
-                for (int r = 0; r < 16; ++r) {
-                    const int m = (mblock0 + mi) * 32 + (r & 3) + 8 * (r >> 2) + 4 * half;
-                    int y = y0 + m / TW, x = x0 + m % TW;
-                    y = y < A.H ? y : A.H - 1; x = x < A.W ? x : A.W - 1;
-                    ev[r] = eres[(((size_t)n * A.H + y) * A.W + x) * A.Cout + (cok ? co : 0)];
-                }
-            }
-#pragma unroll
-            for (int r = 0; r < 16; ++r) {
-                const int m = (mblock0 + mi) * 32 + (r & 3) + 8 * (r >> 2) + 4 * half;
-                const int y = y0 + m / TW, x = x0 + m % TW;
-                float v = fmaf(acc[mi][ni][r], osc, osh);
-                if (A.orelu) v = fmaxf(v, 0.f);
-                if (A.eres) {
-                    v = fmaf(ev[r], esc, esh) + v;
-                    if (A.eres_relu) v = fmaxf(v, 0.f);
-                }
-                if (cok && y < A.H && x < A.W) {
-                    const size_t opix = ((size_t)n * Ho + (y * A.ostride + pa_)) * Wo + (x * A.ostride + pb_);
-                    out[opix * A.out_cstride + A.out_coff + co] = v;
-                }
-            }
-        }
-    }
-}
 
 template <int TH, int TW, int BN, int WM, int WN, int TAPS>
 __global__ __launch_bounds__(256, 2) void conv_f32_kernel(ConvArgs A) {
     using L = Lds32<TH, TW, BN, TAPS>;
-    constexpr int HW_ = TW + 2, NPIX = L::NPIX;
+    using Stage = Stage32<TH, TW, 2 * L::B_PLANE / 16>;
+    constexpr int HW_ = TW + 2;
     constexpr int MT = TH * TW / 32, NT = BN / 32;
     constexpr int MPW = MT / WM, NPW = NT / WN;
-    constexpr int VPP = CK / 8;
-    constexpr int NA = (NPIX * VPP + 255) / 256;
-    constexpr int NBV = 2 * L::B_PLANE / 16;
-    constexpr int NB = (NBV + 255) / 256;
     static_assert(MT % WM == 0 && NT % WN == 0 && WM * WN == 4, "wave tiling");
 
     extern __shared__ __attribute__((aligned(16))) unsigned char smem[];
     unsigned char *lds_a = smem;
     unsigned char *lds_b = smem + 2 * L::A_PLANE;
     float (*s_stats)[2][BN] = reinterpret_cast<float (*)[2][BN]>(smem);
-    float *s_xf = reinterpret_cast<float *>(smem + L::MAIN);
 
     const int tid = threadIdx.x, lane = tid & 63, wave = tid >> 6;
     const int wm = wave / WN, wn = wave % WN;
     const int half = lane >> 5, l31 = lane & 31;
-    const int c0n = A.src[0].C, ctot = c0n + (A.nsrc > 1 ? A.src[1].C : 0);
-    const int xfs = (ctot + 7) / 8 * 8;
-    for (int c = tid; c < ctot; c += 256) {
-        const ConvSrc &S = c < c0n ? A.src[0] : A.src[1];
-        const int cc = c < c0n ? c : c - c0n;
-        s_xf[c] = S.scale ? S.scale[cc] : 1.f;
-        s_xf[xfs + c] = S.shift ? S.shift[cc] : 0.f;
-    }
+    Stage S;
+    S.init(A, reinterpret_cast<float *>(smem + L::MAIN), tid);
 
     const int tiles_x = (A.W + TW - 1) / TW, tiles_y = (A.H + TH - 1) / TH;
     const int tiles_img = tiles_x * tiles_y;
     int tile, cout_tile;
-    {
-        const int NC = (int)gridDim.y, lin = (int)blockIdx.y * (int)gridDim.x + (int)blockIdx.x;
-        const int T = (int)gridDim.x * NC, q = T >> 3, rem = T & 7;
-        const int xcd = lin & 7, idx = lin >> 3;
-        const int seq = xcd < rem ? xcd * (q + 1) + idx : rem * (q + 1) + (xcd - rem) * q + idx;
-        tile = seq / NC;
-        cout_tile = seq - tile * NC;
-    }
+    xcd_tile_order(tile, cout_tile);
     const int z = tile / tiles_img, rt = tile - z * tiles_img;
     const int n = z / A.npar, par = z - n * A.npar;
     const int ty_ = rt / tiles_x;
     const int y0 = ty_ * TH, x0 = (rt - ty_ * tiles_x) * TW;
-
-    int eoff[2][NA];
-    const int slot = tid % VPP;
-#pragma unroll
-    for (int si = 0; si < 2; ++si) {
-        if (si >= A.nsrc) break;
-        const ConvSrc &s = A.src[si];
-        const int rs = s.row_stride ? s.row_stride : s.Ws * s.C;
-#pragma unroll
-        for (int i = 0; i < NA; ++i) {
-            const int v = tid + i * 256;
-            const int pix = v / VPP;
-            const int hy = pix / HW_, hx = pix - hy * HW_;
-            const int y = y0 - 1 + hy, x = x0 - 1 + hx;
-            const int ys = y - s.off_y, xs = x - s.off_x;
-            const bool ok = v < NPIX * VPP && (unsigned)y < (unsigned)A.H && (unsigned)x < (unsigned)A.W && (unsigned)ys < (unsigned)s.Hs &&
-                            (unsigned)xs < (unsigned)s.Ws;
-            eoff[si][i] = ok ? ys * rs + xs * s.C + slot * 8 : -1;
-        }
-    }
-    auto chunk_src = [&](int c, int &si, int &cc0) {
-        const int n0 = A.src[0].C / CK;
-        if (c < n0) { si = 0; cc0 = c * CK; } else { si = 1; cc0 = (c - n0) * CK; }
-    };
+    typename Stage::Eoff eoff;
+    S.geometry(A, eoff, n, y0, x0);
     const unsigned short *wbase = A.w + ((size_t)(par * gridDim.y + cout_tile) * A.nchunk) * (size_t)(L::B_PLANE);
-
-    f32x4 pa[NA][2];
-    u32x4 pb[NB];
-    auto issue = [&](int chunk) {
-        int si, cc0;
-        chunk_src(chunk, si, cc0);
-        const ConvSrc &s = A.src[si];
-        const size_t rs = s.row_stride ? (size_t)s.row_stride : (size_t)s.Ws * s.C;
-        const float *base = reinterpret_cast<const float *>(s.x) + (size_t)n * s.Hs * rs + cc0;
-#pragma unroll
-        for (int i = 0; i < NA; ++i) {
-            const int e = si ? eoff[1][i] : eoff[0][i];
-            const f32x4 *p = reinterpret_cast<const f32x4 *>(base + (e >= 0 ? e : 0));
-            pa[i][0] = p[0];
-            pa[i][1] = p[1];
-        }
-        const u32x4 *wsrc = reinterpret_cast<const u32x4 *>(wbase + (size_t)chunk * L::B_PLANE);
-#pragma unroll
-        for (int i = 0; i < NB; ++i) {
-            const int v = tid + i * 256;
-            if (v < NBV) pb[i] = wsrc[v];
-        }
-    };
-    auto commit = [&](int chunk) {
-        int si, cc0;
-        chunk_src(chunk, si, cc0);
-        const ConvSrc &s = A.src[si];
-        const bool on = s.scale != nullptr, relu = s.relu != 0;
-        const float *xf = s_xf + (si ? c0n : 0) + cc0 + slot * 8;
-        float sc[8], sh[8];
-        if (on) {
-#pragma unroll
-            for (int j = 0; j < 8; ++j) { sc[j] = xf[j]; sh[j] = xf[xfs + j]; }
-        }
-        f32x4 rr[NA][2];
-        if (s.res) {
-            const size_t rs = s.row_stride ? (size_t)s.row_stride : (size_t)s.Ws * s.C;
-            const float *rbase = reinterpret_cast<const float *>(s.res) + (size_t)n * s.Hs * rs + cc0;
-#pragma unroll
-            for (int i = 0; i < NA; ++i) {
-                const int e = si ? eoff[1][i] : eoff[0][i];
-                const f32x4 *p = reinterpret_cast<const f32x4 *>(rbase + (e >= 0 ? e : 0));
-                rr[i][0] = p[0];
-                rr[i][1] = p[1];
-            }
-        }
-        unsigned char *dst0 = lds_a + (tid / VPP) * PSTR + slot * 16;
-#pragma unroll
-        for (int i = 0; i < NA; ++i) {
-            if (tid + i * 256 >= NPIX * VPP) continue;
-            const int e = si ? eoff[1][i] : eoff[0][i];
-            u32x4 hi = {0u, 0u, 0u, 0u}, lo = {0u, 0u, 0u, 0u};
-            if (e >= 0) {
-                float v[8] = {pa[i][0][0], pa[i][0][1], pa[i][0][2], pa[i][0][3], pa[i][1][0], pa[i][1][1], pa[i][1][2], pa[i][1][3]};
-                if (on) {
-#pragma unroll
-                    for (int j = 0; j < 8; ++j) v[j] = fmaf(v[j], sc[j], sh[j]);
-                }
-                if (s.res) {
-                    const float r[8] = {rr[i][0][0], rr[i][0][1], rr[i][0][2], rr[i][0][3], rr[i][1][0], rr[i][1][1], rr[i][1][2], rr[i][1][3]};
-#pragma unroll
-                    for (int j = 0; j < 8; ++j) v[j] += r[j];
-                }
-                if (relu) {
-#pragma unroll
-                    for (int j = 0; j < 8; ++j) v[j] = fmaxf(v[j], 0.f);
-                }
-                split8(v, hi, lo);
-            }
-            unsigned char *d = dst0 + i * (256 / VPP) * PSTR;
-            *reinterpret_cast<u32x4 *>(d) = hi;
-            *reinterpret_cast<u32x4 *>(d + L::A_PLANE) = lo;
-        }
-        u32x4 *bdst = reinterpret_cast<u32x4 *>(lds_b);
-#pragma unroll
-        for (int i = 0; i < NB; ++i) {
-            const int v = tid + i * 256;
-            if (v < NBV) bdst[v] = pb[i];
-        }
-    };
 
     int abase[MPW];
 #pragma unroll
@@ -289,12 +69,12 @@
 #pragma unroll
             for (int r = 0; r < 16; ++r) acc[mi][ni][r] = 0.f;
 
-    issue(0);
+    S.issue(A, eoff, 0, wbase);
     for (int chunk = 0; chunk < A.nchunk; ++chunk) {
         __syncthreads();
-        commit(chunk);
+        S.commit(A, eoff, chunk, lds_a, lds_b);
         __syncthreads();
-        if (chunk + 1 < A.nchunk) issue(chunk + 1);
+        if (chunk + 1 < A.nchunk) S.issue(A, eoff, chunk + 1, wbase + (size_t)(chunk + 1) * L::B_PLANE);
 #pragma unroll
         for (int t = 0; t < TAPS; ++t) {
             bf16x8 ah[MPW], al[MPW], bh[NPW], bl[NPW];
@@ -319,50 +99,7 @@
     __syncthreads();
 
     const int cout0 = cout_tile * BN;
-    if (A.stats) {
-        float ssum[NPW], ssq[NPW];
-        const bool full_tile = y0 + TH <= A.H && x0 + TW <= A.W && !(A.debug & 16);
-#pragma unroll
-        for (int ni = 0; ni < NPW; ++ni) {
-            ssum[ni] = 0.f; ssq[ni] = 0.f;
-            if (full_tile) {
-#pragma unroll
-                for (int mi = 0; mi < MPW; ++mi)
-#pragma unroll
-                    for (int r = 0; r < 16; ++r) {
-                        const float v = acc[mi][ni][r];
-                        ssum[ni] += v;
-                        ssq[ni] = fmaf(v, v, ssq[ni]);
-                    }
-            } else {
-#pragma unroll
-            for (int mi = 0; mi < MPW; ++mi)
-#pragma unroll
-                for (int r = 0; r < 16; ++r) {
-                    const int m = (wm * MPW + mi) * 32 + (r & 3) + 8 * (r >> 2) + 4 * half;
-                    const float v = ((y0 + m / TW) < A.H && (x0 + m % TW) < A.W) ? acc[mi][ni][r] : 0.f;
-                    ssum[ni] += v;
-                    ssq[ni] = fmaf(v, v, ssq[ni]);
-                }
-            }
-            ssum[ni] += __shfl_xor(ssum[ni], 32);
-            ssq[ni] += __shfl_xor(ssq[ni], 32);
-            if (half == 0) {
-                s_stats[wave][0][(wn * NPW + ni) * 32 + l31] = ssum[ni];
-                s_stats[wave][1][(wn * NPW + ni) * 32 + l31] = ssq[ni];
-            }
-        }
-        __syncthreads();
-        if (tid < 2 * BN) {
-            const int which = tid / BN, col = tid % BN;
-            const int wn_of = col / (NPW * 32);
-            float v = 0.f;
-#pragma unroll
-            for (int k = 0; k < WM; ++k) v += s_stats[k * WN + wn_of][which][col];
-            const int co = cout0 + col;
-            if (co < A.Cout) A.stats[((size_t)tile * 2 + which) * A.Cout + co] = v;
-        }
-    }
+    if (A.stats) tile_stats32<TH, TW, BN, WM, WN, MPW, NPW>(A, acc, s_stats, (size_t)tile, y0, x0, cout0, tid);
     store_tile_f32<MPW, NPW, TW>(A, acc, n, y0, x0, wm * MPW, wn * NPW, half, l31, cout0, par >> 1, par & 1);
 }
 
@@ -634,6 +371,11 @@
     for (int i = 0; i < A.nsrc; ++i)
         CDNET_REQUIRE(!A.src[i].pool, "cdnet_conv_forward(f32): pooled sources must be materialised (cdnet_src_materialize)");
     CDNET_REQUIRE(!A.out_f16, "cdnet_conv_forward(f32): out_f16 must be 0");
+    if (A.live_taps)
+        CDNET_REQUIRE(A.live_taps == 1 && A.taps == 9 && A.taps1 == 0 && A.npar == 1 && A.ostride == 1 && A.nsrc == 2 && A.src[0].C == A.src[1].C &&
+                          A.src[0].C % 32 == 0,
+                      "cdnet_conv_forward(f32): live_taps needs a nine-tap launch over two row-parity views of equal C with C / 2 a multiple of 16 "
+                      "(got live_taps=%d taps=%d nsrc=%d C=%d, %d)", A.live_taps, A.taps, A.nsrc, A.src[0].C, A.nsrc > 1 ? A.src[1].C : 0);
     {
         const int rc = conv_forward_f32_ws(A, st);
         if (rc >= 0) return rc;
@@ -642,6 +384,10 @@
                              "(ask cdnet_conv_ws_eligible first)");
     CDNET_REQUIRE(A.taps1 == 0 || A.taps1 == A.taps, "cdnet_conv_forward(f32): a one-tap second source runs on conv_ws32_kernel only (ask cdnet_conv_ws_eligible)");
     CDNET_REQUIRE(!A.pool_out, "cdnet_conv_forward(f32): the fused max-pool output rides in conv_ws32_kernel's epilogue only (ask cdnet_conv_ws_eligible)");
+    if (A.taps == 9 || A.taps == 4) {
+        const int rc = conv_forward_f32_t(A, st);
+        if (rc >= 0) return rc;
+    }
     if (A.taps == 9) return dispatch_conv32<9>(A, st);
     if (A.taps == 4) return dispatch_conv32<4>(A, st);
     {
diff --git a/cdnet_amd/csrc/conv32_tile.h b/cdnet_amd/csrc/conv32_tile.h
--- /dev/null
+++ b/cdnet_amd/csrc/conv32_tile.h
@@ -0,0 +1,312 @@
+#pragma once
+#include "common.h"
+#include "conv_args.h"
+#include "split_bf16.h"
+
+namespace cdnet {
+namespace conv32 {
+
+constexpr int CK = 16;
+constexpr int PSTR = CK * 2 + 16;
+constexpr int XF_MAX = 2048;
+
+template <int TH, int TW, int BN, int TAPS>
+struct Lds32 {
+    static constexpr int NPIX = (TH + 2) * (TW + 2);
+    static constexpr int A_PLANE = NPIX * PSTR;
+    static constexpr int B_PLANE = TAPS * CK * BN * 2;
+    static constexpr int STAGE = 2 * A_PLANE + 2 * B_PLANE;
+    static constexpr int STATS_BYTES = 4 * 2 * BN * 4;
+    static constexpr int MAIN = ((STAGE > STATS_BYTES ? STAGE : STATS_BYTES) + 15) / 16 * 16;
+    static int bytes(int ctot) { return MAIN + 2 * ((ctot + 7) / 8 * 8) * 4; }
+};
+
+__device__ __forceinline__ void xcd_tile_order(int &tile, int &cout_tile) {
+    const int NC = (int)gridDim.y, lin = (int)blockIdx.y * (int)gridDim.x + (int)blockIdx.x;
+    const int T = (int)gridDim.x * NC, q = T >> 3, rem = T & 7;
+    const int xcd = lin & 7, idx = lin >> 3;
+    const int seq = xcd < rem ? xcd * (q + 1) + idx : rem * (q + 1) + (xcd - rem) * q + idx;
+    tile = seq / NC;
+    cout_tile = seq - tile * NC;
+}
+
+template <int TH, int TW, int WV, int NIMG = 1, bool RES = true>
+struct Stage32 {
+    static constexpr int HW_ = TW + 2, NPIX = (TH + 2) * (TW + 2), A_PLANE = NPIX * PSTR;
+    static constexpr int VPP = CK / 8;
+    static constexpr int NA = (NPIX * VPP + 255) / 256;
+    static constexpr int NBV = WV * NIMG;
+    static constexpr int NB = (NBV + 255) / 256;
+
+    using Eoff = unsigned long long[NA];
+    f32x4 pa[NA][2];
+    u32x4 pb[NB];
+    int tid, slot, n, c0n, xfs;
+    const float *s_xf;
+
+    __device__ __forceinline__ void init(const ConvArgs &A, float *xf_table, int tid_) {
+        tid = tid_;
+        slot = tid % VPP;
+        s_xf = xf_table;
+        c0n = A.src[0].C;
+        const int ctot = c0n + (A.nsrc > 1 ? A.src[1].C : 0);
+        xfs = (ctot + 7) / 8 * 8;
+        for (int c = tid; c < ctot; c += 256) {
+            const ConvSrc &S = c < c0n ? A.src[0] : A.src[1];
+            const int cc = c < c0n ? c : c - c0n;
+            xf_table[c] = S.scale ? S.scale[cc] : 1.f;
+            xf_table[xfs + c] = S.shift ? S.shift[cc] : 0.f;
+        }
+    }
+    __device__ __forceinline__ void geometry(const ConvArgs &A, Eoff &eoff, int n_, int y0, int x0) {
+        n = n_;
+#pragma unroll
+        for (int i = 0; i < NA; ++i) eoff[i] = 0;
+#pragma unroll
+        for (int si = 0; si < 2; ++si) {
+            if (si >= A.nsrc) continue;
+            const ConvSrc &s = A.src[si];
+            const int rs = s.row_stride ? s.row_stride : s.Ws * s.C;
+#pragma unroll
+            for (int i = 0; i < NA; ++i) {
+                const int v = tid + i * 256;
+                const int pix = v / VPP;
+                const int hy = pix / HW_, hx = pix - hy * HW_;
+                const int y = y0 - 1 + hy, x = x0 - 1 + hx;
+                const int ys = y - s.off_y, xs = x - s.off_x;
+                const bool ok = v < NPIX * VPP && (unsigned)y < (unsigned)A.H && (unsigned)x < (unsigned)A.W && (unsigned)ys < (unsigned)s.Hs &&
+                                (unsigned)xs < (unsigned)s.Ws;
+                eoff[i] |= (unsigned long long)(unsigned)(ok ? ys * rs + xs * s.C + slot * 8 : -1) << (32 * si);
+            }
+        }
+    }
+    static __device__ __forceinline__ void chunk_src(const ConvArgs &A, int c, int &si, int &cc0) {
+        const int n0 = A.src[0].C / CK;
+        if (c < n0) { si = 0; cc0 = c * CK; } else { si = 1; cc0 = (c - n0) * CK; }
+    }
+    __device__ __forceinline__ void issue(const ConvArgs &A, const Eoff &eoff, int chunk, const unsigned short *wchunk, size_t wimg_stride = 0) {
+        int si, cc0;
+        chunk_src(A, chunk, si, cc0);
+        const ConvSrc &s = A.src[si];
+        const size_t rs = s.row_stride ? (size_t)s.row_stride : (size_t)s.Ws * s.C;
+        const float *base = reinterpret_cast<const float *>(s.x) + (size_t)n * s.Hs * rs + cc0;
+#pragma unroll
+        for (int i = 0; i < NA; ++i) {
+            const int e = (int)(eoff[i] >> (32 * si));
+            const f32x4 *p = reinterpret_cast<const f32x4 *>(base + (e >= 0 ? e : 0));
+            pa[i][0] = p[0];
+            pa[i][1] = p[1];
+        }
+#pragma unroll
+        for (int i = 0; i < NB; ++i) {
+            const int v = tid + i * 256;
+            if (v < NBV) {
+                if constexpr (NIMG == 1) {
+                    pb[i] = reinterpret_cast<const u32x4 *>(wchunk)[v];
+                } else {
+                    const int img = v / WV;
+                    pb[i] = reinterpret_cast<const u32x4 *>(wchunk + (size_t)img * wimg_stride)[v - img * WV];
+                }
+            }
+        }
+    }
+    __device__ __forceinline__ void commit(const ConvArgs &A, const Eoff &eoff, int chunk, unsigned char *lds_a, unsigned char *lds_b) {
+        int si, cc0;
+        chunk_src(A, chunk, si, cc0);
+        const ConvSrc &s = A.src[si];
+        const bool on = s.scale != nullptr, relu = s.relu != 0;
+        const float *xf = s_xf + (si ? c0n : 0) + cc0 + slot * 8;
+        float sc[8], sh[8];
+        if (on) {
+#pragma unroll
+            for (int j = 0; j < 8; ++j) { sc[j] = xf[j]; sh[j] = xf[xfs + j]; }
+        }
+        f32x4 rr[NA][2];
+        if (RES && s.res) {
+            const size_t rs = s.row_stride ? (size_t)s.row_stride : (size_t)s.Ws * s.C;
+            const float *rbase = reinterpret_cast<const float *>(s.res) + (size_t)n * s.Hs * rs + cc0;
+#pragma unroll
+            for (int i = 0; i < NA; ++i) {
+                const int e = (int)(eoff[i] >> (32 * si));
+                const f32x4 *p = reinterpret_cast<const f32x4 *>(rbase + (e >= 0 ? e : 0));
+                rr[i][0] = p[0];
+                rr[i][1] = p[1];
+            }
+        }
+        unsigned char *dst0 = lds_a + (tid / VPP) * PSTR + slot * 16;
+#pragma unroll
+        for (int i = 0; i < NA; ++i) {
+            if (tid + i * 256 >= NPIX * VPP) continue;
+            const int e = (int)(eoff[i] >> (32 * si));
+            u32x4 hi = {0u, 0u, 0u, 0u}, lo = {0u, 0u, 0u, 0u};
+            if (e >= 0) {
+                float v[8] = {pa[i][0][0], pa[i][0][1], pa[i][0][2], pa[i][0][3], pa[i][1][0], pa[i][1][1], pa[i][1][2], pa[i][1][3]};
+                if (on) {
+#pragma unroll
+                    for (int j = 0; j < 8; ++j) v[j] = fmaf(v[j], sc[j], sh[j]);
+                }
+                if (RES && s.res) {
+                    const float r[8] = {rr[i][0][0], rr[i][0][1], rr[i][0][2], rr[i][0][3], rr[i][1][0], rr[i][1][1], rr[i][1][2], rr[i][1][3]};
+#pragma unroll
+                    for (int j = 0; j < 8; ++j) v[j] += r[j];
+                }
+                if (relu) {
+#pragma unroll
+                    for (int j = 0; j < 8; ++j) v[j] = fmaxf(v[j], 0.f);
+                }
+                split8(v, hi, lo);
+            }
+            unsigned char *d = dst0 + i * (256 / VPP) * PSTR;
+            *reinterpret_cast<u32x4 *>(d) = hi;
+            *reinterpret_cast<u32x4 *>(d + A_PLANE) = lo;
+        }
+        u32x4 *bdst = reinterpret_cast<u32x4 *>(lds_b);
+#pragma unroll
+        for (int i = 0; i < NB; ++i) {
+            const int v = tid + i * 256;
+            if (v < NBV) bdst[v] = pb[i];
+        }
+    }
+};
+
+template <int TH, int TW, int BN, int WM, int WN, int MPW, int NPW>
+__device__ __forceinline__ void tile_stats32(const ConvArgs &A, const f32x16 (&acc)[MPW][NPW], float (*s_stats)[2][BN], size_t row, int y0, int x0,
+                                             int cout0, int tid) {
+    const int lane = tid & 63, wave = tid >> 6;
+    const int wm = wave / WN, wn = wave % WN;
+    const int half = lane >> 5, l31 = lane & 31;
+    float ssum[NPW], ssq[NPW];
+    const bool full_tile = y0 + TH <= A.H && x0 + TW <= A.W && !(A.debug & 16);
+#pragma unroll
+    for (int ni = 0; ni < NPW; ++ni) {
+        ssum[ni] = 0.f; ssq[ni] = 0.f;
+        if (full_tile) {
+#pragma unroll
+            for (int mi = 0; mi < MPW; ++mi)
+#pragma unroll
+                for (int r = 0; r < 16; ++r) {
+                    const float v = acc[mi][ni][r];
+                    ssum[ni] += v;
+                    ssq[ni] = fmaf(v, v, ssq[ni]);
+                }
+        } else {
+#pragma unroll
+            for (int mi = 0; mi < MPW; ++mi)
+#pragma unroll
+                for (int r = 0; r < 16; ++r) {
+                    const int m = (wm * MPW + mi) * 32 + (r & 3) + 8 * (r >> 2) + 4 * half;
+                    const float v = ((y0 + m / TW) < A.H && (x0 + m % TW) < A.W) ? acc[mi][ni][r] : 0.f;
+                    ssum[ni] += v;
+                    ssq[ni] = fmaf(v, v, ssq[ni]);
+                }
+        }
+        ssum[ni] += __shfl_xor(ssum[ni], 32);
+        ssq[ni] += __shfl_xor(ssq[ni], 32);
+        if (half == 0) {
+            s_stats[wave][0][(wn * NPW + ni) * 32 + l31] = ssum[ni];
+            s_stats[wave][1][(wn * NPW + ni) * 32 + l31] = ssq[ni];
+        }
+    }
+    __syncthreads();
+    if (tid < 2 * BN) {
+        const int which = tid / BN, col = tid % BN;
+        const int wn_of = col / (NPW * 32);
+        float v = 0.f;
+#pragma unroll
+        for (int k = 0; k < WM; ++k) v += s_stats[k * WN + wn_of][which][col];
+        const int co = cout0 + col;
+        if (co < A.Cout) A.stats[(row * 2 + which) * A.Cout + co] = v;
+    }
+}
+
+template <int MPW, int NPW, int TW>
+__device__ __forceinline__ void store_tile_f32(const ConvArgs &A, const f32x16 (&acc)[MPW][NPW], int n, int y0, int x0, int mblock0, int nblock0,
+                                               int half, int l31, int cout0, int pa_, int pb_) {
+    const int Ho = A.H * A.ostride, Wo = A.W * A.ostride;
+    float *out = reinterpret_cast<float *>(A.out);
+    const float *eres = reinterpret_cast<const float *>(A.eres);
+    const bool full = y0 + 16 <= A.H && x0 + TW <= A.W && cout0 + (nblock0 + NPW) * 32 <= A.Cout && A.ostride == 1 && TW == 16 &&
+                      !(A.debug & 16);
+    if (full) {
+        const int cs = A.out_cstride, ce = A.Cout;
+        float *tb = out + (((size_t)n * A.H + y0) * A.W + x0) * cs + A.out_coff;
+        const float *te = eres ? eres + (((size_t)n * A.H + y0) * A.W + x0) * ce : nullptr;
+#pragma unroll
+        for (int ni = 0; ni < NPW; ++ni) {
+            const int co = cout0 + (nblock0 + ni) * 32 + l31;
+            const float osc = A.oscale ? A.oscale[co] : 1.f;
+            const float osh = fmaf(A.bias ? A.bias[co] : 0.f, osc, A.oshift ? A.oshift[co] : 0.f);
+            const float esc = (eres && A.eres_scale) ? A.eres_scale[co] : 1.f;
+            const float esh = (eres && A.eres_shift) ? A.eres_shift[co] : 0.f;
+            float *ob = tb + co;
+#pragma unroll
+            for (int mi = 0; mi < MPW; ++mi) {
+                const int rowb = ((mblock0 + mi) * 2) * A.W + 4 * half;
+                float ev[16];
+                if (eres) {
+#pragma unroll
+                    for (int r = 0; r < 16; ++r) {
+                        const int p = (r & 3) + 8 * (r >> 2);
+                        ev[r] = te[(rowb + (p / 16) * A.W + (p % 16)) * ce + co];
+                    }
+                }
+#pragma unroll
+                for (int r = 0; r < 16; ++r) {
+                    const int p = (r & 3) + 8 * (r >> 2);
+                    const int off = (rowb + (p / 16) * A.W + (p % 16)) * cs;
+                    float v = fmaf(acc[mi][ni][r], osc, osh);
+                    if (A.orelu) v = fmaxf(v, 0.f);
+                    if (eres) {
+                        v = fmaf(ev[r], esc, esh) + v;
+                        if (A.eres_relu) v = fmaxf(v, 0.f);
+                    }
+                    ob[off] = v;
+                }
+            }
+        }
+        return;
+    }
+#pragma unroll
+    for (int ni = 0; ni < NPW; ++ni) {
+        const int co = cout0 + (nblock0 + ni) * 32 + l31;
+        const bool cok = co < A.Cout;
+        const float osc = (A.oscale && cok) ? A.oscale[co] : 1.f;
+        const float osh = fmaf((A.bias && cok) ? A.bias[co] : 0.f, osc, (A.oshift && cok) ? A.oshift[co] : 0.f);
+        const float esc = (A.eres && A.eres_scale && cok) ? A.eres_scale[co] : 1.f;
+        const float esh = (A.eres && A.eres_shift && cok) ? A.eres_shift[co] : 0.f;
+#pragma unroll
+        for (int mi = 0; mi < MPW; ++mi) {
+            float ev[16];
+            if (A.eres) {
+#pragma unroll
+                for (int r = 0; r < 16; ++r) {
+                    const int m = (mblock0 + mi) * 32 + (r & 3) + 8 * (r >> 2) + 4 * half;
+                    int y = y0 + m / TW, x = x0 + m % TW;
+                    y = y < A.H ? y : A.H - 1; x = x < A.W ? x : A.W - 1;
+                    ev[r] = eres[(((size_t)n * A.H + y) * A.W + x) * A.Cout + (cok ? co : 0)];
+                }
+            }
+#pragma unroll
+            for (int r = 0; r < 16; ++r) {
+                const int m = (mblock0 + mi) * 32 + (r & 3) + 8 * (r >> 2) + 4 * half;
+                const int y = y0 + m / TW, x = x0 + m % TW;
+                float v = fmaf(acc[mi][ni][r], osc, osh);
+                if (A.orelu) v = fmaxf(v, 0.f);
+                if (A.eres) {
+                    v = fmaf(ev[r], esc, esh) + v;
+                    if (A.eres_relu) v = fmaxf(v, 0.f);
+                }
+                if (cok && y < A.H && x < A.W) {
+                    const size_t opix = ((size_t)n * Ho + (y * A.ostride + pa_)) * Wo + (x * A.ostride + pb_);
+                    out[opix * A.out_cstride + A.out_coff + co] = v;
+                }
+            }
+        }
+    }
+}
+
+}
+
+int conv_forward_f32_t(const ConvArgs &A, hipStream_t st);
+
+}
diff --git a/cdnet_amd/csrc/conv_args.h b/cdnet_amd/csrc/conv_args.h
--- a/cdnet_amd/csrc/conv_args.h
+++ b/cdnet_amd/csrc/conv_args.h
@@ -31,7 +31,7 @@
     const unsigned short *eres;
     const float *eres_scale, *eres_shift;
     int eres_f16, eres_relu;
-    int taps1, pad_;
+    int taps1, live_taps;
     unsigned short *pool_out;
     const float *dot_w, *dot_b;
     float *dot_out;
diff --git a/cdnet_amd/csrc/convt32.hip b/cdnet_amd/csrc/convt32.hip
--- /dev/null
+++ b/cdnet_amd/csrc/convt32.hip
@@ -0,0 +1,302 @@
+#include <type_traits>
+#include "common.h"
+#include "conv_args.h"
+#include "launch.h"
+#include "conv32_tile.h"
+
+using namespace cdnet;
+using namespace cdnet::conv32;
+
+namespace {
+
+template <int NP, int MPW, int NPW, int TH, int TW>
+__device__ __forceinline__ void store_quad_f32(const ConvArgs &A, const f32x16 (&acc)[NP][MPW][NPW], int n, int y0, int x0, int mblock0, int nblock0,
+                                               int half, int l31, int cout0, int a0) {
+    static_assert(TW == 8 || TW == 16, "4 half never carries into the row");
+    const int Ho = A.H * 2, Wo = A.W * 2, cs = A.out_cstride;
+    float *out = reinterpret_cast<float *>(A.out);
+    const bool full = y0 + TH <= A.H && x0 + TW <= A.W && (long long)(2 * TH) * Wo * cs < (1LL << 31) && !(A.debug & 16);
+#pragma unroll
+    for (int ni = 0; ni < NPW; ++ni) {
+        const int co = cout0 + (nblock0 + ni) * 32 + l31;
+        const bool cok = co < A.Cout;
+        const float osc = (A.oscale && cok) ? A.oscale[co] : 1.f;
+        const float osh = fmaf((A.bias && cok) ? A.bias[co] : 0.f, osc, (A.oshift && cok) ? A.oshift[co] : 0.f);
+        if (full) {
+            if (!cok) continue;
+            float *ob = out + (((size_t)n * Ho + 2 * y0) * Wo + 2 * x0 + 8 * half) * cs + A.out_coff + co;
+#pragma unroll
+            for (int mi = 0; mi < MPW; ++mi)
+#pragma unroll
+                for (int r = 0; r < 16; ++r) {
+                    const int m = (mblock0 + mi) * 32 + (r & 3) + 8 * (r >> 2);
+                    const int y = m / TW, x = m % TW;
+#pragma unroll
+                    for (int ar = 0; ar < NP / 2; ++ar) {
+                        const int off = ((2 * y + a0 + ar) * Wo + 2 * x) * cs;
+                        float v0 = fmaf(acc[2 * ar][mi][ni][r], osc, osh), v1 = fmaf(acc[2 * ar + 1][mi][ni][r], osc, osh);
+                        if (A.orelu) { v0 = fmaxf(v0, 0.f); v1 = fmaxf(v1, 0.f); }
+                        ob[off] = v0;
+                        ob[off + cs] = v1;
+                    }
+                }
+            continue;
+        }
+#pragma unroll
+        for (int mi = 0; mi < MPW; ++mi)
+#pragma unroll
+            for (int r = 0; r < 16; ++r) {
+                const int m = (mblock0 + mi) * 32 + (r & 3) + 8 * (r >> 2) + 4 * half;
+                const int y = y0 + m / TW, x = x0 + m % TW;
+                const bool ok = cok && y < A.H && x < A.W;
+#pragma unroll
+                for (int p = 0; p < NP; ++p) {
+                    float v = fmaf(acc[p][mi][ni][r], osc, osh);
+                    if (A.orelu) v = fmaxf(v, 0.f);
+                    if (ok) {
+                        const size_t opix = ((size_t)n * Ho + (y * 2 + a0 + (p >> 1))) * Wo + (x * 2 + (p & 1));
+                        out[opix * cs + A.out_coff + co] = v;
+                    }
+                }
+            }
+    }
+}
+
+template <int TH, int TW, int BN, int WM, int WN, int NP>
+__global__ __launch_bounds__(256, (TH == 16 && BN == 64) ? 1 : 2) void convt4_quad_f32_kernel(ConvArgs A) {
+    using L4 = Lds32<TH, TW, BN, 4>;
+    using L = Lds32<TH, TW, BN, 4 * NP>;
+    using Stage = Stage32<TH, TW, 2 * L4::B_PLANE / 16, NP, false>;
+    constexpr int HW_ = TW + 2;
+    constexpr int MT = TH * TW / 32, NT = BN / 32;
+    constexpr int MPW = MT / WM, NPW = NT / WN;
+    constexpr int NR = NP == 4 ? 3 : 2;
+    static_assert(MT % WM == 0 && NT % WN == 0 && WM * WN == 4 && (NP == 4 || NP == 2), "wave tiling");
+
+    extern __shared__ __attribute__((aligned(16))) unsigned char smem[];
+    unsigned char *lds_a = smem;
+    unsigned char *lds_b = smem + 2 * L::A_PLANE;
+    float (*s_stats)[2][BN] = reinterpret_cast<float (*)[2][BN]>(smem);
+
+    const int tid = threadIdx.x, lane = tid & 63, wave = tid >> 6;
+    const int wm = wave / WN, wn = wave % WN;
+    const int half = lane >> 5, l31 = lane & 31;
+    Stage S;
+    S.init(A, reinterpret_cast<float *>(smem + L::MAIN), tid);
+
+    const int tiles_x = (A.W + TW - 1) / TW, tiles_y = (A.H + TH - 1) / TH;
+    const int tiles_img = tiles_x * tiles_y;
+    int tile, cout_tile;
+    xcd_tile_order(tile, cout_tile);
+    const int n = tile / tiles_img, rt = tile - n * tiles_img;
+    const int ty_ = rt / tiles_x;
+    const int y0 = ty_ * TH, x0 = (rt - ty_ * tiles_x) * TW;
+    typename Stage::Eoff eoff;
+    S.geometry(A, eoff, n, y0, x0);
+    const size_t wpar = (size_t)gridDim.y * A.nchunk * (size_t)L4::B_PLANE;
+    const unsigned short *wtile = A.w + (size_t)cout_tile * A.nchunk * (size_t)L4::B_PLANE;
+    const int cout0 = cout_tile * BN;
+
+    int abase[MPW];
+#pragma unroll
+    for (int mi = 0; mi < MPW; ++mi) {
+        const int m = (wm * MPW + mi) * 32 + l31;
+        abase[mi] = ((m / TW) * HW_ + m % TW) * PSTR + half * 16;
+    }
+    const int bbase = half * BN * 16 + (wn * NPW * 32 + l31) * 16;
+
+    for (int pass = 0; pass < 4 / NP; ++pass) {
+        const int par0 = pass * NP;
+        const int arow = (NP == 4 ? 0 : pass) * HW_ * PSTR;
+        const unsigned short *wp = wtile + (size_t)par0 * wpar;
+        f32x16 acc[NP][MPW][NPW];
+#pragma unroll
+        for (int p = 0; p < NP; ++p)
+#pragma unroll
+            for (int mi = 0; mi < MPW; ++mi)
+#pragma unroll
+                for (int ni = 0; ni < NPW; ++ni)
+#pragma unroll
+                    for (int r = 0; r < 16; ++r) acc[p][mi][ni][r] = 0.f;
+
+        S.issue(A, eoff, 0, wp, wpar);
+        for (int chunk = 0; chunk < A.nchunk; ++chunk) {
+            __syncthreads();
+            S.commit(A, eoff, chunk, lds_a, lds_b);
+            __syncthreads();
+            if (chunk + 1 < A.nchunk) S.issue(A, eoff, chunk + 1, wp + (size_t)(chunk + 1) * L4::B_PLANE, wpar);
+#pragma unroll
+            for (int rr = NR - 1; rr >= 0; --rr)
+#pragma unroll
+                for (int c = 2; c >= 0; --c) {
+                    bf16x8 ah[MPW], al[MPW];
+#pragma unroll
+                    for (int mi = 0; mi < MPW; ++mi) {
+                        ah[mi] = *reinterpret_cast<const bf16x8 *>(lds_a + abase[mi] + arow + (rr * HW_ + c) * PSTR);
+                        al[mi] = *reinterpret_cast<const bf16x8 *>(lds_a + L::A_PLANE + abase[mi] + arow + (rr * HW_ + c) * PSTR);
+                    }
+#pragma unroll
+                    for (int p = 0; p < NP; ++p) {
+                        const int dy = rr - (NP == 4 ? (p >> 1) : 0), dx = c - (p & 1);
+                        if (dy < 0 || dy > 1 || dx < 0 || dx > 1) continue;
+                        const int t = (dy == 1 ? 0 : 2) + (dx == 1 ? 0 : 1);
+                        const unsigned char *img = lds_b + p * 2 * L4::B_PLANE + bbase + t * 2 * BN * 16;
+#pragma unroll
+                        for (int ni = 0; ni < NPW; ++ni) {
+                            const bf16x8 bh = *reinterpret_cast<const bf16x8 *>(img + ni * 512);
+                            const bf16x8 bl = *reinterpret_cast<const bf16x8 *>(img + L4::B_PLANE + ni * 512);
+#pragma unroll
+                            for (int mi = 0; mi < MPW; ++mi) acc[p][mi][ni] = mfma3(acc[p][mi][ni], ah[mi], al[mi], bh, bl);
+                        }
+                    }
+                }
+        }
+        __syncthreads();
+
+        if (A.stats) {
+#pragma unroll
+            for (int p = 0; p < NP; ++p) {
+                if (p) __syncthreads();
+                tile_stats32<TH, TW, BN, WM, WN, MPW, NPW>(A, acc[p], s_stats, ((size_t)n * 4 + par0 + p) * tiles_img + rt, y0, x0, cout0, tid);
+            }
+        }
+        store_quad_f32<NP, MPW, NPW, TH, TW>(A, acc, n, y0, x0, wm * MPW, wn * NPW, half, l31, cout0, par0 >> 1);
+    }
+}
+
+template <int TH, int TW, int BN, int WM, int WN>
+__global__ __launch_bounds__(256, 2) void conv_f32_live4_kernel(ConvArgs A) {
+    using L = Lds32<TH, TW, BN, 9>;
+    using Stage = Stage32<TH, TW, 2 * L::B_PLANE / 16>;
+    constexpr int HW_ = TW + 2;
+    constexpr int MT = TH * TW / 32, NT = BN / 32;
+    constexpr int MPW = MT / WM, NPW = NT / WN;
+    static_assert(MT % WM == 0 && NT % WN == 0 && WM * WN == 4, "wave tiling");
+
+    extern __shared__ __attribute__((aligned(16))) unsigned char smem[];
+    unsigned char *lds_a = smem;
+    unsigned char *lds_b = smem + 2 * L::A_PLANE;
+    float (*s_stats)[2][BN] = reinterpret_cast<float (*)[2][BN]>(smem);
+
+    const int tid = threadIdx.x, lane = tid & 63, wave = tid >> 6;
+    const int wm = wave / WN, wn = wave % WN;
+    const int half = lane >> 5, l31 = lane & 31;
+    Stage S;
+    S.init(A, reinterpret_cast<float *>(smem + L::MAIN), tid);
+
+    const int tiles_x = (A.W + TW - 1) / TW, tiles_y = (A.H + TH - 1) / TH;
+    const int tiles_img = tiles_x * tiles_y;
+    int tile, cout_tile;
+    xcd_tile_order(tile, cout_tile);
+    const int n = tile / tiles_img, rt = tile - n * tiles_img;
+    const int ty_ = rt / tiles_x;
+    const int y0 = ty_ * TH, x0 = (rt - ty_ * tiles_x) * TW;
+    typename Stage::Eoff eoff;
+    S.geometry(A, eoff, n, y0, x0);
+    const unsigned short *wbase = A.w + ((size_t)cout_tile * A.nchunk) * (size_t)(L::B_PLANE);
+
+    int abase[MPW];
+#pragma unroll
+    for (int mi = 0; mi < MPW; ++mi) {
+        const int m = (wm * MPW + mi) * 32 + l31;
+        abase[mi] = ((m / TW) * HW_ + m % TW) * PSTR + half * 16;
+    }
+    const int bbase = half * BN * 16 + (wn * NPW * 32 + l31) * 16;
+    const int chalf = A.src[0].C / 2;
+    f32x16 acc[MPW][NPW];
+#pragma unroll
+    for (int mi = 0; mi < MPW; ++mi)
+#pragma unroll
+        for (int ni = 0; ni < NPW; ++ni)
+#pragma unroll
+            for (int r = 0; r < 16; ++r) acc[mi][ni][r] = 0.f;
+
+    S.issue(A, eoff, 0, wbase);
+    for (int chunk = 0; chunk < A.nchunk; ++chunk) {
+        __syncthreads();
+        S.commit(A, eoff, chunk, lds_a, lds_b);
+        __syncthreads();
+        if (chunk + 1 < A.nchunk) S.issue(A, eoff, chunk + 1, wbase + (size_t)(chunk + 1) * L::B_PLANE);
+        int a, cc0;
+        Stage::chunk_src(A, chunk, a, cc0);
+        const int ty0 = 1 - a, tx0 = 1 - (cc0 >= chalf ? 1 : 0);
+        const int aoff = (ty0 * HW_ + tx0) * PSTR, boff = (ty0 * 3 + tx0) * 2 * BN * 16;
+#pragma unroll
+        for (int j = 0; j < 4; ++j) {
+            const int jy = j >> 1, jx = j & 1;
+            bf16x8 ah[MPW], al[MPW], bh[NPW], bl[NPW];
+#pragma unroll
+            for (int mi = 0; mi < MPW; ++mi) {
+                ah[mi] = *reinterpret_cast<const bf16x8 *>(lds_a + abase[mi] + aoff + (jy * HW_ + jx) * PSTR);
+                al[mi] = *reinterpret_cast<const bf16x8 *>(lds_a + L::A_PLANE + abase[mi] + aoff + (jy * HW_ + jx) * PSTR);
+            }
+#pragma unroll
+            for (int ni = 0; ni < NPW; ++ni) {
+                bh[ni] = *reinterpret_cast<const bf16x8 *>(lds_b + bbase + boff + (jy * 3 + jx) * 2 * BN * 16 + ni * 512);
+                bl[ni] = *reinterpret_cast<const bf16x8 *>(lds_b + L::B_PLANE + bbase + boff + (jy * 3 + jx) * 2 * BN * 16 + ni * 512);
+            }
+#pragma unroll
+            for (int mi = 0; mi < MPW; ++mi)
+#pragma unroll
+                for (int ni = 0; ni < NPW; ++ni) {
+                    acc[mi][ni] = mfma3(acc[mi][ni], ah[mi], al[mi], bh[ni], bl[ni]);
+                }
+        }
+    }
+    __syncthreads();
+
+    const int cout0 = cout_tile * BN;
+    if (A.stats) tile_stats32<TH, TW, BN, WM, WN, MPW, NPW>(A, acc, s_stats, (size_t)tile, y0, x0, cout0, tid);
+    store_tile_f32<MPW, NPW, TW>(A, acc, n, y0, x0, wm * MPW, wn * NPW, half, l31, cout0, 0, 0);
+}
+
+int source_channels(const ConvArgs &A) {
+    int ctot = 0;
+    for (int i = 0; i < A.nsrc; ++i) ctot += A.src[i].C;
+    return ctot;
+}
+
+template <int TH, int TW, int BN, int WM, int WN, int NP>
+int launch_quad(const ConvArgs &A, hipStream_t st) {
+    using L = Lds32<TH, TW, BN, 4 * NP>;
+    dim3 grid(cdiv(A.W, TW) * cdiv(A.H, TH) * A.N, cdiv(A.Cout, BN), 1);
+    g_conv_last_form = conv_form(CDNET_CONV_FAMILY_T4QUAD, BN, 4, 0, false, false, false, 0, 0, TH);
+    return launch_lds<convt4_quad_f32_kernel<TH, TW, BN, WM, WN, NP>>(grid, 256, L::bytes(XF_MAX), L::bytes(source_channels(A)), st,
+                                                                       "hipFuncSetAttribute(convt32)", "convt4_quad_f32_kernel", A);
+}
+
+template <int TH, int TW, int BN, int WM, int WN>
+int launch_live4(const ConvArgs &A, hipStream_t st) {
+    using L = Lds32<TH, TW, BN, 9>;
+    dim3 grid(cdiv(A.W, TW) * cdiv(A.H, TH) * A.N, cdiv(A.Cout, BN), 1);
+    g_conv_last_form = conv_form(CDNET_CONV_FAMILY_LIVE4, BN, 9, 0, false, false, false, 0, 0, TH);
+    return launch_lds<conv_f32_live4_kernel<TH, TW, BN, WM, WN>>(grid, 256, L::bytes(XF_MAX), L::bytes(source_channels(A)), st,
+                                                                  "hipFuncSetAttribute(convt32)", "conv_f32_live4_kernel", A);
+}
+
+}
+
+namespace cdnet {
+
+int conv_forward_f32_t(const ConvArgs &A, hipStream_t st) {
+    const bool k64 = A.tile == 16 && A.BN == 64, k32 = A.tile == 16 && A.BN == 32, k8 = A.tile == 8 && A.BN == 64;
+    if (!k64 && !k32 && !k8) return -1;
+    if (A.taps == 4) {
+        if (A.npar != 4 || A.ostride != 2 || A.eres || (A.debug & (CONV_DBG_ONE_TILE | CONV_DBG_NO_STREAM_1X1))) return -1;
+        for (int i = 0; i < A.nsrc; ++i)
+            if (A.src[i].res) return -1;
+        int n_cu = 0;
+        if (const int rc = cu_count(&n_cu)) return rc;
+        const long long wgs = (long long)cdiv(A.W, A.tile) * cdiv(A.H, A.tile) * A.N * cdiv(A.Cout, A.BN);
+        if (wgs < n_cu && 4 * wgs >= n_cu && !(A.debug & CONV_DBG_PERSIST_SMALL)) return -1;
+        if (k64) return launch_quad<16, 16, 64, 4, 1, 2>(A, st);
+        if (k32) return launch_quad<16, 16, 32, 4, 1, 4>(A, st);
+        return launch_quad<8, 8, 64, 2, 2, 4>(A, st);
+    }
+    if (A.taps != 9 || !A.live_taps) return -1;
+    if (k64) return launch_live4<16, 16, 64, 4, 1>(A, st);
+    if (k32) return launch_live4<16, 16, 32, 4, 1>(A, st);
+    return launch_live4<8, 8, 64, 2, 2>(A, st);
+}
+
+}
diff --git a/cdnet_amd/engine.py b/cdnet_amd/engine.py
--- a/cdnet_amd/engine.py
+++ b/cdnet_amd/engine.py
@@ -166,12 +166,17 @@
     return out
 
 
+def bwdt4_live_taps(a, b):
+    return tuple(3 * (1 - a + jy) + (1 - b + jx) for jy in (0, 1) for jx in (0, 1))
+
+
 CONV_DEBUG = 0
+CONVT4_QUAD = os.environ.get('CDNET_CONVT4_QUAD', '1') != '0'
 
 
 def conv_forward(srcs, wpacked, Cout, cfg, taps=9, transposed=False, bias=None, oscale=None, oshift=None,
                  orelu=False, out=None, stats=None, H=None, W=None, out_dtype=torch.bfloat16, eres=None, query_ws=False, bns=None, taps1=0, pool_out=None, dot=None,
-                 pad_chunks=0, debug_or=0, out_coff=0):
+                 pad_chunks=0, debug_or=0, out_coff=0, live_taps=False):
     tile, CK, BN = cfg[:3]
     s0 = srcs[0]
     f32 = s0.f32
@@ -211,8 +216,12 @@
     a.out_f16 = int(out is not None and out.dtype == torch.float16)
     a.ws = 0
     a.taps1 = taps1
+    assert not live_taps or (f32 and taps == 9 and len(srcs) == 2)
+    a.live_taps = int(live_taps)
     a.pool_out = _dp(pool_out)
     a.debug = CONV_DEBUG | debug_or
+    if f32 and taps == 4 and not CONVT4_QUAD:
+        a.debug |= 256
     a.f32 = int(f32)
     assert out is None or (out.dtype == torch.float32) == f32
     if eres is not None:
diff --git a/cdnet_amd/trainer.py b/cdnet_amd/trainer.py
--- a/cdnet_amd/trainer.py
+++ b/cdnet_amd/trainer.py
@@ -18,6 +18,7 @@
 WGRAD_STREAM = True
 HEAD_BWD_FUSE = True
 HEAD_COEF_SRC = os.environ.get('CDNET_HEAD_COEF_SRC', '1') != '0'
+BWDT4_LIVE_TAPS = os.environ.get('CDNET_BWDT4_LIVE_TAPS', '1') != '0'
 _WGRAD_DEFER = 0x100
 _WGRAD_DEEP_HW = 16384
 
@@ -739,7 +740,8 @@
         else:
             gin = self.buf(('din', L.name), (N, H, W, cin_total), runtime.act_dtype())
             views = [Src(g, view=(a * 2 * W * Cout, H, W, 2 * Cout, 4 * W * Cout)) for a in (0, 1)]
-            engine.conv_forward(views, wpb, cin_total, cfgb, taps=(9 if L.kind == 'convT4' else 1), out=gin, H=H, W=W)
+            live = BWDT4_LIVE_TAPS and L.kind == 'convT4' and gin.dtype == torch.float32 and Cout % 16 == 0
+            engine.conv_forward(views, wpb, cin_total, cfgb, taps=(9 if L.kind == 'convT4' else 1), out=gin, H=H, W=W, live_taps=live)
         coff = 0
         for s, dead_s in zip(srcs, dead):
             if s.is_input or dead_s:
diff --git a/include/cdnet_hip.h b/include/cdnet_hip.h
--- a/include/cdnet_hip.h
+++ b/include/cdnet_hip.h
@@ -111,7 +111,7 @@
     const float *eres_scale, *eres_shift;
     int eres_f16, eres_relu;
     int taps1;
-    int pad_;
+    int live_taps;
     uint16_t *pool_out;
     const float *dot_w;
     const float *dot_b;
@@ -140,6 +140,8 @@
 #define CDNET_CONV_FAMILY_F32    4
 #define CDNET_CONV_FAMILY_STREAM 5
 #define CDNET_CONV_FAMILY_WS32   6
+#define CDNET_CONV_FAMILY_T4QUAD 7
+#define CDNET_CONV_FAMILY_LIVE4  8
 int cdnet_conv_forward_last_form(void);
 
 typedef struct cdnet_dilated_conv_args {
```

New measurement: 1106, median of 6. Within noise of the previous version (+0.8%).
